# lxtGH/Video-K-Net

Hardware: AMD Instinct MI355X
Metric: frames/sec (S=3, N=100, 1024x2048) (higher is better)
Workload: dtype f32; 1 GPU; cfg2 video_knet_s3_r50: VideoKernelIterHead S=3, N=100 proposals + 17 stuff = 117 kernels, C=256, 1024x2048 frame -> 128x256 stride-8 features, ffn tracking link, x4 bilinear upsample of the final logits; streams_per_gpu=1, parallelism=frame-sharded dp1, x_storage=fp32

## Files before the change

### include/vkn.h

```cpp
#ifndef VKN_H
#define VKN_H
#include <stddef.h>
#include <stdint.h>

#ifdef __cplusplus
extern "C" {
#endif

#define VKN_VERSION 0x000600

#define VKN_OK 0
#define VKN_E_ARG (-1)
#define VKN_E_SHAPE (-2)
#define VKN_E_WORKSPACE (-3)
#define VKN_E_LAUNCH (-4)
#define VKN_E_ALIGN (-5)
#define VKN_E_RANGE (-6)

#define VKN_STATUS_RANGE 1u

#define VKN_FLAG_REF_KERNELS 1u
#define VKN_FLAG_EXACT_GEMM 2u
#define VKN_FLAG_LOGITS_HANDOFF 4u
#define VKN_FLAG_BITS_HANDOFF 16u
#define VKN_X_F32 0
#define VKN_X_F16 1
#define VKN_X_BF16 2
#define VKN_FLAG_X_F16 64u
#define VKN_FLAG_X_BF16 128u
#define VKN_FLAG_CHAIN_LAUNCHES 256u
#define VKN_FLAG_CHAIN_PERSISTENT 512u
#define VKN_FLAG_JOIN_EARLY 32768u
#define VKN_FLAG_SCALED_F16 16384u
#define VKN_FLAG_CHAIN_BF16X3 65536u
#define VKN_FLAG_CHAIN_KSPLIT 8192u
#define VKN_FLAG_SERIAL_LINK 32u
#define VKN_FLAG_CLIP_LINK 8u

#define VKN_FLAG_INIT_SEPARATE 131072u
#define VKN_FLAG_PHASE_A 1024u
#define VKN_FLAG_PHASE_B 2048u
#define VKN_FLAG_PHASE_C 4096u
#define VKN_FLAG_PHASE_MASK (VKN_FLAG_PHASE_A | VKN_FLAG_PHASE_B | VKN_FLAG_PHASE_C)

#define VKN_MAX_FCS 4

typedef struct VknDims {
    int B;
    int N;
    int C;
    int H, W;
    int heads;
    int ff;
    int ncls;
    int n_cls_fcs, n_mask_fcs;
    float thr_logit;
    float ln_eps;
} VknDims;

typedef struct VknStageWeights {
    const float *ft_w, *ft_b, *ft_wT;
    const float *dyn_w, *dyn_b;
    const float *inp_w, *inp_b;
    const float *ig_w, *ig_b, *ug_w, *ug_b;
    const float *norm_in_w, *norm_in_b;
    const float *norm_out_w, *norm_out_b;
    const float *inorm_in_w, *inorm_in_b;
    const float *inorm_out_w, *inorm_out_b;
    const float *fc_w, *fc_b, *fc_norm_w, *fc_norm_b;
    const float *attn_in_w, *attn_in_b;
    const float *attn_out_w, *attn_out_b;
    const float *attn_norm_w, *attn_norm_b;
    const float *ffn1_w, *ffn1_b;
    const float *ffn2_w, *ffn2_b;
    const float *ffn_norm_w, *ffn_norm_b;
    const float *cls_fc_w[VKN_MAX_FCS], *cls_ln_w[VKN_MAX_FCS], *cls_ln_b[VKN_MAX_FCS];
    const float *fc_cls_w, *fc_cls_b;
    const float *mask_fc_w[VKN_MAX_FCS], *mask_ln_w[VKN_MAX_FCS], *mask_ln_b[VKN_MAX_FCS];
    const float *fc_mask_w, *fc_mask_b;
    const float *pa_in_w, *pa_in_b, *pa_out_w, *pa_out_b, *pa_norm_w, *pa_norm_b;
    const float *lffn1_w, *lffn1_b, *lffn2_w, *lffn2_b, *lffn_norm_w, *lffn_norm_b;
    const void* prepared;
    size_t prepared_bytes;
} VknStageWeights;

int vkn_version(void);
const char* vkn_strerror(int code);
int vkn_workspace_init(void* ws, size_t ws_bytes, void* stream);
int vkn_workspace_status(void* ws, size_t ws_bytes, void* stream);
size_t vkn_sizeof_dims(void);
size_t vkn_sizeof_stage_weights(void);

size_t vkn_gather_workspace_bytes(int B, int N, int C, int P);
int vkn_mask_gather_f32(const float* x, const float* mask_logits, float thr_logit, float* xraw_out, float* cnt_out, int B,
                        int N, int C, int P, void* ws, size_t ws_bytes, unsigned flags, void* stream);

int vkn_mask_gather_real_f32(const float* x, const float* a, float* out, float* asum_out, int B, int N, int C, int P, void* ws,
                             size_t ws_bytes, void* stream);

size_t vkn_decode_workspace_bytes(int B, int N, int C);
int vkn_mask_decode_f32(const float* x, const float* kernels, const float* bias, float* out, int B, int N, int C, int P,
                        void* ws, size_t ws_bytes, unsigned flags, void* stream);
int vkn_mask_decode_scaled_f32(const float* x, const float* kernels, const float* bias, const float* out_scale, float* out, int B,
                               int N, int C, int P, void* ws, size_t ws_bytes, unsigned flags, void* stream);

int vkn_split_planes_f32(const float* kernels, void* kf_hi, void* kf_lo, int B, int N, int C, void* stream);
int vkn_mask_decode_planes_f32(const float* x, const void* kf_hi, const void* kf_lo, const float* bias, float* out, int B,
                               int N, int C, int P, void* stream);
int vkn_mask_decode_planes_x(const void* x, int x_dtype, const void* kf_hi, const void* kf_lo, const float* bias, float* out, int B,
                             int N, int C, int P, void* stream);

int vkn_decode_gather_supported(int C, int P);
int vkn_decode_gather_f32(const float* x, const void* kf_hi, const void* kf_lo, const float* bias, float thr_logit,
                          float* xraw_out, float* cnt_out, int B, int N, int C, int P, void* ws, size_t ws_bytes, void* stream);
int vkn_decode_gather_x(const void* x, int x_dtype, const void* kf_hi, const void* kf_lo, const float* bias, float thr_logit,
                        float* xraw_out, float* cnt_out, int B, int N, int C, int P, void* ws, size_t ws_bytes, void* stream);

int vkn_upsample_bilinear_f32(const float* in, float* out, int planes, int H, int W, int S, void* stream);
int vkn_upsample_bilinear_f16out(const float* in, void* out_f16, int planes, int H, int W, int S, void* stream);
int vkn_upsample_bilinear_bwd_f32(const float* grad_out, float* grad_in, int planes, int H, int W, int S, void* stream);

int vkn_focal_loss_blocks(int M, int ncls);
// ... 291 lines not shown
```

### video-k-net_amd/csrc/vkn_api.hip

```cpp
#include "../../include/vkn.h"
#include "vkn_common.h"
#include "vkn_launch.h"

namespace {

struct Carver {
    char* base;
    size_t off;
    template <class T>
    T* take(size_t n) {
        off = (off + 255) & ~(size_t)255;
        T* p = base ? reinterpret_cast<T*>(base + off) : nullptr;
        off += n * sizeof(T);
        return p;
    }
};

inline bool aligned16(const void* p) { return (reinterpret_cast<uintptr_t>(p) & 15) == 0; }
inline int npt_of(int N) { return (N + 31) / 32 * 32; }

struct StageWs {
    float *part, *cntp, *xraw, *cnt, *xfeat, *params, *inputf, *ig, *ug, *f, *obj1, *qkv, *ao, *obj2, *h, *partial, *t1, *t2,
        *maskfeat, *kb, *kern32, *lq, *lkv, *lobj, *lupd, *lf;
    _Float16 *kfh, *kfl;
    int* status;
};


enum MasksFrom {
    FROM_LOGITS,
    FROM_BITS,
    FROM_GATHERED,
    FROM_XFEAT
};
enum MasksTo {
    TO_LOGITS,
    TO_BITS,
    TO_GATHER,
    TO_KERNELS,
    TO_NONE
};
struct StageCall {
    const VknStageWeights* w = nullptr;
    const float *x = nullptr, *obj_in = nullptr;
    float *obj_out = nullptr, *cls_logits = nullptr, *x_feat_out = nullptr;
    bool cls_sigmoid = false;
    MasksFrom from = FROM_LOGITS;
    const float *masks_in = nullptr, *xfeat_in = nullptr;
    const unsigned* bits_in = nullptr;
    MasksTo to = TO_LOGITS;
    float* masks_out = nullptr;
    unsigned* bits_out = nullptr;
    float *kern_out = nullptr, *kb_out = nullptr;
    hipEvent_t prof0 = nullptr, prof1 = nullptr, obj_ready = nullptr;
    float* up_out = nullptr;
    int up_stride = 0, up_chunk = 0;
    bool* up_done = nullptr;
    const float* prev_obj = nullptr;
    float* track_out = nullptr;
    const VknStageWeights* link_pre = nullptr;
    const float* prev_pre = nullptr;
    const VknStageWeights* link_track = nullptr;
    int track_src = 0;
    bool keep_xfeat = false;
    const void* touch_next = nullptr;
    size_t touch_next_bytes = 0;
};

struct PrepW {
    const void *ft, *ftT, *dyn, *inp, *ig, *ug, *fc, *attn_in, *attn_out, *ffn1, *ffn2, *cls_fc[VKN_MAX_FCS], *fc_cls,
        *mask_fc[VKN_MAX_FCS], *fc_mask, *pa_in, *pa_in_kv, *pa_out, *lffn1, *lffn2;
    const void *dynft, *dec;
    float *dynft32, *bcnt, *dec32, *decb, *dvec, *kb0, *fmT;
    float* chain_consts;
    const void* h2[VKN_H2_COUNT];
    float* h2_scale;
    unsigned* h2_scratch;
};

inline bool has_composites(const VknDims* d, const VknStageWeights* w) {
    return w->ft_w && w->ft_wT && w->ft_b && w->dyn_w && w->dyn_b && w->fc_mask_w && w->fc_mask_b && d->n_mask_fcs > 0;
}

struct PrepItem {
    const float* src;
    int nout, k;
    const void** dst;
};

struct H2Shape { int nout, k; };
inline H2Shape h2_shape(const VknDims* d, const VknStageWeights* w, int i) {
    const int C = d->C, FF = d->ff;
    switch (i) {
        case VKN_H2_DYNFT: case VKN_H2_DYN: case VKN_H2_INP: return H2Shape{2 * C, C};
        case VKN_H2_IN: return H2Shape{3 * C, C};
        case VKN_H2_FFN1: return H2Shape{FF, C};
        case VKN_H2_FFN2: return H2Shape{C, FF};
        case VKN_H2_FCCLS: return H2Shape{w->fc_cls_w ? d->ncls : 0, C};
        default: return H2Shape{C, C};
    }
}

inline bool chain_width_ok(const VknDims* d) { return d->C == 256 && d->ff % 256 == 0 && d->ff <= 2048; }
inline bool chain_shape_ok(const VknDims* d) { return chain_width_ok(d) && d->n_cls_fcs == 1 && d->n_mask_fcs == 1; }

size_t carve_prepared(const VknDims* d, const VknStageWeights* w, char* base, PrepW* p, PrepItem* it = nullptr, int* n_out = nullptr) {
    const int C = d->C, FF = d->ff;
    Carver c{base, 0};
    int n = 0;
    auto add = [&](const float* src, int nout, int k, const void** dst) {
        *dst = src ? c.take<char>(vkn_split_w3_bytes(nout, k)) : nullptr;
        if (src && it) it[n] = PrepItem{src, nout, k, dst};
        if (src) ++n;
    };
    add(w->ft_w, C, C, &p->ft); add(w->ft_wT, C, C, &p->ftT);
    add(w->dyn_w, 2 * C, C, &p->dyn); add(w->inp_w, 2 * C, C, &p->inp);
    add(w->ig_w, C, C, &p->ig); add(w->ug_w, C, C, &p->ug); add(w->fc_w, C, C, &p->fc);
    add(w->attn_in_w, 3 * C, C, &p->attn_in); add(w->attn_out_w, C, C, &p->attn_out);
    add(w->ffn1_w, FF, C, &p->ffn1); add(w->ffn2_w, C, FF, &p->ffn2);
    for (int i = 0; i < VKN_MAX_FCS; ++i) add(i < d->n_cls_fcs ? w->cls_fc_w[i] : nullptr, C, C, &p->cls_fc[i]);
    add(w->fc_cls_w, d->ncls, C, &p->fc_cls);
    for (int i = 0; i < VKN_MAX_FCS; ++i) add(i < d->n_mask_fcs ? w->mask_fc_w[i] : nullptr, C, C, &p->mask_fc[i]);
    add(w->fc_mask_w, C, C, &p->fc_mask);
    add(w->pa_in_w, C, C, &p->pa_in); add(w->pa_in_w ? w->pa_in_w + (size_t)C * C : nullptr, 2 * C, C, &p->pa_in_kv);
    add(w->pa_out_w, C, C, &p->pa_out);
    add(w->lffn1_w, FF, C, &p->lffn1); add(w->lffn2_w, C, FF, &p->lffn2);
    p->dynft = p->dec = nullptr;
    p->dynft32 = p->bcnt = p->dec32 = p->decb = p->dvec = p->kb0 = p->fmT = p->chain_consts = nullptr;
    if (has_composites(d, w)) {
        const size_t Cs = d->C;
        p->dynft = c.take<char>(vkn_split_w3_bytes(2 * C, C));
        p->dec = c.take<char>(vkn_split_w3_bytes(C, C));
        p->dynft32 = c.take<float>(2 * Cs * Cs);
        p->bcnt = c.take<float>(2 * Cs);
        p->dec32 = c.take<float>(Cs * Cs);
        p->decb = c.take<float>(Cs);
        p->dvec = c.take<float>(Cs);
        p->kb0 = c.take<float>(4);
        p->fmT = c.take<float>(Cs * Cs);
        if (C == 256 && FF <= 2048) p->chain_consts = c.take<float>(vkn_chain_consts_floats());
    }
    for (int i = 0; i < VKN_H2_COUNT; ++i) p->h2[i] = nullptr;
    p->h2_scale = nullptr;
    p->h2_scratch = nullptr;
    if (has_composites(d, w) && chain_shape_ok(d) && w->inp_w && w->ig_w && w->ug_w && w->fc_w && w->attn_in_w && w->attn_out_w && w->ffn1_w &&
        w->ffn2_w && w->cls_fc_w[0] && w->mask_fc_w[0]) {
        for (int i = 0; i < VKN_H2_COUNT; ++i) {
            const H2Shape h = h2_shape(d, w, i);
            if (h.nout > 0) p->h2[i] = c.take<char>(vkn_split_h2_bytes(h.nout, h.k));
// ... 153 lines not shown
        e.bias = in_b + C; e.out = s.lkv; e.ldo = 2 * C;
        VKN_TRY(vkn_launch_gemm(kvsrc, nullptr, C, in_w + (size_t)C * C, in_kv_ws, M, C, 2 * C, 1, nullptr, e, st));
        VKN_TRY(vkn_launch_attn(s.lq, C, s.lkv, s.lkv + C, 2 * C, s.ao, C, d->B, d->N, d->N, heads, hd, st));
    }
    e = mk_epi(d);
    e.bias = out_b; e.resid = qsrc; e.ldr = C; e.ln_w = nw; e.ln_b = nb; e.out = out; e.ldo = C;
    return vkn_launch_gemm(s.ao, nullptr, C, out_w, out_ws, M, C, C, 1, nullptr, e, st);
}

int run_updator(const VknDims* d, const VknStageWeights* w, const PrepW& pw, const float* xfeat, const float* xraw,
                const float* cnt, const float* obj_in, float* out, const StageWs& s, hipStream_t st) {
    const int C = d->C, M = d->B * d->N;
    const bool fuse = (C == 256);
    VknGemmProb pr[2];
    VknEpi e = mk_epi(d); e.out = s.params; e.ldo = 2 * C;
    if (fuse) { e.ln_w = w->norm_out_w; e.ln_b = w->norm_out_b; e.ln_from_col = C; }
    if (xraw && pw.dynft) {
        e.bias = pw.bcnt; e.rowscale = cnt; e.bias2 = w->dyn_b;
        pr[0] = VknGemmProb{xraw, nullptr, nullptr, nullptr, C, pw.dynft32, pw.dynft, 2 * C, e};
    } else {
        e.bias = w->dyn_b;
        pr[0] = VknGemmProb{xfeat, nullptr, nullptr, nullptr, C, w->dyn_w, pw.dyn, 2 * C, e};
    }
    e = mk_epi(d); e.bias = w->inp_b; e.out = s.inputf; e.ldo = 2 * C;
    if (fuse) { e.ln_w = w->inorm_out_w; e.ln_b = w->inorm_out_b; e.ln_from_col = C; }
    pr[1] = VknGemmProb{obj_in, nullptr, nullptr, nullptr, C, w->inp_w, pw.inp, 2 * C, e};
    VKN_TRY(vkn_launch_gemm_group(pr, 2, M, C, 1, nullptr, st));
    float* ig = s.ig;
    float* ug = fuse ? s.ig + C : s.ug;
    const int ldg = fuse ? 2 * C : C;
    e = mk_epi(d); e.bias = w->ig_b; e.ln_w = w->inorm_in_w; e.ln_b = w->inorm_in_b; e.act = 2; e.out = ig; e.ldo = ldg;
    pr[0] = VknGemmProb{s.inputf, s.params, nullptr, nullptr, 2 * C, w->ig_w, pw.ig, C, e};
    e = mk_epi(d); e.bias = w->ug_b; e.ln_w = w->norm_in_w; e.ln_b = w->norm_in_b; e.act = 2; e.out = ug; e.ldo = ldg;
    pr[1] = VknGemmProb{s.inputf, s.params, nullptr, nullptr, 2 * C, w->ug_w, pw.ug, C, e};
    VKN_TRY(vkn_launch_gemm_group(pr, 2, M, C, 1, nullptr, st));
    e = mk_epi(d); e.bias = w->fc_b; e.ln_w = w->fc_norm_w; e.ln_b = w->fc_norm_b; e.act = 1; e.out = out; e.ldo = C;
    if (fuse) {
        pr[0] = VknGemmProb{ug, s.params + C, ig, s.inputf + C, 2 * C, w->fc_w, pw.fc, C, e};
        return vkn_launch_gemm_group(pr, 1, M, C, 1, nullptr, st);
    }
    VKN_TRY(vkn_launch_ku_mix(s.params, s.inputf, ig, ug, w->norm_out_w, w->norm_out_b, w->inorm_out_w, w->inorm_out_b,
                              d->ln_eps, s.f, M, C, st));
    return vkn_launch_gemm(s.f, nullptr, C, w->fc_w, pw.fc, M, C, C, 1, nullptr, e, st);
}

bool link_ks_ok(const VknDims* d, const VknStageWeights* w, const PrepW& pw, unsigned flags);
int run_link_ks(const VknDims* d, const VknStageWeights* w, const PrepW& pw, const float* cur, const float* kv, float* out,
                const StageWs& s, hipStream_t st);
int run_link(const VknDims* d, const VknStageWeights* w, const PrepW& pw, const float* cur, const float* prev,
             float* out, const StageWs& s, hipStream_t st, const float* update_feature = nullptr, unsigned flags = 0) {
    if (!w->pa_in_w || !w->lffn1_w) return VKN_E_ARG;
    const float* kv = prev;
    if (update_feature) {
        if (!w->dyn_w) return VKN_E_ARG;
        StageWs su = s;
        su.f = s.lf;
        VKN_TRY(run_updator(d, w, pw, update_feature, nullptr, nullptr, prev, s.lupd, su, st));
        kv = s.lupd;
    }
    if (link_ks_ok(d, w, pw, flags)) return run_link_ks(d, w, pw, cur, kv, out, s, st);
    VKN_TRY(run_attention(d, s, cur, kv, 8, w->pa_in_w, pw.pa_in, pw.pa_in_kv, w->pa_in_b, w->pa_out_w, pw.pa_out, w->pa_out_b,
                          w->pa_norm_w, w->pa_norm_b, s.t1, st));
    return run_ffn(d, s, s.t1, w->lffn1_w, pw.lffn1, w->lffn1_b, w->lffn2_w, pw.lffn2, w->lffn2_b, w->lffn_norm_w,
                   w->lffn_norm_b, out, st);
}

int carve_pw(const VknDims* d, const VknStageWeights* w, unsigned flags, PrepW* pw) {
    *pw = PrepW{};
    if (w->prepared && !(flags & VKN_FLAG_EXACT_GEMM) &&
        carve_prepared(d, w, static_cast<char*>(const_cast<void*>(w->prepared)), pw) > w->prepared_bytes)
        return VKN_E_WORKSPACE;
    return VKN_OK;
}

int run_track_link(const VknDims* d, const StageWs& s, hipStream_t st, const float* cur, const float* prev, float* out,
                   const VknStageWeights* w, const VknStageWeights* link_track, int track_src, const float* xfeat, unsigned flags) {
    const VknStageWeights* lw = link_track ? link_track : w;
    PrepW pw;
    VKN_TRY(carve_pw(d, lw, flags, &pw));
    return run_link(d, lw, pw, cur, prev, out, s, st, link_track ? (track_src == 2 ? cur : xfeat) : nullptr, flags);
}

int run_gather(const VknDims* d, const float* x, const float* masks, const unsigned* bits, const StageWs& s, unsigned flags,
               hipStream_t st, const void* touch = nullptr, size_t touch_bytes = 0) {
    const int B = d->B, N = d->N, C = d->C, P = d->H * d->W, xdt = xdt_of(flags);
    if (flags & VKN_FLAG_REF_KERNELS) return vkn_launch_gather_ref(x, masks, d->thr_logit, s.xraw, s.cnt, B, N, C, P, st);
    if (bits) return vkn_launch_gather_bits(x, bits, s.xraw, s.cnt, s.part, s.cntp, B, N, C, P, st, xdt, s.status, touch, touch_bytes);
    return vkn_launch_gather(x, masks, d->thr_logit, s.xraw, s.cnt, s.part, s.cntp, B, N, C, P, st, xdt, s.status, touch, touch_bytes);
}

int final_decode(const VknDims* d, const float* x, const StageWs& s, const float* kb, float* masks_out, unsigned flags,
                 hipStream_t st, hipEvent_t prof0, hipEvent_t prof1, float* up_out, int up_stride, int up_chunk, bool* up_done) {
    const int B = d->B, N = d->N, C = d->C, P = d->H * d->W;
    if ((flags & VKN_FLAG_REF_KERNELS) || (P & 1)) return vkn_launch_decode_ref(x, s.kern32, kb, masks_out, B, N, C, P, st);
    const int ch = (up_out && up_chunk > 0 && up_chunk < B) ? up_chunk : B;
    const size_t NPTC = (size_t)npt_of(N) * C;
    for (int b0 = 0; b0 < B; b0 += ch) {
        const int bn = (B - b0 < ch) ? B - b0 : ch;
        const float* xb = reinterpret_cast<const float*>(reinterpret_cast<const char*>(x) + (size_t)b0 * C * P * (xdt_of(flags) ? 2 : 4));
        if (b0 == 0 && prof0 && hipEventRecord(prof0, st) != hipSuccess) return VKN_E_LAUNCH;
        VKN_TRY(vkn_launch_decode(xb, s.kfh + b0 * NPTC, s.kfl + b0 * NPTC, kb ? kb + (size_t)b0 * N : nullptr,
                                  masks_out + (size_t)b0 * N * P, bn, N, C, P, st, xdt_of(flags)));
        if (b0 == 0 && prof1 && hipEventRecord(prof1, st) != hipSuccess) return VKN_E_LAUNCH;
        if (ch < B)
            VKN_TRY(vkn_launch_upsample(masks_out + (size_t)b0 * N * P,
                                        (flags & VKN_FLAG_SCALED_F16) ? reinterpret_cast<float*>(reinterpret_cast<_Float16*>(up_out) + (size_t)b0 * N * P * up_stride * up_stride)
                                                                      : up_out + (size_t)b0 * N * P * up_stride * up_stride,
                                        bn * N, d->H, d->W, up_stride, st, (flags & VKN_FLAG_SCALED_F16) ? 1 : 0));
    }
    if (ch < B && up_done) *up_done = true;
    return VKN_OK;
}

inline int persistent_min_row_tiles(const PrepW& pw, unsigned flags) {
    return (!(flags & VKN_FLAG_CHAIN_BF16X3) && pw.h2_scale && pw.h2[VKN_H2_DYNFT]) ? 22 : 64;
}
inline unsigned pw_off(const VknStageWeights* w, const void* p) {
    return (unsigned)(static_cast<const char*>(p) - static_cast<const char*>(w->prepared));
}
inline bool chain_weights_ok(const PrepW& pw, bool have_cls) {
    return pw.dynft && pw.dyn && pw.dec && pw.inp && pw.ig && pw.ug && pw.fc && pw.attn_in && pw.attn_out && pw.ffn1 && pw.ffn2 &&
           pw.cls_fc[0] && pw.mask_fc[0] && (!have_cls || pw.fc_cls);
}
inline bool chain_stage_ok(const VknDims* d, const VknStageWeights* w, const PrepW& pw, bool have_cls) {
    return chain_shape_ok(d) && w->prepared && w->prepared_bytes < (1ull << 31) && chain_weights_ok(pw, have_cls) && w->ffn1_w &&
           w->cls_ln_w[0] && w->mask_ln_w[0];
}
bool chain_fast_ok(const VknDims* d, const VknStageWeights* w, const PrepW& pw, unsigned flags, bool have_cls) {
    if (flags & (VKN_FLAG_CHAIN_LAUNCHES | VKN_FLAG_EXACT_GEMM)) return false;
    if (vkn_dbg_env("VKN_CHAIN_LAUNCHES", 0)) return false;
    if (!(flags & VKN_FLAG_CHAIN_PERSISTENT) && !vkn_dbg_env("VKN_CHAIN_PERSISTENT", 0) &&
        (d->B * d->N + 31) / 32 < persistent_min_row_tiles(pw, flags))
        return false;
    return pw.chain_consts && chain_stage_ok(d, w, pw, have_cls);
}
inline bool chain_h2(const PrepW& pw, unsigned flags, bool have_cls) {
    return !(flags & VKN_FLAG_CHAIN_BF16X3) && pw.h2_scale && pw.h2[VKN_H2_DYNFT] && pw.h2[VKN_H2_DEC] && (!have_cls || pw.h2[VKN_H2_FCCLS]);
}

int run_chain_fast(const VknDims* d, const VknStageWeights* w, const PrepW& pw, const float* a0, bool a0_raw, const float* cnt,
                   const float* obj_in, float* obj_out, float* cls_logits, bool cls_sigmoid, float* kern32_out, const StageWs& s,
                   hipStream_t st, bool h2 = false) {
    const int M = d->B * d->N, C = d->C;
    VknChainA a{};
    a.a0 = a0; a.obj_in = obj_in; a.rowscale = a0_raw ? cnt : nullptr;
    a.wbase = w->prepared; a.wbytes = w->prepared_bytes;
    if (h2) {
        a.off_dyn = pw_off(w, pw.h2[a0_raw ? VKN_H2_DYNFT : VKN_H2_DYN]);
        a.off_inp = pw_off(w, pw.h2[VKN_H2_INP]); a.off_ig = pw_off(w, pw.h2[VKN_H2_IG]); a.off_ug = pw_off(w, pw.h2[VKN_H2_UG]);
        a.off_fc = pw_off(w, pw.h2[VKN_H2_FC]); a.off_in = pw_off(w, pw.h2[VKN_H2_IN]);
    } else {
        a.off_dyn = pw_off(w, a0_raw ? pw.dynft : pw.dyn);
        a.off_inp = pw_off(w, pw.inp); a.off_ig = pw_off(w, pw.ig); a.off_ug = pw_off(w, pw.ug); a.off_fc = pw_off(w, pw.fc);
        a.off_in = pw_off(w, pw.attn_in);
    }
    a.consts = pw.chain_consts;
    a.eps = d->ln_eps; a.M = M; a.obj1 = s.obj1; a.qkv = s.qkv; a.status = s.status;
    VKN_TRY(h2 ? vkn_launch_chain_a_h2(a, st) : vkn_launch_chain_a(a, st));
    VKN_TRY(vkn_launch_attn(s.qkv, 3 * C, s.qkv + C, s.qkv + 2 * C, 3 * C, s.ao, C, d->B, d->N, d->N, d->heads, C / d->heads, st));
    VknChainC c{};
    c.ao = s.ao; c.obj1 = s.obj1; c.wbase = w->prepared; c.wbytes = w->prepared_bytes;
    if (h2) {
        c.off_out = pw_off(w, pw.h2[VKN_H2_OUT]); c.off_ffn1 = pw_off(w, pw.h2[VKN_H2_FFN1]); c.off_ffn2 = pw_off(w, pw.h2[VKN_H2_FFN2]);
        c.off_clsfc = pw_off(w, pw.h2[VKN_H2_CLSFC]); c.off_maskfc = pw_off(w, pw.h2[VKN_H2_MASKFC]);
        c.off_fccls = pw.h2[VKN_H2_FCCLS] ? pw_off(w, pw.h2[VKN_H2_FCCLS]) : 0u; c.off_dec = pw_off(w, pw.h2[VKN_H2_DEC]);
    } else {
        c.off_out = pw_off(w, pw.attn_out); c.off_ffn1 = pw_off(w, pw.ffn1); c.off_ffn2 = pw_off(w, pw.ffn2);
        c.off_clsfc = pw_off(w, pw.cls_fc[0]); c.off_maskfc = pw_off(w, pw.mask_fc[0]);
        c.off_fccls = pw.fc_cls ? pw_off(w, pw.fc_cls) : 0u; c.off_dec = pw_off(w, pw.dec);
    }
    c.consts = pw.chain_consts; c.kb0 = pw.kb0;
    c.ff = d->ff; c.ncls = d->ncls; c.cls_sigmoid = cls_sigmoid ? 1 : 0; c.eps = d->ln_eps; c.M = M;
    c.obj_out = obj_out; c.cls_out = cls_logits; c.kb_out = s.kb;
    if (kern32_out) c.kern_out = kern32_out;
    else { c.plane_hi = s.kfh; c.plane_lo = s.kfl; }
    c.rows_per_frame = d->N; c.NPT = npt_of(d->N); c.status = s.status;
    return h2 ? vkn_launch_chain_c_h2(c, st) : vkn_launch_chain_c(c, st);
}

#define VKN_KS_MAX_ROW_TILES 16
inline bool ks_width_ok(const VknDims* d) {
    return chain_width_ok(d) && (d->ff % 512 == 0 || d->ff <= 1024);
}
bool chain_ks_ok(const VknDims* d, const VknStageWeights* w, const PrepW& pw, unsigned flags, bool have_cls) {
    if (flags & (VKN_FLAG_CHAIN_LAUNCHES | VKN_FLAG_CHAIN_PERSISTENT | VKN_FLAG_EXACT_GEMM)) return false;
    if (vkn_dbg_env("VKN_CHAIN_LAUNCHES", 0) || vkn_dbg_env("VKN_CHAIN_PERSISTENT", 0) || !vkn_dbg_env("VKN_CHAIN_KSPLIT", 1)) return false;
    if (!(flags & VKN_FLAG_CHAIN_KSPLIT) && (d->B * d->N + 31) / 32 > VKN_KS_MAX_ROW_TILES) return false;
    if (!ks_width_ok(d) || !chain_stage_ok(d, w, pw, have_cls)) return false;
    const void* v16[] = {w->inorm_in_w, w->inorm_in_b, w->norm_in_w, w->norm_in_b, w->norm_out_w, w->norm_out_b, w->inorm_out_w, w->inorm_out_b,
                         w->fc_norm_w, w->fc_norm_b, w->attn_norm_w, w->attn_norm_b, w->ffn_norm_w, w->ffn_norm_b, w->ffn2_b,
                         w->cls_ln_w[0], w->cls_ln_b[0], w->mask_ln_w[0], w->mask_ln_b[0], pw.dvec};
    for (const void* p : v16)
        if (!p || !aligned16(p)) return false;
    return true;
}

VknKsProb ks_prob(const float* a, int lda, const void* W, int Nout, int KT, float eps) {
    VknKsProb p{};
    p.pro.a[0] = a; p.pro.lda[0] = lda; p.pro.nsum = 1; p.pro.eps = eps;
    p.Wsplit = W; p.Nout = Nout; p.KT = KT;
    return p;
}

int run_chain_ks(const VknDims* d, const VknStageWeights* w, const PrepW& pw, const float* a0, bool a0_raw, const float* cnt,
                 const float* obj_in, float* obj_out, float* cls_logits, bool cls_sigmoid, float* kern32_out, const StageWs& s,
                 hipStream_t st, hipEvent_t obj_ready) {
    const int M = d->B * d->N, C = d->C, FF = d->ff;
    const float eps = d->ln_eps;
    VknKsProb pr[2];
    pr[0] = ks_prob(a0, C, a0_raw ? pw.dynft : pw.dyn, 2 * C, 8, eps);
    if (a0_raw) { pr[0].epi.bias = pw.bcnt; pr[0].epi.rowscale = cnt; pr[0].epi.bias2 = w->dyn_b; }
    else pr[0].epi.bias = w->dyn_b;
    pr[0].epi.out = s.params; pr[0].epi.ldo = 2 * C;
    pr[1] = ks_prob(obj_in, C, pw.inp, 2 * C, 8, eps);
    pr[1].epi.bias = w->inp_b; pr[1].epi.out = s.inputf; pr[1].epi.ldo = 2 * C;
    VKN_TRY(vkn_launch_gemm_ks(pr, 2, 0, 0, 1, 0, M, st));
    pr[0] = ks_prob(s.inputf, 2 * C, pw.ig, C, 8, eps);
    pr[0].pro.a[1] = s.params; pr[0].pro.lda[1] = 2 * C;
    pr[1] = pr[0];
    pr[0].epi.bias = w->ig_b; pr[0].epi.out = s.ig; pr[0].epi.ldo = 2 * C;
    pr[1].Wsplit = pw.ug; pr[1].epi.bias = w->ug_b; pr[1].epi.out = s.ig + C; pr[1].epi.ldo = 2 * C;
    VKN_TRY(vkn_launch_gemm_ks(pr, 2, 1, 0, 1, 0, M, st));
    pr[0] = ks_prob(s.ig, 2 * C, pw.fc, C, 8, eps);
    pr[0].pro.a[1] = s.ig + C; pr[0].pro.lda[1] = 2 * C;
    pr[0].pro.a[2] = s.params + C; pr[0].pro.lda[2] = 2 * C;
    pr[0].pro.a[3] = s.inputf + C; pr[0].pro.lda[3] = 2 * C;
    pr[0].pro.ln_w[0] = w->inorm_in_w; pr[0].pro.ln_b[0] = w->inorm_in_b;
    pr[0].pro.ln_w[1] = w->norm_in_w; pr[0].pro.ln_b[1] = w->norm_in_b;
    pr[0].pro.ln_w[2] = w->norm_out_w; pr[0].pro.ln_b[2] = w->norm_out_b;
    pr[0].pro.ln_w[3] = w->inorm_out_w; pr[0].pro.ln_b[3] = w->inorm_out_b;
    pr[0].epi.bias = w->fc_b; pr[0].epi.out = s.f; pr[0].epi.ldo = C;
    VKN_TRY(vkn_launch_gemm_ks(pr, 1, 2, 0, 1, 0, M, st));
    pr[0] = ks_prob(s.f, C, pw.attn_in, 3 * C, 8, eps);
    pr[0].pro.ln_w[0] = w->fc_norm_w; pr[0].pro.ln_b[0] = w->fc_norm_b; pr[0].pro.act = 1;
    pr[0].pro.side_out = s.obj1; pr[0].pro.ld_side = C;
    pr[0].epi.bias = w->attn_in_b; pr[0].epi.out = s.qkv; pr[0].epi.ldo = 3 * C;
    VKN_TRY(vkn_launch_gemm_ks(pr, 1, 0, 0, 1, 0, M, st));
    VKN_TRY(vkn_launch_attn(s.qkv, 3 * C, s.qkv + C, s.qkv + 2 * C, 3 * C, s.ao, C, d->B, d->N, d->N, d->heads, C / d->heads, st));
    pr[0] = ks_prob(s.ao, C, pw.attn_out, C, 8, eps);
    pr[0].epi.bias = w->attn_out_b; pr[0].epi.resid = s.obj1; pr[0].epi.ldr = C; pr[0].epi.out = s.obj2; pr[0].epi.ldo = C;
    VKN_TRY(vkn_launch_gemm_ks(pr, 1, 0, 0, 1, 0, M, st));
    pr[0] = ks_prob(s.obj2, C, pw.ffn1, FF, 8, eps);
    pr[0].pro.ln_w[0] = w->attn_norm_w; pr[0].pro.ln_b[0] = w->attn_norm_b;
    pr[0].pro.side_out = s.t1; pr[0].pro.ld_side = C;
    pr[0].epi.bias = w->ffn1_b; pr[0].epi.act = 1; pr[0].epi.out = s.h; pr[0].epi.ldo = FF;
    VKN_TRY(vkn_launch_gemm_ks(pr, 1, 0, 0, 1, 0, M, st));
    const int kpw = (FF % 512 == 0) ? 2 : 1, zch = FF / (256 * kpw);
    pr[0] = ks_prob(s.h, FF, pw.ffn2, C, FF / 32, eps);
    pr[0].epi.out = s.partial; pr[0].epi.ldo = C;
    VKN_TRY(vkn_launch_gemm_ks(pr, 1, 0, zch, kpw, (long long)M * C, M, st));
    pr[0] = ks_prob(s.partial, C, pw.cls_fc[0], C, 8, eps);
    pr[0].pro.nsum = zch; pr[0].pro.sum_stride = (long long)M * C;
    pr[0].pro.pbias = w->ffn2_b; pr[0].pro.presid = s.t1; pr[0].pro.ldr = C;
    pr[0].pro.ln_w[0] = w->ffn_norm_w; pr[0].pro.ln_b[0] = w->ffn_norm_b;
    pr[1] = pr[0];
    pr[0].pro.side_out = obj_out; pr[0].pro.ld_side = C;
    pr[0].epi.out = s.lkv; pr[0].epi.ldo = 2 * C;
    pr[1].Wsplit = pw.mask_fc[0]; pr[1].epi.out = s.lkv + C; pr[1].epi.ldo = 2 * C;
    VKN_TRY(vkn_launch_gemm_ks(pr, 2, 0, 0, 1, 0, M, st));
    if (obj_ready && hipEventRecord(obj_ready, st) != hipSuccess) return VKN_E_LAUNCH;
    int np = 0;
    if (cls_logits) {
        pr[np] = ks_prob(s.lkv, 2 * C, pw.fc_cls, d->ncls, 8, eps);
        pr[np].pro.ln_w[0] = w->cls_ln_w[0]; pr[np].pro.ln_b[0] = w->cls_ln_b[0]; pr[np].pro.act = 1;
        pr[np].epi.bias = w->fc_cls_b; pr[np].epi.act = cls_sigmoid ? 2 : 0; pr[np].epi.out = cls_logits; pr[np].epi.ldo = d->ncls;
        ++np;
    }
    pr[np] = ks_prob(s.lkv + C, 2 * C, pw.dec, C, 8, eps);
    pr[np].pro.ln_w[0] = w->mask_ln_w[0]; pr[np].pro.ln_b[0] = w->mask_ln_b[0]; pr[np].pro.act = 1;
    pr[np].pro.dot_vec = pw.dvec; pr[np].pro.dot_bias = pw.kb0; pr[np].pro.dot_out = s.kb;
    pr[np].epi.bias = pw.decb; pr[np].epi.ldo = C;
    if (kern32_out) pr[np].epi.out = kern32_out;
    else { pr[np].epi.plane_hi = s.kfh; pr[np].epi.plane_lo = s.kfl; pr[np].epi.rows_per_frame = d->N; pr[np].epi.NPT = npt_of(d->N); }
    ++np;
    return vkn_launch_gemm_ks(pr, np, 0, 0, 1, 0, M, st);
}

bool link_ks_ok(const VknDims* d, const VknStageWeights* w, const PrepW& pw, unsigned flags) {
    if (flags & (VKN_FLAG_CHAIN_LAUNCHES | VKN_FLAG_CHAIN_PERSISTENT | VKN_FLAG_EXACT_GEMM)) return false;
    if (vkn_dbg_env("VKN_CHAIN_LAUNCHES", 0) || !vkn_dbg_env("VKN_CHAIN_KSPLIT", 1)) return false;
    if (!(flags & VKN_FLAG_CHAIN_KSPLIT) && (d->B * d->N + 31) / 32 > VKN_KS_MAX_ROW_TILES) return false;
    if (!ks_width_ok(d)) return false;
    if (!pw.pa_in || !pw.pa_in_kv || !pw.pa_out || !pw.lffn1 || !pw.lffn2) return false;
    if (!w->pa_norm_w || !w->pa_norm_b || !aligned16(w->pa_norm_w) || !aligned16(w->pa_norm_b)) return false;
    return true;
}

int run_link_ks(const VknDims* d, const VknStageWeights* w, const PrepW& pw, const float* cur, const float* kv, float* out,
                const StageWs& s, hipStream_t st) {
    const int M = d->B * d->N, C = d->C, FF = d->ff;
    const float eps = d->ln_eps;
    VknKsProb pr[2];
    pr[0] = ks_prob(cur, C, pw.pa_in, C, 8, eps);
    pr[0].epi.bias = w->pa_in_b; pr[0].epi.out = s.lq; pr[0].epi.ldo = C;
    pr[1] = ks_prob(kv, C, pw.pa_in_kv, 2 * C, 8, eps);
    pr[1].epi.bias = w->pa_in_b ? w->pa_in_b + C : nullptr; pr[1].epi.out = s.lkv; pr[1].epi.ldo = 2 * C;
    VKN_TRY(vkn_launch_gemm_ks(pr, 2, 0, 0, 1, 0, M, st));
    VKN_TRY(vkn_launch_attn(s.lq, C, s.lkv, s.lkv + C, 2 * C, s.ao, C, d->B, d->N, d->N, 8, C / 8, st));
    pr[0] = ks_prob(s.ao, C, pw.pa_out, C, 8, eps);
    pr[0].epi.bias = w->pa_out_b; pr[0].epi.resid = cur; pr[0].epi.ldr = C; pr[0].epi.out = s.t1; pr[0].epi.ldo = C;
    VKN_TRY(vkn_launch_gemm_ks(pr, 1, 0, 0, 1, 0, M, st));
    pr[0] = ks_prob(s.t1, C, pw.lffn1, FF, 8, eps);
    pr[0].pro.ln_w[0] = w->pa_norm_w; pr[0].pro.ln_b[0] = w->pa_norm_b;
    pr[0].pro.side_out = s.lf; pr[0].pro.ld_side = C;
    pr[0].epi.bias = w->lffn1_b; pr[0].epi.act = 1; pr[0].epi.out = s.h; pr[0].epi.ldo = FF;
    VKN_TRY(vkn_launch_gemm_ks(pr, 1, 0, 0, 1, 0, M, st));
    const int kpw = (FF % 512 == 0) ? 2 : 1, zch = FF / (256 * kpw);
    pr[0] = ks_prob(s.h, FF, pw.lffn2, C, FF / 32, eps);
    pr[0].epi.out = s.partial; pr[0].epi.ldo = C;
    VKN_TRY(vkn_launch_gemm_ks(pr, 1, 0, zch, kpw, (long long)M * C, M, st));
    VknEpi e = mk_epi(d);
    e.bias = w->lffn2_b; e.resid = s.lf; e.ldr = C; e.ln_w = w->lffn_norm_w; e.ln_b = w->lffn_norm_b; e.out = out; e.ldo = C;
    return vkn_launch_rowepi(s.partial, zch, M, C, e, st);
}

int emit_masks(const VknDims* d, const StageCall& c, const StageWs& s, bool ref_decode, const float* kern32, const float* kb,
               const void* touch, size_t touch_bytes, unsigned flags, hipStream_t st) {
    const int B = d->B, N = d->N, C = d->C, P = d->H * d->W, xdt = xdt_of(flags);
    if (c.to == TO_KERNELS) {
        if (c.kb_out && kb && hipMemcpyAsync(c.kb_out, kb, (size_t)B * N * sizeof(float), hipMemcpyDeviceToDevice, st) != hipSuccess)
            return VKN_E_LAUNCH;
        return VKN_OK;
    }
    if (c.to == TO_NONE) return VKN_OK;
    if (ref_decode) return vkn_launch_decode_ref(c.x, kern32, kb, c.masks_out, B, N, C, P, st);
    if (c.to == TO_GATHER)
        return vkn_launch_fused_decode_gather(c.x, s.kfh, s.kfl, kb, d->thr_logit, s.xraw, s.cnt, s.part, s.cntp, B, N, C, P, st, xdt, s.status,
                                              touch, touch_bytes);
    if (c.to == TO_BITS) return vkn_launch_decode_bits(c.x, s.kfh, s.kfl, kb, c.bits_out, d->thr_logit, B, N, C, P, st, xdt);
    return final_decode(d, c.x, s, kb, c.masks_out, flags, st, c.prof0, c.prof1, c.up_out, c.up_stride, c.up_chunk, c.up_done);
}

int run_stage(const VknDims* d, const StageCall& c, const StageWs& s, unsigned flags, hipStream_t st) {
    const VknStageWeights* w = c.w;
    const int N = d->N, C = d->C, P = d->H * d->W, M = d->B * N;
    const bool ref = (flags & VKN_FLAG_REF_KERNELS) != 0;
    const bool chain_only = c.to == TO_KERNELS, given_xfeat = c.from == FROM_XFEAT;
    const bool ref_decode = ref || (P & 1) || chain_only;
    const bool has_ft = w->ft_w != nullptr;
    const bool have_cls = w->fc_cls_w && c.cls_logits;
    float* const cls_logits = have_cls ? c.cls_logits : nullptr;
    const bool pre_link = c.link_pre && c.prev_pre;
    const bool need_xfeat = (pre_link && c.link_pre->dyn_w) || (c.link_track && c.track_src == 1) || c.keep_xfeat;
    if (xdt_of(flags) && !chain_only && (ref || (P % 64) != 0)) return VKN_E_SHAPE;
    PrepW pw;
    VKN_TRY(carve_pw(d, w, flags, &pw));
    const bool comp = pw.dynft != nullptr;
    const bool fewrow = comp && chain_ks_ok(d, w, pw, flags, have_cls), persistent = comp && chain_fast_ok(d, w, pw, flags, have_cls);
    const bool fast = fewrow || persistent;

    const bool will_fast = !given_xfeat && persistent && vkn_dbg_env("VKN_CHAIN_TOUCH", 1);
    const void* touch_nx = vkn_dbg_env("VKN_CHAIN_TOUCH", 1) ? c.touch_next : nullptr;
    const size_t touch_nx_bytes = touch_nx ? c.touch_next_bytes : 0;
    if (c.from == FROM_LOGITS || c.from == FROM_BITS)
        VKN_TRY(run_gather(d, c.x, c.masks_in, c.from == FROM_BITS ? c.bits_in : nullptr, s, flags, st, will_fast ? w->prepared : nullptr,
                           will_fast ? w->prepared_bytes : 0));

    float* xfeat = c.x_feat_out ? c.x_feat_out : s.xfeat;
    VknEpi e = mk_epi(d);
    if (given_xfeat) {
        xfeat = const_cast<float*>(c.xfeat_in);
    } else if (has_ft) {
        if (!comp || c.x_feat_out || need_xfeat) {
            e.bias = w->ft_b; e.rowscale = s.cnt; e.out = xfeat; e.ldo = C;
            VKN_TRY(vkn_launch_gemm(s.xraw, nullptr, C, w->ft_w, pw.ft, M, C, C, 1, nullptr, e, st));
        }
    } else {
        if (hipMemcpyAsync(xfeat, s.xraw, (size_t)M * C * sizeof(float), hipMemcpyDeviceToDevice, st) != hipSuccess)
            return VKN_E_LAUNCH;
    }

    const float* obj_in = c.obj_in;
    if (pre_link) {
        PrepW pl;
        VKN_TRY(carve_pw(d, c.link_pre, flags, &pl));
        VKN_TRY(run_link(d, c.link_pre, pl, obj_in, c.prev_pre, s.lobj, s, st, c.link_pre->dyn_w ? xfeat : nullptr, flags));
        obj_in = s.lobj;
    }

    const float* kb = has_ft ? s.kb : nullptr;
    float* const kern32 = ref_decode ? (chain_only ? c.kern_out : s.kern32) : nullptr;
    const bool link = c.prev_obj && c.track_out;
    if (fast) {
        const bool raw = !given_xfeat;
        if (fewrow) {
            VKN_TRY(run_chain_ks(d, w, pw, raw ? s.xraw : xfeat, raw, s.cnt, obj_in, c.obj_out, cls_logits, c.cls_sigmoid, kern32, s, st, c.obj_ready));
        } else {
            VKN_TRY(run_chain_fast(d, w, pw, raw ? s.xraw : xfeat, raw, s.cnt, obj_in, c.obj_out, cls_logits, c.cls_sigmoid, kern32, s, st,
                                   chain_h2(pw, flags, have_cls)));
            if (c.obj_ready && hipEventRecord(c.obj_ready, st) != hipSuccess) return VKN_E_LAUNCH;
        }
        VKN_TRY(emit_masks(d, c, s, ref_decode, s.kern32, kb, touch_nx, touch_nx_bytes, flags, st));
        if (link) VKN_TRY(run_track_link(d, s, st, c.obj_out, c.prev_obj, c.track_out, w, c.link_track, c.track_src, xfeat, flags));
        return VKN_OK;
    }

    VKN_TRY(run_updator(d, w, pw, xfeat, (comp && !given_xfeat) ? s.xraw : nullptr, s.cnt, obj_in, s.obj1, s, st));

    VKN_TRY(run_attention(d, s, s.obj1, s.obj1, d->heads, w->attn_in_w, pw.attn_in, nullptr, w->attn_in_b, w->attn_out_w,
                          pw.attn_out, w->attn_out_b, w->attn_norm_w, w->attn_norm_b, s.obj2, st));
    if (w->ffn1_w) {
        VKN_TRY(run_ffn(d, s, s.obj2, w->ffn1_w, pw.ffn1, w->ffn1_b, w->ffn2_w, pw.ffn2, w->ffn2_b, w->ffn_norm_w,
                        w->ffn_norm_b, c.obj_out, st));
    } else {
        if (hipMemcpyAsync(c.obj_out, s.obj2, (size_t)M * C * sizeof(float), hipMemcpyDeviceToDevice, st) != hipSuccess)
            return VKN_E_LAUNCH;
    }
    const float* obj3 = c.obj_out;

    const bool fork_late = vkn_dbg_env("VKN_LINK_FORK_LATE", 0) != 0;
    if (c.obj_ready && !fork_late && hipEventRecord(c.obj_ready, st) != hipSuccess) return VKN_E_LAUNCH;

    const float* tc = obj3;
    const float* tm = obj3;
    const int nl = d->n_cls_fcs > d->n_mask_fcs ? d->n_cls_fcs : d->n_mask_fcs;
    VknGemmProb pr[2];
    for (int i = 0; i < nl; ++i) {
        int np = 0;
        if (i < d->n_cls_fcs) {
            float* dst = (i & 1) ? s.t2 : s.t1;
            e = mk_epi(d); e.ln_w = w->cls_ln_w[i]; e.ln_b = w->cls_ln_b[i]; e.act = 1; e.out = dst; e.ldo = C;
            pr[np++] = VknGemmProb{tc, nullptr, nullptr, nullptr, C, w->cls_fc_w[i], pw.cls_fc[i], C, e};
            tc = dst;
        }
        if (i < d->n_mask_fcs) {
            float* dst = (i & 1) ? s.lq : s.f;
            e = mk_epi(d); e.ln_w = w->mask_ln_w[i]; e.ln_b = w->mask_ln_b[i]; e.act = 1; e.out = dst; e.ldo = C;
            if (comp && i == d->n_mask_fcs - 1) { e.dot_vec = pw.dvec; e.dot_bias = pw.kb0; e.dot_out = s.kb; }
            pr[np++] = VknGemmProb{tm, nullptr, nullptr, nullptr, C, w->mask_fc_w[i], pw.mask_fc[i], C, e};
            tm = dst;
        }
        VKN_TRY(vkn_launch_gemm_group(pr, np, M, C, 1, nullptr, st));
    }
    auto to_kernels = [&](VknEpi& ep) {
        ep.ldo = C;
        if (kern32) ep.out = kern32;
        else { ep.plane_hi = s.kfh; ep.plane_lo = s.kfl; ep.rows_per_frame = N; ep.NPT = npt_of(N); }
    };
    int np = 0;
    if (have_cls) {
        e = mk_epi(d); e.bias = w->fc_cls_b; e.out = cls_logits; e.ldo = d->ncls;
        if (c.cls_sigmoid) e.act = 2;
        pr[np++] = VknGemmProb{tc, nullptr, nullptr, nullptr, C, w->fc_cls_w, pw.fc_cls, d->ncls, e};
    }
    const float* kern = s.kern32;
    if (comp) {
        e = mk_epi(d); e.bias = pw.decb; to_kernels(e);
        pr[np++] = VknGemmProb{tm, nullptr, nullptr, nullptr, C, pw.dec32, pw.dec, C, e};
        VKN_TRY(vkn_launch_gemm_group(pr, np, M, C, 1, nullptr, st));
    } else {
        e = mk_epi(d); e.bias = w->fc_mask_b; e.out = (chain_only && !has_ft) ? c.kern_out : s.maskfeat; e.ldo = C;
        if (has_ft) { e.dot_vec = w->ft_b; e.dot_out = s.kb; }
        pr[np++] = VknGemmProb{tm, nullptr, nullptr, nullptr, C, w->fc_mask_w, pw.fc_mask, C, e};
        VKN_TRY(vkn_launch_gemm_group(pr, np, M, C, 1, nullptr, st));
        if (has_ft) {
            e = mk_epi(d); to_kernels(e);
            VKN_TRY(vkn_launch_gemm(s.maskfeat, nullptr, C, w->ft_wT, pw.ftT, M, C, C, 1, nullptr, e, st));
        } else if (chain_only) {
            if (c.kb_out && hipMemsetAsync(c.kb_out, 0, (size_t)M * sizeof(float), st) != hipSuccess) return VKN_E_LAUNCH;
        } else if (!ref_decode) {
            VKN_TRY(vkn_launch_split_planes(s.maskfeat, s.kfh, s.kfl, d->B, N, C, st));
        } else if (c.to == TO_NONE) {
            if (hipMemcpyAsync(s.kern32, s.maskfeat, (size_t)M * C * sizeof(float), hipMemcpyDeviceToDevice, st) != hipSuccess)
                return VKN_E_LAUNCH;
        } else {
            kern = s.maskfeat;
        }
    }
    VKN_TRY(emit_masks(d, c, s, ref_decode, kern, kb, touch_nx, touch_nx_bytes, flags, st));

    if (c.obj_ready && fork_late && hipEventRecord(c.obj_ready, st) != hipSuccess) return VKN_E_LAUNCH;
    if (link) VKN_TRY(run_track_link(d, s, st, obj3, c.prev_obj, c.track_out, w, c.link_track, c.track_src, xfeat, flags));
    return VKN_OK;
}

StageWs frame_ws(const StageWs& s, const VknDims* d, int b) {
    StageWs r = s;
    const size_t R = (size_t)b * d->N, C = d->C;
    r.xraw += R * C; r.cnt += R; r.xfeat += R * C; r.params += R * 2 * C; r.inputf += R * 2 * C; r.ig += R * 2 * C; r.ug += R * C;
    r.f += R * C; r.obj1 += R * C; r.qkv += R * 3 * C; r.ao += R * C; r.obj2 += R * C; r.h += R * d->ff; r.t1 += R * C; r.t2 += R * C;
    r.maskfeat += R * C; r.kb += R; r.kern32 += R * C; r.lq += R * C; r.lkv += R * 2 * C; r.lobj += R * C; r.lupd += R * C; r.lf += R * C;
    r.kfh += (size_t)b * npt_of(d->N) * C; r.kfl += (size_t)b * npt_of(d->N) * C;
    return r;
}

struct InitWs {
    _Float16 *ih, *il, *sh, *sl;
    float *part, *cntp, *cnt, *obj, *seg;
    _Float16 *ph, *pl;
    unsigned* bits;
};
size_t carve_init(int B, int Np, int ncls, int C, int P, bool need_seg, char* base, InitWs* s) {
    Carver c{base, 0};
    const size_t G = vkn_gather_groups(B, P), NPTp = npt_of(Np), NPTs = npt_of(ncls > 0 ? ncls : 1);
    s->ih = c.take<_Float16>(NPTp * C);
    s->il = c.take<_Float16>(NPTp * C);
    s->sh = c.take<_Float16>(NPTs * C);
    s->sl = c.take<_Float16>(NPTs * C);
    s->part = c.take<float>((size_t)B * G * NPTp * C);
    s->cntp = c.take<float>((size_t)B * G * NPTp);
    s->cnt = c.take<float>((size_t)B * Np);
    s->obj = c.take<float>((size_t)B * Np * C);
    s->seg = need_seg ? c.take<float>((size_t)B * ncls * P) : nullptr;
    s->ph = s->pl = nullptr;
    s->bits = nullptr;
    if (ncls > 0 && vkn_init_pass_supported(Np, ncls, C, P)) {
        s->ph = c.take<_Float16>((size_t)160 * C);
        s->pl = c.take<_Float16>((size_t)160 * C);
        s->bits = c.take<unsigned>((size_t)B * (P / 32) * NPTp);
    }
    return (c.off + 255) & ~(size_t)255;
}

}

// ... 562 lines not shown
    *mtmp = c.take<float>(M * P);
    *otmp = c.take<float>(M * d->C);
    *ctmp = c.take<float>(M * d->ncls);
    const size_t nw = (size_t)d->B * ((P + 31) / 32) * npt_of(d->N);
    bits[0] = c.take<unsigned>(nw);
    bits[1] = c.take<unsigned>(nw);
    return (c.off + 255) & ~(size_t)255;
}

size_t vkn_head_workspace_bytes(const VknDims* d) {
    if (check_dims(d) != VKN_OK) return 0;
    StageWs s;
    float *a, *b, *c;
    unsigned* bits[2];
    return carve_head(d, nullptr, &s, &a, &b, &c, bits);
}

static int head_forward_impl(const VknDims* d, int num_stages, const VknStageWeights* stages, const VknStageWeights* link_pre,
                             const VknStageWeights* link_track, int track_src, const float* x, const float* proposal_feats,
                             const float* mask_preds_in, const float* prev_obj, float* obj_out, float* cls_prob,
                             float* mask_preds_out, float* scaled_out, int upsample_stride, float* track_out, void* ws,
                             size_t ws_bytes, unsigned flags, void* stream, void* ev_decode_start, void* ev_decode_stop);

int vkn_head_forward_f32(const VknDims* d, int num_stages, const VknStageWeights* stages, const float* x,
                         const float* proposal_feats, const float* mask_preds_in, const float* prev_obj, float* obj_out,
                         float* cls_prob, float* mask_preds_out, float* scaled_out, int upsample_stride, float* track_out,
                         void* ws, size_t ws_bytes, unsigned flags, void* stream) {
    return head_forward_impl(d, num_stages, stages, nullptr, nullptr, 0, x, proposal_feats, mask_preds_in, prev_obj, obj_out,
                             cls_prob, mask_preds_out, scaled_out, upsample_stride, track_out, ws, ws_bytes, flags, stream, nullptr,
                             nullptr);
}

int vkn_head_forward_prof_f32(const VknDims* d, int num_stages, const VknStageWeights* stages, const float* x,
                              const float* proposal_feats, const float* mask_preds_in, const float* prev_obj, float* obj_out,
                              float* cls_prob, float* mask_preds_out, float* scaled_out, int upsample_stride, float* track_out,
                              void* ws, size_t ws_bytes, unsigned flags, void* stream, void* ev_decode_start,
                              void* ev_decode_stop) {
    return head_forward_impl(d, num_stages, stages, nullptr, nullptr, 0, x, proposal_feats, mask_preds_in, prev_obj, obj_out,
                             cls_prob, mask_preds_out, scaled_out, upsample_stride, track_out, ws, ws_bytes, flags, stream,
                             ev_decode_start, ev_decode_stop);
}

int vkn_head_forward_link_f32(const VknDims* d, int num_stages, const VknStageWeights* stages, const VknStageWeights* link_pre,
                              const VknStageWeights* link_track, int track_src, const float* x, const float* proposal_feats,
                              const float* mask_preds_in, const float* prev_obj, float* obj_out, float* cls_prob,
                              float* mask_preds_out, float* scaled_out, int upsample_stride, float* track_out, void* ws,
                              size_t ws_bytes, unsigned flags, void* stream) {
    if (track_src < 0 || track_src > 2 || (link_track && track_src == 0)) return VKN_E_ARG;
    return head_forward_impl(d, num_stages, stages, link_pre, link_track, track_src, x, proposal_feats, mask_preds_in, prev_obj,
                             obj_out, cls_prob, mask_preds_out, scaled_out, upsample_stride, track_out, ws, ws_bytes, flags, stream,
                             nullptr, nullptr);
}

static int head_forward_impl(const VknDims* d, int num_stages, const VknStageWeights* stages, const VknStageWeights* link_pre,
                             const VknStageWeights* link_track, int track_src, const float* x, const float* proposal_feats,
                             const float* mask_preds_in, const float* prev_obj, float* obj_out, float* cls_prob,
                             float* mask_preds_out, float* scaled_out, int upsample_stride, float* track_out, void* ws,
                             size_t ws_bytes, unsigned flags, void* stream, void* ev_decode_start, void* ev_decode_stop) {
    VKN_TRY(check_dims(d));
    if (num_stages <= 0 || !stages || !x || !proposal_feats || !mask_preds_in || !obj_out || !cls_prob || !mask_preds_out)
        return VKN_E_ARG;
    if (!aligned16(x) || !aligned16(proposal_feats) || !aligned16(mask_preds_in) || !aligned16(obj_out) ||
        !aligned16(mask_preds_out) || (scaled_out && !aligned16(scaled_out)))
        return VKN_E_ALIGN;
    if (mask_preds_in == mask_preds_out || proposal_feats == obj_out) return VKN_E_ARG;
    StageWs s;
    float *mtmp, *otmp, *ctmp;
    unsigned* bits[2];
    const size_t need = carve_head(d, nullptr, &s, &mtmp, &otmp, &ctmp, bits);
    if (!ws || ws_bytes < need || !aligned16(ws)) return VKN_E_WORKSPACE;
    carve_head(d, static_cast<char*>(ws), &s, &mtmp, &otmp, &ctmp, bits);
    hipStream_t st = static_cast<hipStream_t>(stream);
    const bool use_bits = !(flags & (VKN_FLAG_REF_KERNELS | VKN_FLAG_LOGITS_HANDOFF)) && ((d->H * d->W) % 64) == 0;
    const bool use_fused = use_bits && !(flags & VKN_FLAG_BITS_HANDOFF) && vkn_fused_supported(d->C, d->H * d->W);

    const unsigned ph = flags & VKN_FLAG_PHASE_MASK;
    const bool do_a = !ph || (ph & VKN_FLAG_PHASE_A), do_b = !ph || (ph & VKN_FLAG_PHASE_B), do_c = !ph || (ph & VKN_FLAG_PHASE_C);
    if (ph && !(link_pre && (flags & VKN_FLAG_CLIP_LINK) && prev_obj)) return VKN_E_ARG;

    const float* m_in = mask_preds_in;
    const float* o_in = proposal_feats;
    SideStream* joined = nullptr;
    bool up_done = false;
    for (int sidx = 0; sidx < num_stages; ++sidx) {
        const bool last = (sidx == num_stages - 1);
        if (!last && !do_a) {
            const bool to_out_s = ((num_stages - 1 - sidx) & 1) == 0;
            m_in = to_out_s ? mask_preds_out : mtmp;
            o_in = to_out_s ? obj_out : otmp;
            continue;
        }
        const bool to_out = ((num_stages - 1 - sidx) & 1) == 0;
        float* m_out = to_out ? mask_preds_out : mtmp;
        float* o_out = to_out ? obj_out : otmp;
        const float* prev = (last && track_out) ? prev_obj : nullptr;
        const bool clip = prev && (flags & VKN_FLAG_CLIP_LINK);
        SideStream* side = (prev && !(flags & VKN_FLAG_SERIAL_LINK)) ? side_stream() : nullptr;
        const bool link_after = clip || side;
        const float* prev_in_stage = link_after ? nullptr : prev;
        const unsigned* b_in = (use_bits && !use_fused && sidx > 0) ? bits[(sidx - 1) & 1] : nullptr;
        unsigned* b_out = (use_bits && !use_fused && !last) ? bits[sidx & 1] : nullptr;
        const float* prev_pre = (last && link_pre) ? prev_obj : nullptr;
        const bool seq = prev_pre && (flags & VKN_FLAG_CLIP_LINK) && (d->B > 1 || ph);
        const VknStageWeights* ltrack = (last && track_out) ? link_track : nullptr;
        StageCall c{};
        c.w = &stages[sidx]; c.x = x; c.obj_in = o_in; c.obj_out = o_out;
        c.cls_logits = last ? cls_prob : ctmp;
        c.cls_sigmoid = last;
        c.from = (use_fused && sidx > 0) ? FROM_GATHERED : (b_in ? FROM_BITS : FROM_LOGITS);
        c.masks_in = m_in; c.bits_in = b_in;
        c.link_pre = prev_pre ? link_pre : nullptr; c.prev_pre = prev_pre;
        c.link_track = ltrack; c.track_src = track_src;
        if (!last && use_fused && !(flags & (VKN_FLAG_CHAIN_LAUNCHES | VKN_FLAG_EXACT_GEMM)) && stages[sidx + 1].prepared) {
            PrepW pwn;
            (void)carve_pw(d, &stages[sidx + 1], flags, &pwn);
            if ((flags & VKN_FLAG_CHAIN_PERSISTENT) || (d->B * d->N + 31) / 32 >= persistent_min_row_tiles(pwn, flags)) {
                if (chain_h2(pwn, flags, false)) {
                    c.touch_next = pwn.h2[VKN_H2_DYNFT];
                    c.touch_next_bytes = (size_t)(reinterpret_cast<const char*>(pwn.h2_scale) - static_cast<const char*>(pwn.h2[VKN_H2_DYNFT]));
                } else {
                    c.touch_next = stages[sidx + 1].prepared;
                    c.touch_next_bytes = stages[sidx + 1].prepared_bytes;
                }
            }
        }
        hipEvent_t ev0 = last ? static_cast<hipEvent_t>(ev_decode_start) : nullptr;
        hipEvent_t ev1 = last ? static_cast<hipEvent_t>(ev_decode_stop) : nullptr;
        float* up_out = (last && scaled_out && upsample_stride > 1) ? scaled_out : nullptr;
        if (!seq) {
            c.to = (use_fused && !last) ? TO_GATHER : (b_out ? TO_BITS : TO_LOGITS);
            c.masks_out = m_out; c.bits_out = b_out;
            c.prof0 = ev0; c.prof1 = ev1; c.obj_ready = (prev && side) ? side->fork : nullptr;
            c.up_out = up_out; c.up_stride = upsample_stride; c.up_chunk = vkn_dbg_env("VKN_LAST_CHUNK", 0); c.up_done = &up_done;
            c.prev_obj = prev_in_stage; c.track_out = prev_in_stage ? track_out : nullptr;
            VKN_TRY(run_stage(d, c, s, flags, st));
        } else {
            const int N = d->N, C = d->C;
            if (do_a && c.from != FROM_GATHERED) VKN_TRY(run_gather(d, x, m_in, b_in, s, flags, st));
            VknDims d1 = *d;
            d1.B = 1;
            c.from = FROM_GATHERED;
            c.to = TO_NONE;
            c.keep_xfeat = ltrack && track_src == 1;
            c.link_track = nullptr;
            for (int b = 0; b < (do_b ? d->B : 0); ++b) {
                const size_t r = (size_t)b * N;
                const StageWs sb = frame_ws(s, d, b);
                c.obj_in = o_in + r * C; c.obj_out = o_out + r * C; c.cls_logits = cls_prob + r * d->ncls;
                c.prev_pre = b == 0 ? prev_obj : o_out + (r - N) * C;
                VKN_TRY(run_stage(&d1, c, sb, flags, st));
            }
            if (!do_c) return VKN_OK;
            if (prev && side && hipEventRecord(side->fork, st) != hipSuccess) return VKN_E_LAUNCH;
            VKN_TRY(final_decode(d, x, s, stages[sidx].ft_w ? s.kb : nullptr, m_out, flags, st, ev0, ev1, up_out, upsample_stride,
                                 vkn_dbg_env("VKN_LAST_CHUNK", 0), &up_done));
        }
        m_in = m_out;
        o_in = o_out;
        if (prev && link_after) {
            hipStream_t ls = side ? side->st : st;
            if (side && hipStreamWaitEvent(side->st, side->fork, 0) != hipSuccess) return VKN_E_LAUNCH;
            StageWs sl = s;
            if (side) {
                sl.lq = s.qkv;
                sl.lkv = s.qkv + (size_t)d->B * d->N * d->C;
                sl.t1 = s.obj1;
            }
            const float* pv = prev;
            if (clip) {
                const size_t fr = (size_t)d->N * d->C;
                float* pvb = otmp;
                if (hipMemcpyAsync(pvb, prev_obj, fr * sizeof(float), hipMemcpyDeviceToDevice, ls) != hipSuccess) return VKN_E_LAUNCH;
                if (d->B > 1 &&
                    hipMemcpyAsync(pvb + fr, obj_out, (size_t)(d->B - 1) * fr * sizeof(float), hipMemcpyDeviceToDevice, ls) != hipSuccess)
                    return VKN_E_LAUNCH;
                pv = pvb;
            }
            VKN_TRY(run_track_link(d, sl, ls, obj_out, pv, track_out, &stages[sidx], ltrack, track_src, s.xfeat, flags));
            if (side) {
                if (hipEventRecord(side->join, side->st) != hipSuccess) return VKN_E_LAUNCH;
                joined = side;
            }
        }
    }
    const bool join_early = (flags & VKN_FLAG_JOIN_EARLY) != 0;
    if (joined && join_early && hipStreamWaitEvent(st, joined->join, 0) != hipSuccess) return VKN_E_LAUNCH;
    if (scaled_out && upsample_stride > 1 && !up_done)
        VKN_TRY(vkn_launch_upsample(mask_preds_out, scaled_out, d->B * d->N, d->H, d->W, upsample_stride, st, (flags & VKN_FLAG_SCALED_F16) ? 1 : 0));
    if (joined && !join_early && hipStreamWaitEvent(st, joined->join, 0) != hipSuccess) return VKN_E_LAUNCH;
    return VKN_OK;
}

}
```

### video-k-net_amd/csrc/vkn_chain.hip

```cpp
#include "vkn_common.h"
#include "vkn_launch.h"

#ifdef CH_H2
typedef _Float16 ch_e;
#define CH_NPL 2
#define CH_WTILE 32768u
#define k_chain_a k_chain_a_h2
#define k_chain_c k_chain_c_h2
#define ChainAArgs ChainAArgsH2
#define ChainCArgs ChainCArgsH2
#define vkn_launch_chain_a vkn_launch_chain_a_h2
#define vkn_launch_chain_c vkn_launch_chain_c_h2
#else
typedef __bf16 ch_e;
#define CH_NPL 3
#define CH_WTILE 49152u
#endif
typedef ch_e ch_ex8 __attribute__((ext_vector_type(8)));
typedef ch_e ch_ex4 __attribute__((ext_vector_type(4)));
typedef unsigned int cu32x4 __attribute__((ext_vector_type(4)));

#define CH_THREADS 512
#define CH_ROWS 32
#define CH_C 256
// ... 197 lines not shown
        p[v] = s;
    }
}

template <int NV>
__device__ __forceinline__ void ch_layernorm(float (&v)[NV][16], const float* const (&lw)[NV], const float* const (&lb)[NV], float eps,
                                             float* S, int& sb, const ChLane& L) {
    float p[NV];
#pragma unroll
    for (int i = 0; i < NV; ++i) {
        float s = 0.f;
#pragma unroll
        for (int r = 0; r < 16; ++r) s += v[i][r];
        p[i] = s;
    }
    ch_rowsum<NV>(p, S + sb * CH_SBUF, L);
    sb ^= 1;
    float mean[NV];
#pragma unroll
    for (int i = 0; i < NV; ++i) {
        mean[i] = p[i] / 256.f;
        float s = 0.f;
#pragma unroll
        for (int r = 0; r < 16; ++r) {
            const float d = v[i][r] - mean[i];
            s += d * d;
        }
        p[i] = s;
    }
    ch_rowsum<NV>(p, S + sb * CH_SBUF, L);
    sb ^= 1;
#pragma unroll
    for (int i = 0; i < NV; ++i) {
        const float rstd = 1.0f / sqrtf(p[i] / 256.f + eps);
        float w[16], b[16];
        ch_cols(lw[i], L, w);
        ch_cols(lb[i], L, b);
#pragma unroll
        for (int r = 0; r < 16; ++r) v[i][r] = (v[i][r] - mean[i]) * rstd * w[r] + b[r];
    }
}

__device__ __forceinline__ void ch_img_write(ch_e* img, const float (&v)[16], const ChLane& L) {
#ifdef CH_H2
    {
        float m = 0.f;
#pragma unroll
        for (int r = 0; r < 16; ++r) m = fmaxf(m, fabsf(v[r]));
        bool bad = !(m < 32768.f);
#pragma unroll
        for (int r = 0; r < 16; ++r) bad |= (v[r] != v[r]);
        if (bad && L.status) atomicOr(L.status, VKN_STATUS_RANGE);
    }
#endif
#pragma unroll
    for (int q = 0; q < 4; ++q) {
        const float t[4] = {v[4 * q], v[4 * q + 1], v[4 * q + 2], v[4 * q + 3]};
        ch_ex4 o[CH_NPL];
        ch_split4(t, o);
        ch_e* d = img + L.li * CH_C + ((((L.wave << 2) + q) ^ L.li) & 31) * 8 + 4 * L.g;
#pragma unroll
        for (int i = 0; i < CH_NPL; ++i) *reinterpret_cast<ch_ex4*>(d + i * CH_PLANE) = o[i];
    }
}
#ifdef CH_H2
__device__ __forceinline__ float ch_img_write_rs(ch_e* img, const float (&v)[16], const ChLane& L, float* X) {
    float m = 0.f;
#pragma unroll
    for (int r = 0; r < 16; ++r) m = fmaxf(m, fabsf(v[r]));
    X[(L.wave * 2 + L.g) * 32 + L.li] = m;
    CH_BAR();
#pragma unroll
    for (int k = 0; k < 16; ++k) m = fmaxf(m, X[k * 32 + L.li]);
    float inv;
    const float sc = ch_row_pow2(m, inv);
    float t[16];
#pragma unroll
    for (int r = 0; r < 16; ++r) t[r] = v[r] * sc;
    ch_img_write(img, t, L);
    return inv;
}
#endif

__device__ __forceinline__ void ch_img_load(ch_e* img, const float* __restrict__ src, int ld, int m0, int M, int tid, float* rs = nullptr) {
    const int row = tid >> 4, c4 = (tid & 15) << 2;
    const float* s = src + (size_t)min(m0 + row, M - 1) * ld + c4;
    f32x4 t[4];
#pragma unroll
    for (int j = 0; j < 4; ++j) t[j] = *reinterpret_cast<const f32x4*>(s + 64 * j);
#ifdef CH_H2
    {
        float m = 0.f;
#pragma unroll
        for (int j = 0; j < 4; ++j)
#pragma unroll
            for (int e = 0; e < 4; ++e) m = fmaxf(m, fabsf(t[j][e]));
#pragma unroll
        for (int o = 1; o < 16; o <<= 1) m = fmaxf(m, __shfl_xor(m, o));
        float inv;
        const float sc = ch_row_pow2(m, inv);
#pragma unroll
        for (int j = 0; j < 4; ++j) t[j] *= sc;
        if ((tid & 15) == 0) rs[row] = inv;
    }
#endif
#pragma unroll
    for (int j = 0; j < 4; ++j) {
        const int col = c4 + 64 * j;
        const float tv[4] = {t[j][0], t[j][1], t[j][2], t[j][3]};
        ch_ex4 o[CH_NPL];
        ch_split4(tv, o);
        ch_e* d = img + row * CH_C + ((((col >> 3) ^ row) & 31) << 3) + (col & 7);
#pragma unroll
        for (int i = 0; i < CH_NPL; ++i) *reinterpret_cast<ch_ex4*>(d + i * CH_PLANE) = o[i];
    }
}
#ifdef CH_H2
#define CH_UNSCALE(A, U)                                     \
    do {                                                     \
        const float u_ = (U);                                \
        _Pragma("unroll") for (int r_ = 0; r_ < 16; ++r_)(A)[r_] *= u_; \
    } while (0)
#else
#define CH_UNSCALE(A, U) \
    do {                 \
    } while (0)
#endif

__device__ __forceinline__ void ch_store_rows(float* __restrict__ dst, int ld, int col0, int row, bool ok, const float (&v)[16],
                                              const ChLane& L) {
    if (!ok) return;
    float* d = dst + (size_t)row * ld + col0 + L.wave * 32 + 4 * L.g;
#pragma unroll
    for (int q = 0; q < 4; ++q) *reinterpret_cast<f32x4*>(d + 8 * q) = f32x4{v[4 * q], v[4 * q + 1], v[4 * q + 2], v[4 * q + 3]};
}

__device__ __forceinline__ void ch_park(float* P, const float (&v)[16], int tid) {
#pragma unroll
    for (int q = 0; q < 4; ++q) *reinterpret_cast<f32x4*>(P + (q * CH_THREADS + tid) * 4) = f32x4{v[4 * q], v[4 * q + 1], v[4 * q + 2], v[4 * q + 3]};
}
__device__ __forceinline__ void ch_unpark(const float* P, float (&v)[16], int tid) {
#pragma unroll
    for (int q = 0; q < 4; ++q) {
        const f32x4 t = *reinterpret_cast<const f32x4*>(P + (q * CH_THREADS + tid) * 4);
#pragma unroll
        for (int e = 0; e < 4; ++e) v[4 * q + e] = t[e];
    }
}

template <int NF>
__device__ __forceinline__ void ch_stage_consts(float* cst, const float* __restrict__ src, int tid) {
    constexpr int NV = NF / 4, PER = (NV + CH_THREADS - 1) / CH_THREADS;
    f32x4 t[PER];
#pragma unroll
    for (int i = 0; i < PER; ++i) {
        const int k = tid + i * CH_THREADS;
        t[i] = *reinterpret_cast<const f32x4*>(src + 4 * min(k, NV - 1));
    }
#pragma unroll
    for (int i = 0; i < PER; ++i) {
        const int k = tid + i * CH_THREADS;
        if (k < NV) *reinterpret_cast<f32x4*>(cst + 4 * k) = t[i];
    }
}

}

enum {
    CA_DYN_B = 0,
    CA_DYN_B2 = 512,
    CA_NO_W = 1024, CA_NO_B = 1280,
    CA_INP_B = 1536,
    CA_INO_W = 2048, CA_INO_B = 2304,
    CA_IG_B = 2560, CA_INI_W = 2816, CA_INI_B = 3072,
    CA_UG_B = 3328, CA_NI_W = 3584, CA_NI_B = 3840,
    CA_FC_B = 4096, CA_FCN_W = 4352, CA_FCN_B = 4608,
    CA_IN_B = 4864,
    CA_SC = 5632,
    CA_TOTAL = 5640
};

struct ChainAArgs {
    const float* a0;
    const float* obj_in;
    const float* rowscale;
    const void* wbase;
    unsigned wbytes;
    unsigned off_dyn, off_inp, off_ig, off_ug, off_fc, off_in;
    float eps;
    int M;
    float* obj1;
    float* qkv;
    const float* consts;
    int* status;
};

template <int ABL>
__global__ __launch_bounds__(CH_THREADS) void k_chain_a(const ChainAArgs A) {
    extern __shared__ __attribute__((aligned(16))) char smem_ca[];
    ch_e* IMG0 = reinterpret_cast<ch_e*>(smem_ca);
    ch_e* IMG1 = IMG0 + CH_IMG;
    float* S = reinterpret_cast<float*>(IMG1 + CH_IMG);
    float* CST = S + 2 * CH_SBUF;
    float* PARK = CST + CA_TOTAL;
#ifdef CH_H2
    float* RS = PARK + 16 * CH_THREADS;
#endif

    const int tid = threadIdx.x;
    ChLane L_ = ch_lane(tid);
    L_.status = A.status;
    const ChLane L = L_;
    const int m0 = blockIdx.x * CH_ROWS, M = A.M;
    const int row = m0 + L.li;
    const bool row_ok = row < M;
    const __amdgpu_buffer_rsrc_t wrs = __builtin_amdgcn_make_buffer_rsrc(const_cast<void*>(A.wbase), 0, (int)A.wbytes, 0x00020000);

    constexpr int RING = CH_RING_OF(ABL);
    ChRing<RING> R;
    {
        const ChNext first{A.off_dyn, A.off_dyn + 8u * CH_WTILE, 2};
#pragma unroll
        for (int j = 0; j < RING - 1; ++j) ch_wload<RING, CH_AUX_OF(ABL), CH_NP_OF(ABL)>(R, j, wrs, L, first.off(j));
        if (CH_NOLOAD(ABL)) ch_wload<RING>(R, RING - 1, wrs, L, A.off_dyn);
    }
    ch_stage_consts<CA_TOTAL>(CST, A.consts, tid);
#ifdef CH_H2
    ch_img_load(IMG0, A.a0, CH_C, m0, M, tid, RS);
    ch_img_load(IMG1, A.obj_in, CH_C, m0, M, tid, RS + 32);
#else
    ch_img_load(IMG0, A.a0, CH_C, m0, M, tid);
    ch_img_load(IMG1, A.obj_in, CH_C, m0, M, tid);
#endif
    const float bs = A.rowscale ? A.rowscale[min(row, M - 1)] : 1.f;
    CH_BAR();

    int sb = 0;
    f32x16 acc[2];
    float pout[1][16];
    ch_zero(acc[0]);
    ch_zero(acc[1]);
    ch_gemm<2, true, ABL>(acc, IMG0, IMG0, A.off_dyn, A.off_dyn + 8u * CH_WTILE, ChNext{A.off_inp, A.off_inp + 8u * CH_WTILE, 2}, R, wrs, L);
    CH_UNSCALE(acc[0], CST[CA_SC + 0] * RS[L.li]);
    CH_UNSCALE(acc[1], CST[CA_SC + 0] * RS[L.li]);
    {
        float b[16], b2[16], pin[16];
        ch_cols(CST + CA_DYN_B, L, b);
        ch_cols(CST + CA_DYN_B2, L, b2);
#pragma unroll
        for (int r = 0; r < 16; ++r) pin[r] = acc[0][r] + b[r] * bs + b2[r];
        ch_park(PARK, pin, tid);
        ch_cols(CST + CA_DYN_B + 256, L, b);
        ch_cols(CST + CA_DYN_B2 + 256, L, b2);
#pragma unroll
        for (int r = 0; r < 16; ++r) pout[0][r] = acc[1][r] + b[r] * bs + b2[r];
        const float* const lw[1] = {CST + CA_NO_W};
        const float* const lb[1] = {CST + CA_NO_B};
        ch_layernorm<1>(pout, lw, lb, A.eps, S, sb, L);
    }
    ch_zero(acc[0]);
    ch_zero(acc[1]);
    ch_gemm<2, true, ABL>(acc, IMG1, IMG1, A.off_inp, A.off_inp + 8u * CH_WTILE, ChNext{A.off_ig, A.off_ug, 2}, R, wrs, L);
    CH_UNSCALE(acc[0], CST[CA_SC + 1] * RS[32 + L.li]);
    CH_UNSCALE(acc[1], CST[CA_SC + 1] * RS[32 + L.li]);
#ifdef CH_H2
    float gate_inv;
#endif
    {
        float b[16], gate[16], iout[1][16];
        ch_cols(CST + CA_INP_B, L, b);
        ch_unpark(PARK, gate, tid);
#pragma unroll
        for (int r = 0; r < 16; ++r) gate[r] = (acc[0][r] + b[r]) * gate[r];
#ifdef CH_H2
        gate_inv = ch_img_write_rs(IMG0, gate, L, RS + 64);
#else
        ch_img_write(IMG0, gate, L);
#endif
        ch_cols(CST + CA_INP_B + 256, L, b);
#pragma unroll
        for (int r = 0; r < 16; ++r) iout[0][r] = acc[1][r] + b[r];
        const float* const lw[1] = {CST + CA_INO_W};
        const float* const lb[1] = {CST + CA_INO_B};
        ch_layernorm<1>(iout, lw, lb, A.eps, S, sb, L);
        ch_park(PARK, iout[0], tid);
    }
    ch_zero(acc[0]);
    ch_zero(acc[1]);
    ch_gemm<2, true, ABL>(acc, IMG0, IMG0, A.off_ig, A.off_ug, ChNext{A.off_fc, 0u, 1}, R, wrs, L);
#ifdef CH_H2
    CH_UNSCALE(acc[0], CST[CA_SC + 2] * gate_inv);
    CH_UNSCALE(acc[1], CST[CA_SC + 3] * gate_inv);
#endif
    {
        float gt[2][16], b[16];
        ch_cols(CST + CA_IG_B, L, b);
#pragma unroll
        for (int r = 0; r < 16; ++r) gt[0][r] = acc[0][r] + b[r];
        ch_cols(CST + CA_UG_B, L, b);
#pragma unroll
        for (int r = 0; r < 16; ++r) gt[1][r] = acc[1][r] + b[r];
        const float* const lw[2] = {CST + CA_INI_W, CST + CA_NI_W};
        const float* const lb[2] = {CST + CA_INI_B, CST + CA_NI_B};
        ch_layernorm<2>(gt, lw, lb, A.eps, S, sb, L);
        float f[16];
        ch_unpark(PARK, f, tid);
#pragma unroll
        for (int r = 0; r < 16; ++r) {
            const float ig = 1.0f / (1.0f + expf(-gt[0][r]));
            const float ug = 1.0f / (1.0f + expf(-gt[1][r]));
            f[r] = ug * pout[0][r] + ig * f[r];
        }
        ch_img_write(IMG1, f, L);
        CH_BAR();
    }
    f32x16 acc1[1];
    ch_zero(acc1[0]);
    ch_gemm<1, true, ABL>(acc1, IMG1, IMG1, A.off_fc, 0u, ChNext{A.off_in, 0u, 1}, R, wrs, L);
    CH_UNSCALE(acc1[0], CST[CA_SC + 4]);
    {
        float o[1][16], b[16];
        ch_cols(CST + CA_FC_B, L, b);
#pragma unroll
        for (int r = 0; r < 16; ++r) o[0][r] = acc1[0][r] + b[r];
        const float* const lw[1] = {CST + CA_FCN_W};
        const float* const lb[1] = {CST + CA_FCN_B};
        ch_layernorm<1>(o, lw, lb, A.eps, S, sb, L);
#pragma unroll
        for (int r = 0; r < 16; ++r) o[0][r] = fmaxf(o[0][r], 0.f);
        ch_store_rows(A.obj1, CH_C, 0, row, row_ok, o[0], L);
        ch_img_write(IMG0, o[0], L);
        CH_BAR();
    }
#pragma unroll 1
    for (int t = 0; t < 3; ++t) {
        asm volatile("" ::: "memory");
        ch_zero(acc1[0]);
        const ChNext nx = (t < 2) ? ChNext{A.off_in + (unsigned)(t + 1) * 8u * CH_WTILE, 0u, 1} : ChNext{0u, 0u, 0};
        ch_gemm<1, true, ABL>(acc1, IMG0, IMG0, A.off_in + (unsigned)t * 8u * CH_WTILE, 0u, nx, R, wrs, L);
        CH_UNSCALE(acc1[0], CST[CA_SC + 5]);
        float o[16], b[16];
        ch_cols(CST + CA_IN_B + 256 * t, L, b);
#pragma unroll
        for (int r = 0; r < 16; ++r) o[r] = acc1[0][r] + b[r];
        ch_store_rows(A.qkv, 3 * CH_C, 256 * t, row, row_ok, o, L);
    }
}

enum {
    CC_OUT_B = 0, CC_AN_W = 256, CC_AN_B = 512,
    CC_B2 = 768, CC_FN_W = 1024, CC_FN_B = 1280,
    CC_CLN_W = 1536, CC_CLN_B = 1792,
    CC_MLN_W = 2048, CC_MLN_B = 2304,
    CC_DVEC = 2560,
    CC_CLS_B = 2816,
    CC_DEC_B = 3072,
    CC_B1 = 3328,
    CC_SC = 3328 + 2048,
    CC_TOTAL = 3328 + 2048 + 8
};

struct ChainCArgs {
    const float* ao;
    const float* obj1;
    const void* wbase;
    unsigned wbytes;
    unsigned off_out, off_ffn1, off_ffn2, off_clsfc, off_maskfc, off_fccls, off_dec;
    int nchunks;
    int has_cls;
    int cls_sigmoid;
    int ncls;
    float eps;
    int M;
    const float* kb0;
    float* obj_out;
    float* cls_out;
    float* kb_out;
    _Float16* plane_hi;
    _Float16* plane_lo;
    float* kern_out;
    int rows_per_frame, NPT;
    const float* consts;
    int* status;
};

template <int ABL>
__global__ __launch_bounds__(CH_THREADS) void k_chain_c(const ChainCArgs A) {
    extern __shared__ __attribute__((aligned(16))) char smem_cc[];
    ch_e* IMG0 = reinterpret_cast<ch_e*>(smem_cc);
    ch_e* HID = IMG0 + CH_IMG;
    float* S = reinterpret_cast<float*>(HID + CH_IMG);
    float* CST = S + 2 * CH_SBUF;
#ifdef CH_H2
    float* RS = CST + CC_TOTAL;
#endif

    const int tid = threadIdx.x;
    ChLane L_ = ch_lane(tid);
    L_.status = A.status;
    const ChLane L = L_;
    const int m0 = blockIdx.x * CH_ROWS, M = A.M;
    const int row = m0 + L.li;
    const bool row_ok = row < M;
    const int rowc = min(row, M - 1);
    const __amdgpu_buffer_rsrc_t wrs = __builtin_amdgcn_make_buffer_rsrc(const_cast<void*>(A.wbase), 0, (int)A.wbytes, 0x00020000);

    constexpr int RING = CH_RING_OF(ABL);
    ChRing<RING> R;
    {
        const ChNext first{A.off_out, 0u, 1};
#pragma unroll
        for (int j = 0; j < RING - 1; ++j) ch_wload<RING, CH_AUX_OF(ABL), CH_NP_OF(ABL)>(R, j, wrs, L, first.off(j));
        if (CH_NOLOAD(ABL)) ch_wload<RING>(R, RING - 1, wrs, L, A.off_out);
    }
    ch_stage_consts<CC_TOTAL>(CST, A.consts, tid);
#ifdef CH_H2
    ch_img_load(IMG0, A.ao, CH_C, m0, M, tid, RS);
#else
    ch_img_load(IMG0, A.ao, CH_C, m0, M, tid);
#endif
    float obj[1][16];
    {
        const float* s = A.obj1 + (size_t)rowc * CH_C + L.wave * 32 + 4 * L.g;
#pragma unroll
        for (int q = 0; q < 4; ++q) {
            const f32x4 t = *reinterpret_cast<const f32x4*>(s + 8 * q);
#pragma unroll
            for (int e = 0; e < 4; ++e) obj[0][4 * q + e] = t[e];
        }
    }
    CH_BAR();

    int sb = 0;
    f32x16 acc1[1];
    ch_zero(acc1[0]);
    ch_gemm<1, true, ABL>(acc1, IMG0, IMG0, A.off_out, 0u, ChNext{A.off_ffn1, 0u, 1}, R, wrs, L);
    CH_UNSCALE(acc1[0], CST[CC_SC + 0] * RS[L.li]);
    {
        float b[16];
        ch_cols(CST + CC_OUT_B, L, b);
#pragma unroll
        for (int r = 0; r < 16; ++r) obj[0][r] = acc1[0][r] + b[r] + obj[0][r];
        const float* const lw[1] = {CST + CC_AN_W};
        const float* const lb[1] = {CST + CC_AN_B};
        ch_layernorm<1>(obj, lw, lb, A.eps, S, sb, L);
        ch_img_write(IMG0, obj[0], L);
        CH_BAR();
    }
    f32x16 acc2[1];
    ch_zero(acc2[0]);
#pragma unroll 1
    for (int c = 0; c < A.nchunks; ++c) {
        ch_zero(acc1[0]);
        ch_gemm<1, true, ABL>(acc1, IMG0, IMG0, A.off_ffn1 + (unsigned)c * 8u * CH_WTILE, 0u,
                         ChNext{A.off_ffn2 + (unsigned)c * 8u * CH_WTILE, 0u, 1}, R, wrs, L);
        CH_UNSCALE(acc1[0], CST[CC_SC + 1]);
        float h[16], b[16];
        ch_cols(CST + CC_B1 + 256 * c, L, b);
#pragma unroll
        for (int r = 0; r < 16; ++r) h[r] = fmaxf(acc1[0][r] + b[r], 0.f);
        CH_BAR();
        ch_img_write(HID, h, L);
        CH_BAR();
        const bool lastc = (c + 1 == A.nchunks);
        const ChNext nx = lastc ? ChNext{A.off_clsfc, A.off_maskfc, 2} : ChNext{A.off_ffn1 + (unsigned)(c + 1) * 8u * CH_WTILE, 0u, 1};
        ch_gemm<1, true, ABL>(acc2, HID, HID, A.off_ffn2 + (unsigned)c * 8u * CH_WTILE, 0u, nx, R, wrs, L);
    }
    CH_UNSCALE(acc2[0], CST[CC_SC + 2]);
    {
        float b[16];
        ch_cols(CST + CC_B2, L, b);
#pragma unroll
        for (int r = 0; r < 16; ++r) obj[0][r] = obj[0][r] + acc2[0][r] + b[r];
        const float* const lw[1] = {CST + CC_FN_W};
        const float* const lb[1] = {CST + CC_FN_B};
        ch_layernorm<1>(obj, lw, lb, A.eps, S, sb, L);
        ch_store_rows(A.obj_out, CH_C, 0, row, row_ok, obj[0], L);
        ch_img_write(IMG0, obj[0], L);
        CH_BAR();
    }
    f32x16 acc[2];
    ch_zero(acc[0]);
    ch_zero(acc[1]);
    const ChNext nfin = A.has_cls ? ChNext{A.off_fccls, A.off_dec, 2} : ChNext{A.off_dec, 0u, 1};
    ch_gemm<2, true, ABL>(acc, IMG0, IMG0, A.off_clsfc, A.off_maskfc, nfin, R, wrs, L);
    CH_UNSCALE(acc[0], CST[CC_SC + 3]);
    CH_UNSCALE(acc[1], CST[CC_SC + 4]);
    {
        float t[2][16];
#pragma unroll
        for (int r = 0; r < 16; ++r) {
            t[0][r] = acc[0][r];
            t[1][r] = acc[1][r];
        }
        const float* const lw[2] = {CST + CC_CLN_W, CST + CC_MLN_W};
        const float* const lb[2] = {CST + CC_CLN_B, CST + CC_MLN_B};
        ch_layernorm<2>(t, lw, lb, A.eps, S, sb, L);
        float dv[16], kd[1];
        ch_cols(CST + CC_DVEC, L, dv);
        kd[0] = 0.f;
#pragma unroll
        for (int r = 0; r < 16; ++r) {
            t[0][r] = fmaxf(t[0][r], 0.f);
            t[1][r] = fmaxf(t[1][r], 0.f);
            kd[0] += t[1][r] * dv[r];
        }
        ch_img_write(IMG0, t[0], L);
        ch_img_write(HID, t[1], L);
        ch_rowsum<1>(kd, S + sb * CH_SBUF, L);
        sb ^= 1;
        if (row_ok && L.wave == 0 && L.g == 0 && A.kb_out) A.kb_out[row] = kd[0] + (A.kb0 ? *A.kb0 : 0.f);
    }
    ch_zero(acc[0]);
    ch_zero(acc[1]);
    if (A.has_cls) {
        ch_gemm<2, false, ABL>(acc, IMG0, HID, A.off_fccls, A.off_dec, ChNext{0u, 0u, 0}, R, wrs, L);
        CH_UNSCALE(acc[0], CST[CC_SC + 5]);
        if (L.wave * 32 < A.ncls && row_ok && A.cls_out) {
            float b[16];
            ch_cols(CST + CC_CLS_B, L, b);
#pragma unroll
            for (int r = 0; r < 16; ++r) {
                const int col = L.wave * 32 + 8 * (r >> 2) + 4 * L.g + (r & 3);
                float v = acc[0][r] + b[r];
                if (A.cls_sigmoid) v = 1.0f / (1.0f + expf(-v));
                if (col < A.ncls) A.cls_out[(size_t)row * A.ncls + col] = v;
            }
        }
    } else {
        f32x16 accd[1];
        ch_zero(accd[0]);
        ch_gemm<1, true, ABL>(accd, HID, HID, A.off_dec, 0u, ChNext{0u, 0u, 0}, R, wrs, L);
        acc[1] = accd[0];
    }
    CH_UNSCALE(acc[1], CST[CC_SC + 6]);
    {
        float k[16], b[16];
        ch_cols(CST + CC_DEC_B, L, b);
#pragma unroll
        for (int r = 0; r < 16; ++r) k[r] = acc[1][r] + b[r];
        if (A.plane_hi) {
            if (row_ok) {
                const int fb = row / A.rows_per_frame, n = row - fb * A.rows_per_frame;
                const size_t base = ((size_t)fb * A.NPT + n) * CH_C + L.wave * 32 + 4 * L.g;
#pragma unroll
                for (int q = 0; q < 4; ++q) {
                    half4 h, l;
#pragma unroll
                    for (int e = 0; e < 4; ++e) {
                        _Float16 hh, ll;
                        vkn_split_f16(k[4 * q + e], hh, ll);
                        h[e] = hh;
                        l[e] = ll;
                    }
                    *reinterpret_cast<half4*>(A.plane_hi + base + 8 * q) = h;
                    *reinterpret_cast<half4*>(A.plane_lo + base + 8 * q) = l;
                }
            }
        } else {
            ch_store_rows(A.kern_out, CH_C, 0, row, row_ok, k, L);
        }
    }
}

#ifndef CH_H2
template <int ABL, int KC>
__global__ __launch_bounds__(CH_THREADS) void k_gemm_t3(const VknGemmProb p0, const VknGemmProb p1, int nprob, int M) {
    extern __shared__ __attribute__((aligned(16))) char smem_t3[];
    ch_e* IMG = reinterpret_cast<ch_e*>(smem_t3);
    float* S = reinterpret_cast<float*>(IMG + KC * CH_IMG);
    const bool second = (nprob > 1) && (blockIdx.z == 1);
    const VknGemmProb& P = second ? p1 : p0;
    const VknEpi& E = P.epi;
    const int Nout = P.Nout;
    const int m0 = blockIdx.y * CH_ROWS, n0 = blockIdx.x * 256;
    if (n0 >= Nout) return;

    const int tid = threadIdx.x;
    const ChLane L = ch_lane(tid);
    const int ntiles = (Nout + 255) / 256;
    const __amdgpu_buffer_rsrc_t wrs = __builtin_amdgcn_make_buffer_rsrc(const_cast<void*>(P.Wsplit), 0, (int)((unsigned)ntiles * (8u * KC) * CH_WTILE), 0x00020000);
    const unsigned wbase = (unsigned)blockIdx.x * (8u * KC) * CH_WTILE;
    constexpr int RING = CH_RING_OF(ABL);
    ChRing<RING> R;
#pragma unroll
    for (int j = 0; j < RING - 1; ++j) ch_wload<RING, CH_AUX_OF(ABL)>(R, j, wrs, L, wbase + (unsigned)j * CH_WTILE);

#pragma unroll
    for (int kc = 0; kc < KC; ++kc) {
        const int row = tid >> 4, c4 = (tid & 15) << 2;
        const size_t ro = (size_t)min(m0 + row, M - 1) * P.lda + c4 + 256 * kc;
        f32x4 t[4];
#pragma unroll
        for (int j = 0; j < 4; ++j) t[j] = *reinterpret_cast<const f32x4*>(P.A + ro + 64 * j);
        if (P.A2) {
#pragma unroll
            for (int j = 0; j < 4; ++j) t[j] *= *reinterpret_cast<const f32x4*>(P.A2 + ro + 64 * j);
        }
// ... 187 lines not shown
};
__global__ __launch_bounds__(256) void k_chain_pack(const ChPackTab T, float* __restrict__ out) {
    const int i = blockIdx.x;
    const float* s = T.src[i];
    for (int k = threadIdx.x; k < T.n[i]; k += 256) out[T.dst[i] + k] = s ? s[k] : T.fill[i];
}
static void ch_tab_add(ChPackTab& T, const float* src, int dst, int n, float fill) {
    if (T.count >= CH_PACK_MAX) return;
    const int i = T.count++;
    T.src[i] = src;
    T.dst[i] = dst;
    T.n[i] = n;
    T.fill[i] = fill;
}

size_t vkn_chain_consts_floats() { return (size_t)2 * CA_TOTAL + CC_TOTAL; }

int vkn_chain_pack_consts(const VknChainConsts& c, float* out, hipStream_t stream) {
    if (!out || c.ff <= 0 || c.ff > 2048 || c.ncls < 0 || c.ncls > 256) return VKN_E_ARG;
    ChPackTab T;
    T.count = 0;
    for (int mode = 0; mode < 2; ++mode) {
        const int o = mode * CA_TOTAL;
        ch_tab_add(T, mode == 0 ? c.bcnt : c.dyn_b, o + CA_DYN_B, 512, 0.f);
        ch_tab_add(T, mode == 0 ? c.dyn_b : nullptr, o + CA_DYN_B2, 512, 0.f);
        ch_tab_add(T, c.norm_out_w, o + CA_NO_W, 256, 1.f);   ch_tab_add(T, c.norm_out_b, o + CA_NO_B, 256, 0.f);
        ch_tab_add(T, c.inp_b, o + CA_INP_B, 512, 0.f);
        ch_tab_add(T, c.inorm_out_w, o + CA_INO_W, 256, 1.f); ch_tab_add(T, c.inorm_out_b, o + CA_INO_B, 256, 0.f);
        ch_tab_add(T, c.ig_b, o + CA_IG_B, 256, 0.f);
        ch_tab_add(T, c.inorm_in_w, o + CA_INI_W, 256, 1.f);  ch_tab_add(T, c.inorm_in_b, o + CA_INI_B, 256, 0.f);
        ch_tab_add(T, c.ug_b, o + CA_UG_B, 256, 0.f);
        ch_tab_add(T, c.norm_in_w, o + CA_NI_W, 256, 1.f);    ch_tab_add(T, c.norm_in_b, o + CA_NI_B, 256, 0.f);
        ch_tab_add(T, c.fc_b, o + CA_FC_B, 256, 0.f);
        ch_tab_add(T, c.fc_norm_w, o + CA_FCN_W, 256, 1.f);   ch_tab_add(T, c.fc_norm_b, o + CA_FCN_B, 256, 0.f);
        ch_tab_add(T, c.in_b, o + CA_IN_B, 768, 0.f);
        const float* sc[8] = {mode == 0 ? c.h2_inv[0] : c.h2_inv[1], c.h2_inv[2], c.h2_inv[3], c.h2_inv[4], c.h2_inv[5], c.h2_inv[6], nullptr, nullptr};
        for (int k = 0; k < 8; ++k) ch_tab_add(T, sc[k], o + CA_SC + k, 1, 1.f);
    }
    const int o = 2 * CA_TOTAL;
    ch_tab_add(T, c.out_b, o + CC_OUT_B, 256, 0.f);
    ch_tab_add(T, c.attn_norm_w, o + CC_AN_W, 256, 1.f);  ch_tab_add(T, c.attn_norm_b, o + CC_AN_B, 256, 0.f);
    ch_tab_add(T, c.ffn2_b, o + CC_B2, 256, 0.f);
    ch_tab_add(T, c.ffn_norm_w, o + CC_FN_W, 256, 1.f);   ch_tab_add(T, c.ffn_norm_b, o + CC_FN_B, 256, 0.f);
    ch_tab_add(T, c.cls_ln_w, o + CC_CLN_W, 256, 1.f);    ch_tab_add(T, c.cls_ln_b, o + CC_CLN_B, 256, 0.f);
    ch_tab_add(T, c.mask_ln_w, o + CC_MLN_W, 256, 1.f);   ch_tab_add(T, c.mask_ln_b, o + CC_MLN_B, 256, 0.f);
    ch_tab_add(T, c.dvec, o + CC_DVEC, 256, 0.f);
    ch_tab_add(T, c.fc_cls_b, o + CC_CLS_B, c.fc_cls_b ? c.ncls : 0, 0.f);
    ch_tab_add(T, nullptr, o + CC_CLS_B + (c.fc_cls_b ? c.ncls : 0), 256 - (c.fc_cls_b ? c.ncls : 0), 0.f);
    ch_tab_add(T, c.dec_b, o + CC_DEC_B, 256, 0.f);
    ch_tab_add(T, c.ffn1_b, o + CC_B1, c.ff, 0.f);
    ch_tab_add(T, nullptr, o + CC_B1 + c.ff, 2048 - c.ff, 0.f);
    for (int k = 0; k < 8; ++k) ch_tab_add(T, k < 7 ? c.h2_inv[7 + k] : nullptr, o + CC_SC + k, 1, 1.f);
    if (T.count >= CH_PACK_MAX) return VKN_E_ARG;
    hipLaunchKernelGGL(k_chain_pack, dim3(T.count), dim3(256), 0, stream, T, out);
    VKN_CHECK_LAUNCH();
    return VKN_OK;
}

#else
__global__ __launch_bounds__(256) void k_split_h2(const float* __restrict__ W, _Float16* __restrict__ Wp, int Nout, int K,
                                                  const float* __restrict__ scale) {
    const int kt = blockIdx.x, nt = blockIdx.y;
    _Float16* dst = Wp + ((size_t)nt * gridDim.x + kt) * (CH_WTILE / 2);
    const int row = threadIdx.x, n = nt * 256 + row;
    const float sc = scale[0];
    for (int k = 0; k < 32; ++k) {
        ch_e t[2] = {(ch_e)0.f, (ch_e)0.f};
        if (n < Nout) ch_split(W[(size_t)n * K + kt * 32 + k] * sc, t);
        const int q = k >> 3, e = k & 7;
        dst[((0 * 4 + q) * 256 + row) * 8 + e] = t[0];
        dst[((1 * 4 + q) * 256 + row) * 8 + e] = t[1];
    }
}
size_t vkn_split_h2_bytes(int Nout, int K) { return (size_t)((Nout + 255) / 256) * (size_t)(K / 32) * CH_WTILE; }
int vkn_launch_split_h2(const float* W, void* images, int Nout, int K, const float* scale, hipStream_t stream) {
    if (!W || !images || !scale || Nout <= 0 || K <= 0 || K % 32 != 0) return VKN_E_ARG;
    hipLaunchKernelGGL(k_split_h2, dim3(K / 32, (Nout + 255) / 256), dim3(256), 0, stream, W, static_cast<_Float16*>(images), Nout, K, scale);
    VKN_CHECK_LAUNCH();
    return VKN_OK;
}
#endif

int vkn_launch_chain_a(const VknChainA& p, hipStream_t stream) {
    if (!p.a0 || !p.obj_in || !p.wbase || !p.obj1 || !p.qkv || !p.consts || p.M <= 0 || p.wbytes >= (1ull << 31)) return VKN_E_ARG;
    ChainAArgs A{};
    A.a0 = p.a0; A.obj_in = p.obj_in; A.rowscale = p.rowscale; A.wbase = p.wbase; A.wbytes = (unsigned)p.wbytes;
    A.off_dyn = p.off_dyn; A.off_inp = p.off_inp; A.off_ig = p.off_ig; A.off_ug = p.off_ug; A.off_fc = p.off_fc; A.off_in = p.off_in;
    A.eps = p.eps; A.M = p.M; A.obj1 = p.obj1; A.qkv = p.qkv;
    A.consts = p.consts + (p.rowscale ? 0 : CA_TOTAL);
    A.status = p.status;
#ifdef CH_H2
    const size_t lds = (size_t)2 * CH_IMG * sizeof(ch_e) + (size_t)(2 * CH_SBUF + CA_TOTAL + 16 * CH_THREADS + 64 + 512) * sizeof(float);
#else
    const size_t lds = (size_t)2 * CH_IMG * sizeof(ch_e) + (size_t)(2 * CH_SBUF + CA_TOTAL + 16 * CH_THREADS) * sizeof(float);
#endif
#define CHA_LAUNCH(ABLV)                                                                                            \
    do {                                                                                                            \
        VKN_ALLOW_FULL_LDS(k_chain_a<ABLV>);                                                                        \
        hipLaunchKernelGGL(k_chain_a<ABLV>, dim3((p.M + CH_ROWS - 1) / CH_ROWS), dim3(CH_THREADS), lds, stream, A); \
    } while (0)
#ifdef VKN_DEBUG
    switch (vkn_dbg_env("VKN_CHAIN_ABL", 0)) {
        case 1: CHA_LAUNCH(1); break;
        case 2: CHA_LAUNCH(2); break;
        case 3: CHA_LAUNCH(3); break;
        case 4: CHA_LAUNCH(4); break;
        case 5: CHA_LAUNCH(5); break;
        case 6: CHA_LAUNCH(6); break;
        case 7: CHA_LAUNCH(7); break;
        case 8: CHA_LAUNCH(8); break;
        case 9: CHA_LAUNCH(9); break;
        case 10: CHA_LAUNCH(10); break;
        case 11: CHA_LAUNCH(11); break;
        default: CHA_LAUNCH(0); break;
    }
#else
    CHA_LAUNCH(0);
#endif
#undef CHA_LAUNCH
    VKN_CHECK_LAUNCH();
    return VKN_OK;
}

int vkn_launch_chain_c(const VknChainC& p, hipStream_t stream) {
    if (!p.ao || !p.obj1 || !p.wbase || !p.obj_out || !p.consts || p.M <= 0 || p.wbytes >= (1ull << 31)) return VKN_E_ARG;
    if (p.ff <= 0 || p.ff % 256 != 0 || p.ff > 2048 || p.ncls > 256) return VKN_E_SHAPE;
    if (!p.plane_hi == !p.kern_out || (p.plane_hi && !p.plane_lo)) return VKN_E_ARG;
    ChainCArgs A{};
    A.ao = p.ao; A.obj1 = p.obj1; A.wbase = p.wbase; A.wbytes = (unsigned)p.wbytes;
    A.off_out = p.off_out; A.off_ffn1 = p.off_ffn1; A.off_ffn2 = p.off_ffn2; A.off_clsfc = p.off_clsfc; A.off_maskfc = p.off_maskfc;
    A.off_fccls = p.off_fccls; A.off_dec = p.off_dec;
    A.nchunks = p.ff / 256; A.has_cls = (p.cls_out != nullptr) ? 1 : 0; A.cls_sigmoid = p.cls_sigmoid; A.ncls = p.ncls;
    A.eps = p.eps; A.M = p.M; A.kb0 = p.kb0; A.obj_out = p.obj_out; A.cls_out = p.cls_out; A.kb_out = p.kb_out;
    A.plane_hi = p.plane_hi; A.plane_lo = p.plane_lo; A.kern_out = p.kern_out; A.rows_per_frame = p.rows_per_frame; A.NPT = p.NPT;
    A.consts = p.consts + 2 * CA_TOTAL;
    A.status = p.status;
#ifdef CH_H2
    const size_t lds = (size_t)2 * CH_IMG * sizeof(ch_e) + (size_t)(2 * CH_SBUF + CC_TOTAL + 32) * sizeof(float);
#else
    const size_t lds = (size_t)2 * CH_IMG * sizeof(ch_e) + (size_t)(2 * CH_SBUF + CC_TOTAL) * sizeof(float);
#endif
#define CHC_LAUNCH(ABLV)                                                                                            \
    do {                                                                                                            \
        VKN_ALLOW_FULL_LDS(k_chain_c<ABLV>);                                                                        \
        hipLaunchKernelGGL(k_chain_c<ABLV>, dim3((p.M + CH_ROWS - 1) / CH_ROWS), dim3(CH_THREADS), lds, stream, A); \
    } while (0)
#ifdef VKN_DEBUG
    switch (vkn_dbg_env("VKN_CHAIN_ABL", 0)) {
        case 1: CHC_LAUNCH(1); break;
        case 2: CHC_LAUNCH(2); break;
        case 3: CHC_LAUNCH(3); break;
        case 4: CHC_LAUNCH(4); break;
        case 5: CHC_LAUNCH(5); break;
        case 6: CHC_LAUNCH(6); break;
        case 7: CHC_LAUNCH(7); break;
        case 8: CHC_LAUNCH(8); break;
        case 9: CHC_LAUNCH(9); break;
        case 10: CHC_LAUNCH(10); break;
        case 11: CHC_LAUNCH(11); break;
        default: CHC_LAUNCH(0); break;
    }
#else
    CHC_LAUNCH(0);
#endif
#undef CHC_LAUNCH
    VKN_CHECK_LAUNCH();
    return VKN_OK;
}
```

### video-k-net_amd/csrc/vkn_common.h

```cpp
#pragma once
#include <hip/hip_runtime.h>
#include <stdint.h>

typedef _Float16 half8 __attribute__((ext_vector_type(8)));
typedef _Float16 half4 __attribute__((ext_vector_type(4)));
typedef float f32x16 __attribute__((ext_vector_type(16)));
typedef float f32x4 __attribute__((ext_vector_type(4)));
typedef float f32x2 __attribute__((ext_vector_type(2)));

#define VKN_WAVE 64

#ifdef VKN_DEBUG
#include <stdlib.h>
static inline int vkn_dbg_env(const char* name, int dflt) {
    const char* e = getenv(name);
    return e ? atoi(e) : dflt;
}
#else
#define vkn_dbg_env(name, dflt) (dflt)
#endif
#ifdef VKN_DEBUG
#define VKN_ABL_IS(param, k) ((param) == (k))
#else
#define VKN_ABL_IS(param, k) false
#endif

__device__ __forceinline__ int vkn_cd_row(int r, int lane) { return (r & 3) + 8 * (r >> 2) + 4 * (lane >> 5); }

__device__ __forceinline__ void vkn_split_f16(float v, _Float16& hi, _Float16& lo) {
    hi = (_Float16)v;
    lo = (_Float16)(v - (float)hi);
}

typedef _Float16 vkn_half2 __attribute__((ext_vector_type(2)));
__device__ __forceinline__ void vkn_split_f16x2(float a, float b, vkn_half2& hi, vkn_half2& lo) {
    const f32x2 v = {a, b};
    hi = __builtin_convertvector(v, vkn_half2);
    float r0, r1;
    asm("v_fma_mix_f32 %0, %1, -1.0, %2 op_sel:[0,0,0] op_sel_hi:[1,0,0]" : "=v"(r0) : "v"(hi), "v"(a));
    asm("v_fma_mix_f32 %0, %1, -1.0, %2 op_sel:[1,0,0] op_sel_hi:[1,0,0]" : "=v"(r1) : "v"(hi), "v"(b));
    const f32x2 r = {r0, r1};
    lo = __builtin_convertvector(r, vkn_half2);
}

#define VKN_DPP_STEP(OP, X, CTRL, ROWMASK, IDENT)                                                                            \
    X = OP(X, __uint_as_float((unsigned)__builtin_amdgcn_update_dpp((int)__float_as_uint(IDENT), (int)__float_as_uint(X), CTRL, \
                                                                    ROWMASK, 0xF, false)))
__device__ __forceinline__ float vkn_add_(float a, float b) { return a + b; }
__device__ __forceinline__ float vkn_wave_sum(float v) {
    VKN_DPP_STEP(vkn_add_, v, 0x111, 0xF, 0.f);
    VKN_DPP_STEP(vkn_add_, v, 0x112, 0xF, 0.f);
    VKN_DPP_STEP(vkn_add_, v, 0x114, 0xF, 0.f);
    VKN_DPP_STEP(vkn_add_, v, 0x118, 0xF, 0.f);
    VKN_DPP_STEP(vkn_add_, v, 0x142, 0xA, 0.f);
    VKN_DPP_STEP(vkn_add_, v, 0x143, 0xC, 0.f);
    return __uint_as_float((unsigned)__builtin_amdgcn_readlane((int)__float_as_uint(v), 63));
}
__device__ __forceinline__ float vkn_wave_max(float v) {
    const float ninf = -INFINITY;
    VKN_DPP_STEP(fmaxf, v, 0x111, 0xF, ninf);
    VKN_DPP_STEP(fmaxf, v, 0x112, 0xF, ninf);
    VKN_DPP_STEP(fmaxf, v, 0x114, 0xF, ninf);
    VKN_DPP_STEP(fmaxf, v, 0x118, 0xF, ninf);
    VKN_DPP_STEP(fmaxf, v, 0x142, 0xA, ninf);
    VKN_DPP_STEP(fmaxf, v, 0x143, 0xC, ninf);
    return __uint_as_float((unsigned)__builtin_amdgcn_readlane((int)__float_as_uint(v), 63));
}
#undef VKN_DPP_STEP

#define VKN_OK 0
#define VKN_E_ARG (-1)
#define VKN_E_SHAPE (-2)
#define VKN_E_WORKSPACE (-3)
#define VKN_E_LAUNCH (-4)
#define VKN_E_ALIGN (-5)
#define VKN_E_RANGE (-6)
#ifndef VKN_STATUS_RANGE
#define VKN_STATUS_RANGE 1
#endif

static inline int vkn_allow_full_lds(const void* fn, unsigned long long* done_mask) {
    int dev = 0;
    if (hipGetDevice(&dev) != hipSuccess) return -1;
    const unsigned long long bit = 1ull << (dev & 63);
    if (__atomic_load_n(done_mask, __ATOMIC_ACQUIRE) & bit) return 0;
    hipFuncAttributes fa;
    if (hipFuncGetAttributes(&fa, fn) != hipSuccess) return -1;
    const int dyn = 160 * 1024 - (int)fa.sharedSizeBytes;
    if (hipFuncSetAttribute(fn, hipFuncAttributeMaxDynamicSharedMemorySize, dyn) != hipSuccess) return -1;
    __atomic_fetch_or(done_mask, bit, __ATOMIC_RELEASE);
    return 0;
}
#define VKN_ALLOW_FULL_LDS(fn)                                                        \
    do {                                                                              \
        static unsigned long long lds_done_ = 0;                                      \
        if (vkn_allow_full_lds((const void*)(fn), &lds_done_)) return VKN_E_LAUNCH;   \
    } while (0)

#define VKN_CHECK_LAUNCH()                                  \
    do {                                                    \
        if (hipGetLastError() != hipSuccess) return VKN_E_LAUNCH; \
    } while (0)
```

### video-k-net_amd/csrc/vkn_fused.hip

```cpp
#include "vkn_common.h"
#include "vkn_launch.h"

#define FU_THREADS 256
#define FU_WAVES 4
#define FU_TILE 64

typedef unsigned int fu_u32x2 __attribute__((ext_vector_type(2)));

#ifdef VKN_DEBUG
#include "../../tools/experiments/fused_variants.inc"
#endif

#define FS_THREADS 512
#define FS_TILE 32

#define FS_V_DEFAULT 7
#ifdef VKN_DEBUG
__device__ unsigned long long g_fs_prof[8][8];
#define FS_STAMP(k)                                                     \
    do {                                                                \
        if constexpr ((V & 8) != 0) {                                   \
            const unsigned long long now_ = __builtin_amdgcn_s_memtime(); \
            prof[k] += now_ - tprev;                                    \
            tprev = now_;                                               \
        }                                                               \
    } while (0)
#else
#define FS_STAMP(k) do { } while (0)
#endif
typedef short fs_short4 __attribute__((ext_vector_type(4)));
typedef short fs_short8 __attribute__((ext_vector_type(8)));
#define FS_WRITELANE(wd, val, row) asm volatile("v_writelane_b32 %0, %1, %2" : "+v"(wd) : "s"(val), "n"(row))

#ifdef VKN_DEBUG
#include "../../tools/experiments/fused_older.inc"
#endif

template <int NB, int C, int XH = 0, int PF = 0>
__global__ __launch_bounds__(FS_THREADS, 2) void k_fused_il(const float* __restrict__ x, const _Float16* __restrict__ kfh,
                                                             const _Float16* __restrict__ kfl, const float* __restrict__ kb,
                                                             float thr, float* __restrict__ part, float* __restrict__ cntp,
                                                             int N, int NPT, int n0_in, int P, int NZ) {
    constexpr int KS = C / 16;
    constexpr int NFG = KS / 16, NFD = KS / 4 - NFG, NF = NFD;
    static_assert(KS % 4 == 0 && 4 * (NFD + NFG) == KS, "C must be a multiple of 64");
    constexpr int NCB = C / 32;
    constexpr int CBW = (NCB + 3) / 4;
    constexpr bool ALLDEC = (NB == 4), ALLCB = (NCB % 4) == 0;
    constexpr int LDK = C + 8;
    constexpr int PLANE = FS_TILE * LDK;
    constexpr int IMG = 2 * PLANE;
    constexpr int V = PF ? 8 : 0;

    extern __shared__ __attribute__((aligned(16))) char smem[];
    _Float16* dimg = reinterpret_cast<_Float16*>(smem);
    half8* lut = reinterpret_cast<half8*>(dimg + 3 * IMG);
    unsigned* wbits = reinterpret_cast<unsigned*>(lut + 256);
    float* kbs = reinterpret_cast<float*>(wbits + 256);

    const int b = blockIdx.y, gidx = blockIdx.x / NZ, G = gridDim.x / NZ;
    const int n0 = n0_in + (blockIdx.x - gidx * NZ) * (NB * 32);
    const int tid = threadIdx.x, lane = tid & 63;
    const int wave = __builtin_amdgcn_readfirstlane(tid >> 6);
    const int g = lane >> 5, li = lane & 31;
    unsigned long long prof[8] = {0, 0, 0, 0, 0, 0, 0, 0}, tprev = 0;
    (void)prof; (void)tprev;

    const int nsup = ((P >> 6) - gidx + G - 1) / G;
    const int T = 2 * nsup;
    auto tile_p0 = [&](int t) { return (((t >> 1) * G + gidx) << 6) + ((t & 1) << 5); };

    for (int v = tid; v < 256; v += FS_THREADS) {
        half8 h;
#pragma unroll
        for (int e = 0; e < 8; ++e) h[e] = ((v >> ((e >> 1) + 4 * (e & 1))) & 1) ? (_Float16)1.f : (_Float16)0.f;
        lut[v] = h;
    }
    if (tid < 128) {
        const int n = n0 + tid;
        kbs[tid] = (kb && tid < NB * 32 && n < N) ? kb[(size_t)b * N + n] : 0.f;
        wbits[128 + tid] = 0u;
    }
    for (int v = tid; v < IMG / 8; v += FS_THREADS)
        reinterpret_cast<half8*>(dimg + 2 * IMG)[v] = half8{0, 0, 0, 0, 0, 0, 0, 0};

    const __amdgpu_buffer_rsrc_t xrs =
        XH ? __builtin_amdgcn_make_buffer_rsrc(const_cast<unsigned short*>(reinterpret_cast<const unsigned short*>(x) + (size_t)b * C * P), 0,
                                               C * P * 2, 0x00020000)
           : __builtin_amdgcn_make_buffer_rsrc(const_cast<float*>(x + (size_t)b * C * P), 0, C * P * 4, 0x00020000);
    const int lq = lane >> 4, lp = lane & 15;
    constexpr int XSH = XH ? 1 : 2;
    const int voff = (((lq << 2) * P + 2 * lp) << XSH);
    fu_u32x2 raw[2][NF][4];
    auto frag_ks = [&](int f) { return wave < 4 ? wave + 4 * f : 4 * NFD + (wave - 4) + 4 * f; };
    auto issue = [&](int slot, int t, int f) {
        const int ks = frag_ks(f);
        {
            const int soff = ((ks << 4) * P + tile_p0(t)) << XSH;
#pragma unroll
            for (int e = 0; e < 4; ++e) {
                if (XH) raw[slot][f][e] = fu_u32x2{__builtin_amdgcn_raw_buffer_load_b32(xrs, voff, soff + ((e * P) << 1), 0), 0u};
                else raw[slot][f][e] = __builtin_amdgcn_raw_buffer_load_b64(xrs, voff, soff + ((e * P) << 2), 3);
            }
        }
    };
    auto commit = [&](int slot, int buf, int f) {
        const int ks = frag_ks(f);
        {
            half4 h0, l0, h1, l1;
#pragma unroll
            for (int e = 0; e < 4; ++e) {
                const unsigned u0 = raw[slot][f][e][0], u1 = raw[slot][f][e][1];
                _Float16 h, l;
                if (XH == 1) {
                    h0[e] = __builtin_bit_cast(_Float16, (unsigned short)(u0 & 0xFFFFu));
                    h1[e] = __builtin_bit_cast(_Float16, (unsigned short)(u0 >> 16));
                } else if (XH == 2) {
                    h0[e] = (_Float16)__uint_as_float(u0 << 16);
                    h1[e] = (_Float16)__uint_as_float(u0 & 0xFFFF0000u);
                } else {
                    vkn_split_f16(__uint_as_float(u0), h, l);
                    h0[e] = h;
                    l0[e] = l;
                    vkn_split_f16(__uint_as_float(u1), h, l);
                    h1[e] = h;
// ... 225 lines not shown
            for (int nb = 0; nb < NB; ++nb) {
                const unsigned wv = wbits[wb * 128 + nb * 32 + li];
#pragma unroll
                for (int ps = 0; ps < 2; ++ps)
                    a[ps][nb] = lut[((wv >> (8 * ps + 4 * g)) & 0xFu) | (((wv >> (16 + 8 * ps + 4 * g)) & 0xFu) << 4)];
            }
            ldf(0, 0, dh);
            if (NSTEP > 1) ldf(1, 1, dh);
        };
        auto gather = [&](int t) {
            const _Float16* dh = dimg + (size_t)(t % 3) * IMG;
#pragma unroll
            for (int st = 0; st < NSTEP; ++st) {
                if (st + 2 < NSTEP) ldf((st + 2) % 3, st + 2, dh);
                const int j = st >> 1, ps = st & 1, cb = gw + 4 * j;
                if (ALLCB || cb < NCB) {
#pragma unroll
                    for (int nb = 0; nb < NB; ++nb) {
                        accg[j][nb] = __builtin_amdgcn_mfma_f32_32x32x16_f16(a[ps][nb], fbh[st % 3], accg[j][nb], 0, 0, 0);
                        if (!XH) accg[j][nb] = __builtin_amdgcn_mfma_f32_32x32x16_f16(a[ps][nb], fbl[st % 3], accg[j][nb], 0, 0, 0);
                    }
                }
            }
        };
#ifdef VKN_DEBUG
        if constexpr (PF != 0) tprev = __builtin_amdgcn_s_memtime();
#endif
        for (int i0 = 0; i0 < T; i0 += 2) {
#pragma unroll
            for (int u = 0; u < 2; ++u) {
                const int i = i0 + u;
                prep((i + 2) % 3, (i + 1) & 1);
                {
                    const _Float16* dh = dimg + (size_t)((i + 2) % 3) * IMG;
                    constexpr int NUNIT = 2 * NFG * 4, NCH = NSTEP * (XH ? 1 : 2);
                    int ch = 0;
#pragma unroll
                    for (int st = 0; st < NSTEP; ++st) {
                        if (st + 2 < NSTEP) ldf((st + 2) % 3, st + 2, dh);
                        const int j = st >> 1, ps = st & 1, cb = gw + 4 * j;
#pragma unroll
                        for (int pl = 0; pl < (XH ? 1 : 2); ++pl) {
                            if (ALLCB || cb < NCB) {
#pragma unroll
                                for (int nb = 0; nb < NB; ++nb)
                                    accg[j][nb] = __builtin_amdgcn_mfma_f32_32x32x16_f16(a[ps][nb], pl ? fbl[st % 3] : fbh[st % 3], accg[j][nb], 0, 0, 0);
                            }
#pragma unroll
                            for (int uu = (ch * NUNIT) / NCH; uu < ((ch + 1) * NUNIT) / NCH; ++uu) loader_unit(NFG, u ^ 1, (i + 1) % 3, min(i + 3, tlast), uu);
                            ++ch;
                            __builtin_amdgcn_sched_barrier(0);
                        }
                    }
                }
                __builtin_amdgcn_sched_barrier(0);
                FS_STAMP(4);
                __syncthreads();
                FS_STAMP(5);
            }
        }
        if (T >= 1) {
            prep((T - 1) % 3, (T - 1) & 1);
            gather(T - 1);
        }
#ifdef VKN_DEBUG
        if constexpr (PF != 0)
            if (lane == 0 && blockIdx.x == 0 && blockIdx.y == 0)
                for (int k = 0; k < 8; ++k) g_fs_prof[wave][k] = prof[k];
#endif
#pragma unroll
        for (int j = 0; j < CBW; ++j) {
            const int cb = gw + 4 * j;
            if (cb < NCB) {
#pragma unroll
                for (int nb = 0; nb < NB; ++nb)
#pragma unroll
                    for (int r = 0; r < 16; ++r) {
                        const int n = n0 + nb * 32 + vkn_cd_row(r, lane);
                        if (n < NPT) pp[(size_t)n * C + cb * 32 + li] = accg[j][nb][r];
                    }
            }
        }
    }
}

#ifdef VKN_DEBUG
#include "../../tools/experiments/fused_w4.inc"
#endif


#ifdef VKN_DEBUG
static size_t fusedw4_lds_bytes(int C) { return (size_t)4 * 2 * FS_TILE * (C + 8) * sizeof(_Float16) + 256 * 16 + 256 * 4 + 128 * 4; }
#endif
static size_t fuseds_lds_bytes(int C) { return (size_t)3 * 2 * FS_TILE * (C + 8) * sizeof(_Float16) + 256 * 16 + 256 * 4 + 128 * 4; }

#ifdef VKN_DEBUG
static size_t fused_lds_bytes(int C) { return (size_t)4 * FU_TILE * (C + 8) * sizeof(_Float16) + 256 * 16 + 256 * 4 + 128 * 4; }
static size_t fused8_lds_bytes(int C) {
    return (size_t)(2 * FU_TILE + 128) * (C + 8) * sizeof(_Float16) + 256 * 16 + 256 * 4 + 128 * 4 + 128 * 4;
}
#endif

int vkn_fused_supported(int C, int P) {
    return (C == 64 || C == 128 || C == 256) && (P % 64) == 0 && (size_t)C * P * 4 < ((size_t)1 << 31);
}

int vkn_launch_fused_decode_gather(const float* x, const _Float16* kfh, const _Float16* kfl, const float* kb, float thr,
                                   float* xraw, float* cnt, float* part, float* cntp, int B, int N, int C, int P,
                                   hipStream_t stream, int xdt, int* status, const void* touch, size_t touch_bytes) {
    if (B <= 0 || N <= 0 || P <= 0 || xdt < 0 || xdt > 2) return VKN_E_ARG;
    if (!vkn_fused_supported(C, P)) return VKN_E_SHAPE;
    const int NPT = (N + 31) / 32 * 32;
    const int G = vkn_gather_groups(B, P);
#ifdef VKN_DEBUG
    const int variant = vkn_dbg_env("VKN_FUSED", 10);
    const bool eight = variant == 1;
    const size_t lds = variant >= 2 ? fuseds_lds_bytes(C) : (eight ? fused8_lds_bytes(C) : fused_lds_bytes(C));
#else
    const size_t lds = fuseds_lds_bytes(C);
#endif
#ifdef VKN_DEBUG
    const bool one_pass = (variant >= 10 && variant <= 19) && !vkn_dbg_env("VKN_FUSED_CHUNK_LOOP", 0);
#else
    const bool one_pass = true;
#endif
    const int NZ = one_pass ? (NPT + 127) / 128 : 1;
    const int nb_one = (NPT / 32 + NZ - 1) / NZ;
    for (int n0 = 0; n0 < (one_pass ? 1 : NPT); n0 += 128) {
        const int nb = one_pass ? nb_one : ((NPT - n0 >= 128) ? 4 : (NPT - n0) / 32);
        dim3 grid(G * NZ, B, 1);
#ifdef VKN_DEBUG
#define FU_LAUNCH_XV(NBV, CV, XHV, VV)                                                                                         \
    do {                                                                                                                       \
        VKN_ALLOW_FULL_LDS((k_fused_dgs<NBV, CV, XHV, VV>));                                                                   \
        hipLaunchKernelGGL((k_fused_dgs<NBV, CV, XHV, VV>), grid, dim3(FS_THREADS), lds, stream, x, kfh, kfl, kb, thr, part,   \
                           cntp, N, NPT, n0, P);                                                                               \
    } while (0)
#define FU_LAUNCH_PQ(NBV, CV, XHV, PFV)                                                                                        \
    do {                                                                                                                       \
        VKN_ALLOW_FULL_LDS((k_fused_pq<NBV, CV, XHV, PFV>));                                                                   \
        hipLaunchKernelGGL((k_fused_pq<NBV, CV, XHV, PFV>), grid, dim3(FS_THREADS), fusedq_lds_bytes(C), stream, x, kfh, kfl,  \
                           kb, thr, part, cntp, N, NPT, n0, P);                                                                \
    } while (0)
#endif
#define FU_LAUNCH_IL(NBV, CV, XHV, PFV)                                                                                        \
    do {                                                                                                                       \
        VKN_ALLOW_FULL_LDS((k_fused_il<NBV, CV, XHV, PFV>));                                                                   \
        hipLaunchKernelGGL((k_fused_il<NBV, CV, XHV, PFV>), grid, dim3(FS_THREADS), lds, stream, x, kfh, kfl, kb, thr, part,   \
                           cntp, N, NPT, n0, P, NZ);                                                                           \
    } while (0)
#ifdef VKN_DEBUG
#define FU_LAUNCH_W4(NBV, CV, XHV, PFV)                                                                                        \
    do {                                                                                                                       \
        VKN_ALLOW_FULL_LDS((k_fused_w4<NBV, CV, XHV, PFV>));                                                                   \
        hipLaunchKernelGGL((k_fused_w4<NBV, CV, XHV, PFV>), grid, dim3(W4_THREADS), fusedw4_lds_bytes(C), stream, x, kfh, kfl,  \
                           kb, thr, part, cntp, N, NPT, n0, P, NZ);                                                            \
    } while (0)
#endif
#ifdef VKN_DEBUG
#define FU_LAUNCH_PP(NBV, CV, XHV, PFV)                                                                                        \
    do {                                                                                                                       \
        VKN_ALLOW_FULL_LDS((k_fused_pp<NBV, CV, XHV, PFV>));                                                                   \
        hipLaunchKernelGGL((k_fused_pp<NBV, CV, XHV, PFV>), grid, dim3(FS_THREADS), lds, stream, x, kfh, kfl, kb, thr, part,   \
                           cntp, N, NPT, n0, P);                                                                               \
    } while (0)
#endif
#ifdef VKN_DEBUG
#define FU_LAUNCH_X(NBV, CV, XHV)                                                          \
    do {                                                                                   \
        const int vv = vkn_dbg_env("VKN_FUSED_V", FS_V_DEFAULT);                           \
        const bool cfg2 = NBV == 4 && CV == 256 && XHV == 0;                               \
        if (variant == 4 && cfg2) FU_LAUNCH_PP(4, 256, 0, 1);                              \
        else if (variant == 6 && cfg2) FU_LAUNCH_PQ(4, 256, 0, 1);                         \
        else if (variant == 7 && cfg2) FU_LAUNCH_PQ(4, 256, 0, 2);                         \
        else if (variant == 8 && cfg2) FU_LAUNCH_PQ(4, 256, 0, 3);                         \
        else if (variant == 9 && cfg2) FU_LAUNCH_PQ(4, 256, 0, 4);                         \
        else if (variant == 3) FU_LAUNCH_PP(NBV, CV, XHV, 0);                              \
        else if (variant == 10) FU_LAUNCH_IL(NBV, CV, XHV, 0);                             \
        else if (variant == 12) FU_LAUNCH_W4(NBV, CV, XHV, 0);                             \
        else if (variant == 13 && cfg2) FU_LAUNCH_W4(4, 256, 0, 1);                        \
        else if (variant == 14 && cfg2) FU_LAUNCH_W4(4, 256, 0, 2);                        \
        else if (variant == 15 && cfg2) FU_LAUNCH_W4(4, 256, 0, 3);                        \
        else if (variant == 16 && cfg2) FU_LAUNCH_W4(4, 256, 0, 4);                        \
        else if (variant == 11 && cfg2) FU_LAUNCH_IL(4, 256, 0, 1);                        \
        else if (variant == 17 && cfg2) FU_LAUNCH_IL(4, 256, 0, 2);                        \
        else if (variant == 18 && cfg2) FU_LAUNCH_IL(4, 256, 0, 3);                        \
        else if (variant == 19 && cfg2) FU_LAUNCH_IL(4, 256, 0, 4);                        \
        else if (variant == 5) FU_LAUNCH_PQ(NBV, CV, XHV, 0);                              \
        else if (cfg2 && vv != FS_V_DEFAULT) {                                             \
            switch (vv) {                                                                  \
                case 0: FU_LAUNCH_XV(4, 256, 0, 0); break;                                 \
                case 1: FU_LAUNCH_XV(4, 256, 0, 1); break;                                 \
                case 2: FU_LAUNCH_XV(4, 256, 0, 2); break;                                 \
                case 3: FU_LAUNCH_XV(4, 256, 0, 3); break;                                 \
                case 4: FU_LAUNCH_XV(4, 256, 0, 4); break;                                 \
                case 5: FU_LAUNCH_XV(4, 256, 0, 5); break;                                 \
                case 15: FU_LAUNCH_XV(4, 256, 0, 15); break;                               \
                default: FU_LAUNCH_XV(4, 256, 0, 6); break;                                \
            }                                                                              \
        } else FU_LAUNCH_XV(NBV, CV, XHV, FS_V_DEFAULT);                                   \
    } while (0)
#else
#define FU_LAUNCH_X(NBV, CV, XHV) FU_LAUNCH_IL(NBV, CV, XHV, 0)
#endif
#define FU_LAUNCH_S(NBV, CV)                        \
    do {                                            \
        if (xdt == 1) FU_LAUNCH_X(NBV, CV, 1);      \
        else if (xdt == 2) FU_LAUNCH_X(NBV, CV, 2); \
        else FU_LAUNCH_X(NBV, CV, 0);               \
    } while (0)
#ifdef VKN_DEBUG
#define FU_LAUNCH(NBV, CV)                                                                                                     \
    do {                                                                                                                       \
        if (variant >= 2 || xdt != 0) FU_LAUNCH_S(NBV, CV);                                                                    \
        else if (eight) {                                                                                                      \
            VKN_ALLOW_FULL_LDS((k_fused_dg8<NBV, CV>));                                                                        \
            hipLaunchKernelGGL((k_fused_dg8<NBV, CV>), grid, dim3(FU8_THREADS), lds, stream, x, kfh, kfl, kb, thr, part, cntp, \
                               N, NPT, n0, P);                                                                                 \
        } else {                                                                                                               \
            VKN_ALLOW_FULL_LDS((k_fused_dg<NBV, CV>));                                                                         \
            hipLaunchKernelGGL((k_fused_dg<NBV, CV>), grid, dim3(FU_THREADS), lds, stream, x, kfh, kfl, kb, thr, part, cntp,   \
                               N, NPT, n0, P);                                                                                 \
        }                                                                                                                      \
    } while (0)
#else
#define FU_LAUNCH(NBV, CV) FU_LAUNCH_S(NBV, CV)
#endif
#define FU_CASE(NBV)                               \
    case NBV:                                      \
        if (C == 256) FU_LAUNCH(NBV, 256);         \
        else if (C == 128) FU_LAUNCH(NBV, 128);    \
        else FU_LAUNCH(NBV, 64);                   \
        break;
        switch (nb) {
            FU_CASE(1)
            FU_CASE(2)
            FU_CASE(3)
            FU_CASE(4)
            default:
                return VKN_E_SHAPE;
        }
#undef FU_CASE
#undef FU_LAUNCH
#undef FU_LAUNCH_S
#undef FU_LAUNCH_X
#undef FU_LAUNCH_IL
#ifdef VKN_DEBUG
#undef FU_LAUNCH_XV
#undef FU_LAUNCH_PP
#undef FU_LAUNCH_PQ
#undef FU_LAUNCH_W4
#endif
        VKN_CHECK_LAUNCH();
    }
    return vkn_launch_gather_reduce(part, cntp, xraw, cnt, B, N, C, G, stream, status, touch, touch_bytes);
}

#ifdef VKN_DEBUG
extern "C" int vkn_dbg_fused_prof(unsigned long long* out64) {
    return hipMemcpyFromSymbol(out64, HIP_SYMBOL(g_fs_prof), sizeof(unsigned long long) * 64) == hipSuccess ? 0 : -4;
}
#endif
```

### video-k-net_amd/csrc/vkn_gather.hip

```cpp
#include "vkn_common.h"
#include "vkn_launch.h"

#define GA_THREADS 512
#define GA_WAVES 8
#define GA_PT 32
#define GA_LDR 40

template <int NB, int BITS, int XH = 0>
__global__ __launch_bounds__(GA_THREADS, 2) void k_gather_mfma(const float* __restrict__ x,
                                                               const float* __restrict__ masks, float thr,
                                                               float* __restrict__ part, float* __restrict__ cntp, int N,
                                                               int NPT, int n0, int C, int P, int px_per_wg,
                                                               long long mask_fs, int ileave, int x_alias) {
    extern __shared__ __attribute__((aligned(16))) char smem[];
    constexpr bool REAL = (BITS == 2 || BITS == 3);
    static_assert(!(XH && REAL), "half-storage x: binary operands only");
    constexpr int XCH = XH ? 2 : 4;
    const int rows_buf = 2 * C + (REAL ? 2 : 1) * NB * 32;
    _Float16* lds = reinterpret_cast<_Float16*>(smem);

    const int b = blockIdx.y, gidx = blockIdx.x, G = gridDim.x;
    const int tid = threadIdx.x, lane = tid & 63;
    const int wave = __builtin_amdgcn_readfirstlane(tid >> 6);
    const int g = lane >> 5, li = lane & 31;

    const int p_begin = ileave ? 0 : gidx * px_per_wg;
    const int p_end = ileave ? 0 : min(P, p_begin + px_per_wg);
    const int nsup_i = ileave ? (((P >> 6) - gidx + G - 1) / G) : 0;
    const int ntiles = ileave ? 2 * nsup_i : ((p_end > p_begin) ? (p_end - p_begin + GA_PT - 1) / GA_PT : 0);
    auto tile_p0 = [&](int t) { return ileave ? ((((t >> 1) * G + gidx) << 6) + ((t & 1) << 5)) : p_begin + t * GA_PT; };

    const float* xb = x + (size_t)b * C * P;
    const unsigned short* xb16 = reinterpret_cast<const unsigned short*>(x) + (size_t)b * C * P;
    const float* mb = masks + (size_t)b * mask_fs;
    const unsigned* wb = reinterpret_cast<const unsigned*>(masks) + (size_t)b * (P >> 5) * NPT + n0;
    const bool vec_ok = ((P & 3) == 0);
    half8* lut = reinterpret_cast<half8*>(lds + (size_t)2 * rows_buf * GA_LDR);
    if (BITS == 1) {
        for (int v = tid; v < 256; v += GA_THREADS) {
            half8 h;
#pragma unroll
            for (int e = 0; e < 8; ++e) h[e] = ((v >> ((e >> 1) + 4 * (e & 1))) & 1) ? (_Float16)1.f : (_Float16)0.f;
            lut[v] = h;
        }
    }

    const int nxch = XH ? C * 4 : C * 8;
    const int nmch = NB * 32 * 8;
    f32x4 xrA[4], xrB[4];
    f32x4 mrA[2], mrB[2];

    const float off_v = (BITS == 2) ? 0.f : -INFINITY;
    const f32x4 neg_inf = {off_v, off_v, off_v, off_v};

    auto issue = [&](int t, f32x4 (&xr)[4], f32x4 (&mr)[2]) {
        const int p0 = tile_p0(t);
#pragma unroll
        for (int i = 0; i < XCH; ++i) {
            const int idc = min(tid + i * GA_THREADS, nxch - 1);
            if (XH)
                xr[i] = *reinterpret_cast<const f32x4*>(xb16 + (size_t)(idc >> 2) * P + p0 + ((idc & 3) << 3));
            else if (BITS == 2 && x_alias >= 0) {
                const int ch = idc >> 3;
                xr[i] = *reinterpret_cast<const f32x4*>(xb + (size_t)(ch >= x_alias ? ch - x_alias : ch) * P + p0 + ((idc & 7) << 2));
            } else
                xr[i] = __builtin_nontemporal_load(reinterpret_cast<const f32x4*>(xb + (size_t)(idc >> 3) * P + p0 + ((idc & 7) << 2)));
        }
        if (BITS == 1) {
            const unsigned* wp = wb + (size_t)((p0 >> 6) << 1) * NPT + min(tid, NB * 32 - 1);
            const unsigned we = wp[0], wo = wp[NPT];
            mr[0][0] = __uint_as_float(we);
            mr[0][1] = __uint_as_float(wo);
        } else {
#pragma unroll
            for (int i = 0; i < 2; ++i) {
                const int idc = min(tid + i * GA_THREADS, nmch - 1);
                const int n = min(n0 + (idc >> 3), N - 1);
                mr[i] = *reinterpret_cast<const f32x4*>(mb + (size_t)n * P + p0 + ((idc & 7) << 2));
            }
        }
    };

    auto issue_slow = [&](int t, f32x4 (&xr)[4], f32x4 (&mr)[2]) {
        const int p0 = tile_p0(t);
#pragma unroll
        for (int i = 0; i < 4; ++i) {
            const int idx = tid + i * GA_THREADS;
            f32x4 v = {0.f, 0.f, 0.f, 0.f};
            if (idx < nxch) {
                const int p = p0 + ((idx & 7) << 2);
                const int ch = idx >> 3;
                const float* src = xb + (size_t)((BITS == 2 && x_alias >= 0 && ch >= x_alias) ? ch - x_alias : ch) * P + p;
#pragma unroll
                for (int k = 0; k < 4; ++k)
                    if (p + k < p_end) v[k] = src[k];
            }
// ... 116 lines not shown
        for (int ks = 0; ks < 2; ++ks) {
            const int off = (ks << 4) + (g << 3);
            const int bsh = 16 * odd32 + 8 * ks + 4 * g;
            if (has_cb) {
                const half8 bh = *reinterpret_cast<const half8*>(xh + (wave * 32 + li) * GA_LDR + off);
                const half8 bl = *reinterpret_cast<const half8*>(xl + (wave * 32 + li) * GA_LDR + off);
#pragma unroll
                for (int nb = 0; nb < NB; ++nb) {
                    half8 a;
                    if (BITS == 1) {
                        const unsigned we = reinterpret_cast<const unsigned*>(mk)[nb * 32 + li];
                        const unsigned wo = reinterpret_cast<const unsigned*>(mk)[NB * 32 + nb * 32 + li];
                        a = lut[((we >> bsh) & 0xFu) | (((wo >> bsh) & 0xFu) << 4)];
                    } else {
                        a = *reinterpret_cast<const half8*>(mk + (nb * 32 + li) * GA_LDR + off);
                    }
                    acc[nb] = __builtin_amdgcn_mfma_f32_32x32x16_f16(a, bh, acc[nb], 0, 0, 0);
                    if (!XH) acc[nb] = __builtin_amdgcn_mfma_f32_32x32x16_f16(a, bl, acc[nb], 0, 0, 0);
                    if (REAL) {
                        const half8 al = *reinterpret_cast<const half8*>(mk + (NB * 32 + nb * 32 + li) * GA_LDR + off);
                        acc[nb] = __builtin_amdgcn_mfma_f32_32x32x16_f16(al, bh, acc[nb], 0, 0, 0);
                    }
                }
            }
            if (has_cnt) {
                half8 a;
                if (BITS == 1) {
                    const unsigned we = reinterpret_cast<const unsigned*>(mk)[wave * 32 + li];
                    const unsigned wo = reinterpret_cast<const unsigned*>(mk)[NB * 32 + wave * 32 + li];
                    a = lut[((we >> bsh) & 0xFu) | (((wo >> bsh) & 0xFu) << 4)];
                } else {
                    a = *reinterpret_cast<const half8*>(mk + (wave * 32 + li) * GA_LDR + off);
                }
                accc = __builtin_amdgcn_mfma_f32_32x32x16_f16(a, ones, accc, 0, 0, 0);
                if (REAL) {
                    const half8 al = *reinterpret_cast<const half8*>(mk + (NB * 32 + wave * 32 + li) * GA_LDR + off);
                    accc = __builtin_amdgcn_mfma_f32_32x32x16_f16(al, ones, accc, 0, 0, 0);
                }
            }
        }
    };

    const int nfull = ileave ? ntiles : (vec_ok ? (p_end - p_begin) / GA_PT : 0);
    if (nfull > 0) {
        issue(0, xrA, mrA);
        issue(min(1, nfull - 1), xrB, mrB);
        commit(0, xrA, mrA);
        __syncthreads();
        for (int t = 0; t < nfull; t += 2) {
            issue(min(t + 2, nfull - 1), xrA, mrA);
            compute(0, (tile_p0(t) >> 5) & 1);
            if (t + 1 < nfull) commit(1, xrB, mrB);
            __syncthreads();
            if (t + 1 >= nfull) break;
            issue(min(t + 3, nfull - 1), xrB, mrB);
            compute(1, (tile_p0(t + 1) >> 5) & 1);
            if (t + 2 < nfull) commit(0, xrA, mrA);
            __syncthreads();
        }
    }
    for (int t = nfull; t < ntiles; ++t) {
        issue_slow(t, xrA, mrA);
        commit(0, xrA, mrA);
        __syncthreads();
        compute(0, 0);
        __syncthreads();
    }

    float* pp = part + ((size_t)b * G + gidx) * NPT * C;
    if (has_cb) {
#pragma unroll
        for (int nb = 0; nb < NB; ++nb)
#pragma unroll
            for (int r = 0; r < 16; ++r) {
                const int n = n0 + nb * 32 + vkn_cd_row(r, lane);
                pp[(size_t)n * C + wave * 32 + li] = acc[nb][r];
            }
    }
    if (has_cnt && li == 0) {
        float* cp = cntp + ((size_t)b * G + gidx) * NPT;
#pragma unroll
        for (int r = 0; r < 16; ++r) cp[n0 + wave * 32 + vkn_cd_row(r, lane)] = accc[r];
    }
}

template <int NB>
__global__ __launch_bounds__(GA_THREADS, 2) void k_gather_bits_w(const float* __restrict__ x, const unsigned* __restrict__ bits,
                                                                  float* __restrict__ part, float* __restrict__ cntp, int N,
                                                                  int NPT, int n0, int C, int P, int px_per_wg, int ileave) {
    extern __shared__ __attribute__((aligned(16))) char smem[];
    constexpr int WTILE = 2 * 32 * GA_LDR;
    const int b = blockIdx.y, gidx = blockIdx.x, G = gridDim.x;
    const int tid = threadIdx.x, lane = tid & 63;
    const int wave = __builtin_amdgcn_readfirstlane(tid >> 6);
    const int g = lane >> 5, li = lane & 31;
    _Float16* wl = reinterpret_cast<_Float16*>(smem) + (size_t)wave * 2 * WTILE;
    half8* lut = reinterpret_cast<half8*>(reinterpret_cast<_Float16*>(smem) + (size_t)GA_WAVES * 2 * WTILE);
    for (int v = tid; v < 256; v += GA_THREADS) {
        half8 h;
#pragma unroll
        for (int e = 0; e < 8; ++e) h[e] = ((v >> ((e >> 1) + 4 * (e & 1))) & 1) ? (_Float16)1.f : (_Float16)0.f;
        lut[v] = h;
    }
    __syncthreads();

    const int p_begin = gidx * px_per_wg;
    const int p_end = min(P, p_begin + px_per_wg);
    const int nsup = ileave ? (((P >> 6) - gidx + G - 1) / G)
                            : ((p_end > p_begin) ? (p_end - p_begin) >> 6 : 0);
    auto sup_p0 = [&](int s) { return ileave ? ((s * G + gidx) << 6) : p_begin + (s << 6); };
    const bool has_cb = (wave * 32 < C);
    const bool has_cnt = (wave < NB);

    f32x16 acc[NB];
#pragma unroll
    for (int nb = 0; nb < NB; ++nb)
#pragma unroll
        for (int r = 0; r < 16; ++r) acc[nb][r] = 0.f;
    unsigned cnt_i = 0;

    if (has_cb && nsup > 0) {
        const float* xw = x + ((size_t)b * C + wave * 32) * P;
        const unsigned* wb = bits + (size_t)b * (P >> 5) * NPT + n0 + li;
        const int lrow = lane >> 3, lchk = lane & 7;
        f32x4 xa[8], xb[8];
        unsigned wa[2 * NB], wv[2 * NB];

        auto issue = [&](int s, f32x4 (&xr)[8], unsigned (&wr)[2 * NB]) {
            const int p0 = sup_p0(s);
#pragma unroll
            for (int h = 0; h < 2; ++h)
#pragma unroll
                for (int i = 0; i < 4; ++i)
                    xr[h * 4 + i] = __builtin_nontemporal_load(
                        reinterpret_cast<const f32x4*>(xw + (size_t)(lrow + 8 * i) * P + p0 + 32 * h + (lchk << 2)));
            const unsigned* wp = wb + (size_t)((p0 >> 6) << 1) * NPT;
#pragma unroll
            for (int nb = 0; nb < NB; ++nb) {
                wr[nb] = wp[nb * 32];
                wr[NB + nb] = wp[NPT + nb * 32];
            }
        };
        auto commit = [&](const f32x4 (&xr)[8]) {
#pragma unroll
            for (int h = 0; h < 2; ++h) {
                _Float16* xh = wl + h * WTILE;
                _Float16* xl = xh + 32 * GA_LDR;
#pragma unroll
                for (int i = 0; i < 4; ++i) {
                    half4 hh, ll;
#pragma unroll
                    for (int k = 0; k < 4; ++k) {
                        _Float16 a, c2;
                        vkn_split_f16(xr[h * 4 + i][k], a, c2);
                        hh[k] = a;
                        ll[k] = c2;
                    }
                    const int off = (lrow + 8 * i) * GA_LDR + (lchk << 2);
                    *reinterpret_cast<half4*>(xh + off) = hh;
                    *reinterpret_cast<half4*>(xl + off) = ll;
                }
            }
        };
        auto compute = [&](const unsigned (&wr)[2 * NB]) {
#pragma unroll
            for (int h = 0; h < 2; ++h) {
                const _Float16* xh = wl + h * WTILE;
                const _Float16* xl = xh + 32 * GA_LDR;
#pragma unroll
                for (int ks = 0; ks < 2; ++ks) {
                    const int off = (ks << 4) + (g << 3);
                    const int bsh = 16 * h + 8 * ks + 4 * g;
                    const half8 bh = *reinterpret_cast<const half8*>(xh + li * GA_LDR + off);
                    const half8 bl = *reinterpret_cast<const half8*>(xl + li * GA_LDR + off);
#pragma unroll
                    for (int nb = 0; nb < NB; ++nb) {
                        const half8 a = lut[((wr[nb] >> bsh) & 0xFu) | (((wr[NB + nb] >> bsh) & 0xFu) << 4)];
                        acc[nb] = __builtin_amdgcn_mfma_f32_32x32x16_f16(a, bh, acc[nb], 0, 0, 0);
                        acc[nb] = __builtin_amdgcn_mfma_f32_32x32x16_f16(a, bl, acc[nb], 0, 0, 0);
                    }
                }
            }
        };
        auto lds_fence = [&]() {
            __builtin_amdgcn_s_waitcnt(0xc07f);
            __builtin_amdgcn_wave_barrier();
        };

        const int last = nsup - 1;
        issue(0, xa, wa);
        for (int s = 0; s < nsup; s += 2) {
            issue(min(s + 1, last), xb, wv);
            commit(xa);
            lds_fence();
            compute(wa);
            lds_fence();
            if (s + 1 >= nsup) break;
            issue(min(s + 2, last), xa, wa);
            commit(xb);
            lds_fence();
            compute(wv);
            lds_fence();
        }
    }

    if (has_cnt) {
        const unsigned* wc = bits + (size_t)b * (P >> 5) * NPT + n0 + wave * 32 + li;
        for (int s2 = 0; s2 < nsup; ++s2) {
            const unsigned* wp = wc + (size_t)((sup_p0(s2) >> 6) << 1) * NPT;
            cnt_i += __popc(wp[0]) + __popc(wp[NPT]);
        }
    }

    float* pp = part + ((size_t)b * G + gidx) * NPT * C;
    if (has_cb) {
#pragma unroll
        for (int nb = 0; nb < NB; ++nb)
#pragma unroll
            for (int r = 0; r < 16; ++r) {
                const int n = n0 + nb * 32 + vkn_cd_row(r, lane);
                pp[(size_t)n * C + wave * 32 + li] = acc[nb][r];
            }
    }
    if (has_cnt && g == 0) cntp[((size_t)b * G + gidx) * NPT + n0 + wave * 32 + li] = (float)cnt_i;
}

__global__ __launch_bounds__(256) void k_gather_reduce(const float* __restrict__ part, const float* __restrict__ cntp,
                                                        float* __restrict__ xraw, float* __restrict__ cnt, int N, int NPT,
                                                        int C, int G, int* __restrict__ status, const char* __restrict__ touch,
                                                        unsigned touch_bytes) {
    if (touch) {
        const unsigned per = (touch_bytes / gridDim.x + 15u) & ~15u;
        const unsigned t0 = blockIdx.x * per, t1 = min(t0 + per, touch_bytes & ~15u);
        for (unsigned o = t0 + threadIdx.x * 16u; o < t1; o += 256u * 16u) {
            const f32x4 v = *reinterpret_cast<const f32x4*>(touch + o);
            asm volatile("" ::"v"(v));
        }
    }
    __shared__ f32x4 comb[3][64];
    const int row = blockIdx.x;
    const int b = row / N, n = row - b * N;
    const int lane = threadIdx.x & 63;
    const int k = __builtin_amdgcn_readfirstlane(threadIdx.x >> 6);
    const size_t gstride = (size_t)NPT * C;
    const float* pp = part + ((size_t)b * G * NPT + n) * C;
    const int G4 = G & ~3;
    for (int c0 = 0; c0 < C; c0 += 256) {
        const int c4 = c0 + lane * 4;
        const bool ok = c4 < C;
        const float* pc = pp + (ok ? c4 : 0);
        f32x4 s = {0.f, 0.f, 0.f, 0.f};
        int gi = k;
        for (; gi + 28 < G4; gi += 32) {
            f32x4 v[8];
#pragma unroll
            for (int u = 0; u < 8; ++u) v[u] = *reinterpret_cast<const f32x4*>(pc + (size_t)(gi + 4 * u) * gstride);
#pragma unroll
            for (int u = 0; u < 8; ++u) s += v[u];
        }
        for (; gi < G4; gi += 4) s += *reinterpret_cast<const f32x4*>(pc + (size_t)gi * gstride);
        if (k == 0)
            for (gi = G4; gi < G; ++gi) s += *reinterpret_cast<const f32x4*>(pc + (size_t)gi * gstride);
        if (c0) __syncthreads();
        if (k) comb[k - 1][lane] = s;
        __syncthreads();
        if (k == 0 && ok) {
            const f32x4 r = (s + comb[0][lane]) + (comb[1][lane] + comb[2][lane]);
            *reinterpret_cast<f32x4*>(xraw + (size_t)row * C + c4) = r;
            if (status && !(fabsf(r[0]) <= 3.0e38f && fabsf(r[1]) <= 3.0e38f && fabsf(r[2]) <= 3.0e38f && fabsf(r[3]) <= 3.0e38f))
                atomicOr(status, 1);
        }
    }
    if (k == 1) {
        const float* cp = cntp + (size_t)b * G * NPT + n;
        float s = 0.f;
        for (int gi = lane; gi < G; gi += 64) s += cp[(size_t)gi * NPT];
        s = vkn_wave_sum(s);
        if (lane == 0) cnt[row] = s;
    }
}

__global__ __launch_bounds__(256) void k_gather_ref(const float* __restrict__ x, const float* __restrict__ masks,
                                                    float thr, float* __restrict__ xraw, float* __restrict__ cnt, int N,
                                                    int C, int P, long long mask_fs) {
    const int n = blockIdx.x, b = blockIdx.y;
    const float* mp = masks + (size_t)b * mask_fs + (size_t)n * P;
    for (int c = threadIdx.x; c < C; c += 256) {
        const float* xp = x + ((size_t)b * C + c) * P;
        float s = 0.f;
        for (int p = 0; p < P; ++p)
            if (mp[p] >= thr) s += xp[p];
        xraw[((size_t)b * N + n) * C + c] = s;
    }
    if (threadIdx.x == 0) {
        float s = 0.f;
        for (int p = 0; p < P; ++p)
            if (mp[p] >= thr) s += 1.f;
        cnt[(size_t)b * N + n] = s;
    }
}

int vkn_launch_gather_reduce(const float* part, const float* cntp, float* xraw, float* cnt, int B, int N, int C, int G,
                             hipStream_t stream, int* status, const void* touch, size_t touch_bytes) {
    if (touch_bytes >= (1ull << 31)) touch = nullptr;
    hipLaunchKernelGGL(k_gather_reduce, dim3(B * N), dim3(256), 0, stream, part, cntp, xraw, cnt, N, (N + 31) / 32 * 32, C, G, status,
                       static_cast<const char*>(touch), (unsigned)touch_bytes);
    VKN_CHECK_LAUNCH();
    return VKN_OK;
}

int vkn_gather_groups(int B, int P) {
    int wg_per_frame = 256 / (B > 0 ? B : 1);
    if (wg_per_frame < 1) wg_per_frame = 1;
    int px_per_wg = (P + wg_per_frame - 1) / wg_per_frame;
    px_per_wg = (px_per_wg + GA_PT - 1) / GA_PT * GA_PT;
    return (P + px_per_wg - 1) / px_per_wg;
}

int vkn_launch_gather(const float* x, const float* masks, float thr, float* xraw, float* cnt, float* part, float* cntp,
                      int B, int N, int C, int P, hipStream_t stream, int xdt, int* status, const void* touch, size_t touch_bytes) {
    return vkn_launch_gather_ex(x, masks, thr, xraw, cnt, part, cntp, B, N, C, P, N, stream, xdt, status, touch, touch_bytes);
}

static int gather_launch(const float* x, const float* masks, float thr, float* xraw, float* cnt, float* part, float* cntp, int B,
                         int N, int C, int P, int mask_rows, int bits, hipStream_t stream, int xdt = 0, int* status = nullptr,
                         const void* touch = nullptr, size_t touch_bytes = 0, int x_alias = -1);

int vkn_launch_gather_ex(const float* x, const float* masks, float thr, float* xraw, float* cnt, float* part, float* cntp,
                         int B, int N, int C, int P, int mask_rows, hipStream_t stream, int xdt, int* status, const void* touch,
                         size_t touch_bytes) {
    return gather_launch(x, masks, thr, xraw, cnt, part, cntp, B, N, C, P, mask_rows, 0, stream, xdt, status, touch, touch_bytes);
}

int vkn_launch_gather_real(const float* x, const float* a, float* xraw, float* cnt, float* part, float* cntp, int B, int N, int C,
                           int P, int mask_rows, hipStream_t stream, int x_alias, float x_floor) {
    if (x_alias > C || (x_alias > 0 && (C - x_alias > x_alias || B != 1))) return VKN_E_ARG;
    return gather_launch(x, a, x_alias >= 0 ? x_floor : 0.f, xraw, cnt, part, cntp, B, N, C, P, mask_rows, 2, stream, 0, nullptr, nullptr, 0,
                         x_alias);
}

int vkn_launch_gather_soft(const float* x, const float* masks, float thr, float* xraw, float* cnt, float* part, float* cntp, int B,
                           int N, int C, int P, int mask_rows, hipStream_t stream) {
    return gather_launch(x, masks, thr, xraw, cnt, part, cntp, B, N, C, P, mask_rows, 3, stream);
}

int vkn_launch_gather_bits(const float* x, const unsigned* bits, float* xraw, float* cnt, float* part, float* cntp, int B, int N,
                           int C, int P, hipStream_t stream, int xdt, int* status, const void* touch, size_t touch_bytes) {
    if ((P % 64) != 0) return VKN_E_SHAPE;
    return gather_launch(x, reinterpret_cast<const float*>(bits), 0.f, xraw, cnt, part, cntp, B, N, C, P, N, 1, stream, xdt, status, touch,
                         touch_bytes);
}

static int gather_launch(const float* x, const float* masks, float thr, float* xraw, float* cnt, float* part, float* cntp, int B,
                         int N, int C, int P, int mask_rows, int bits, hipStream_t stream, int xdt, int* status, const void* touch,
                         size_t touch_bytes, int x_alias) {
    if (x_alias >= 0 && bits != 2) return VKN_E_ARG;
    if (B <= 0 || N <= 0 || P <= 0 || mask_rows < N) return VKN_E_ARG;
    if (xdt < 0 || xdt > 2) return VKN_E_ARG;
    if (xdt && (bits >= 2 || (P % 64) != 0)) return VKN_E_SHAPE;
    const long long mask_fs = (long long)mask_rows * P;
    if (C % 32 != 0 || C > 256) return VKN_E_SHAPE;
    const int NPT = (N + 31) / 32 * 32;
    int wg_per_frame = 256 / B;
    if (wg_per_frame < 1) wg_per_frame = 1;
    int px_per_wg = (P + wg_per_frame - 1) / wg_per_frame;
    px_per_wg = (px_per_wg + GA_PT - 1) / GA_PT * GA_PT;
    const int G = (P + px_per_wg - 1) / px_per_wg;
    const int ileave = ((P % 64) == 0 && vkn_dbg_env("VKN_GATHER_ILEAVE", 1) != 0) ? 1 : 0;
    const bool wave_indep = bits == 1 && xdt == 0 && vkn_dbg_env("VKN_GATHER_BITS_W", 1) != 0 && (C % 32) == 0 &&
                            (px_per_wg % 64) == 0;
    for (int n0 = 0; n0 < NPT; n0 += 128) {
        const int nb = (NPT - n0 >= 128) ? 4 : (NPT - n0) / 32;
        dim3 grid(G, B, 1), block(GA_THREADS);
        if (wave_indep) {
            const size_t ldsw = (size_t)GA_WAVES * 2 * 2 * 32 * GA_LDR * sizeof(_Float16) + 4096;
            const unsigned* bw = reinterpret_cast<const unsigned*>(masks);
#define GA_WLAUNCH(NBV)                                                                                              \
    case NBV:                                                                                                        \
        VKN_ALLOW_FULL_LDS(k_gather_bits_w<NBV>);                                                                    \
        hipLaunchKernelGGL(k_gather_bits_w<NBV>, grid, block, ldsw, stream, x, bw, part, cntp, N, NPT, n0, C, P, px_per_wg, ileave); \
        break;
            switch (nb) {
                GA_WLAUNCH(1)
                GA_WLAUNCH(2)
                GA_WLAUNCH(3)
                GA_WLAUNCH(4)
                default:
                    return VKN_E_SHAPE;
            }
#undef GA_WLAUNCH
            VKN_CHECK_LAUNCH();
            continue;
        }
        const size_t lds = (size_t)2 * (2 * C + (bits >= 2 ? 2 : 1) * nb * 32) * GA_LDR * sizeof(_Float16) + (bits == 1 ? 4096 : 0);
#define GA_LAUNCH(NBV, BV, XHV)                                                                                  \
    do {                                                                                                         \
        VKN_ALLOW_FULL_LDS((k_gather_mfma<NBV, BV, XHV>));                                                       \
        hipLaunchKernelGGL((k_gather_mfma<NBV, BV, XHV>), grid, block, lds, stream, x, masks, thr, part, cntp, N, NPT, n0, C, P, \
                           px_per_wg, mask_fs, ileave, x_alias);                                                 \
    } while (0)
#define GA_CASE(NBV)                                 \
    case NBV:                                        \
        if (bits == 3) GA_LAUNCH(NBV, 3, 0);         \
        else if (bits == 2) GA_LAUNCH(NBV, 2, 0);    \
        else if (bits && xdt == 1) GA_LAUNCH(NBV, 1, 1); \
        else if (bits && xdt == 2) GA_LAUNCH(NBV, 1, 2); \
        else if (bits) GA_LAUNCH(NBV, 1, 0);         \
        else if (xdt == 1) GA_LAUNCH(NBV, 0, 1);     \
        else if (xdt == 2) GA_LAUNCH(NBV, 0, 2);     \
        else GA_LAUNCH(NBV, 0, 0);                   \
        break;
        switch (nb) {
            GA_CASE(1)
            GA_CASE(2)
            GA_CASE(3)
            GA_CASE(4)
            default:
                return VKN_E_SHAPE;
        }
#undef GA_CASE
#undef GA_LAUNCH
        VKN_CHECK_LAUNCH();
    }
    hipLaunchKernelGGL(k_gather_reduce, dim3(B * N), dim3(256), 0, stream, part, cntp, xraw, cnt, N, NPT, C, G, status,
                       static_cast<const char*>(touch), (unsigned)(touch_bytes < (1ull << 31) ? touch_bytes : 0));
    VKN_CHECK_LAUNCH();
    return VKN_OK;
}

int vkn_launch_gather_ref(const float* x, const float* masks, float thr, float* xraw, float* cnt, int B, int N, int C,
                          int P, hipStream_t stream) {
    return vkn_launch_gather_ref_ex(x, masks, thr, xraw, cnt, B, N, C, P, N, stream);
}

int vkn_launch_gather_ref_ex(const float* x, const float* masks, float thr, float* xraw, float* cnt, int B, int N, int C,
                             int P, int mask_rows, hipStream_t stream) {
    if (mask_rows < N) return VKN_E_ARG;
    hipLaunchKernelGGL(k_gather_ref, dim3(N, B), dim3(256), 0, stream, x, masks, thr, xraw, cnt, N, C, P,
                       (long long)mask_rows * P);
    VKN_CHECK_LAUNCH();
    return VKN_OK;
}
```

### video-k-net_amd/csrc/vkn_launch.h

```cpp
#pragma once
#include <hip/hip_runtime.h>
#include <stddef.h>

struct VknEpi {
    const float* bias;
    const float* rowscale;
    const float* bias2;
    const float* resid;
    int ldr;
    const float* ln_w;
    const float* ln_b;
    int ln_from_col;
    float eps;
    int act;
    float* out;
    int ldo;
    const float* dot_vec;
    const float* dot_bias;
    float* dot_out;
    _Float16* plane_hi;
    _Float16* plane_lo;
    int rows_per_frame;
    int NPT;
};

struct VknGemmProb {
    const float* A;
    const float* A2;
    const float* A3;
    const float* A4;
    int lda;
    const float* W;
    const void* Wsplit;
    int Nout;
    VknEpi epi;
};

int vkn_gather_groups(int B, int P);
int vkn_launch_gather_ex(const float* x, const float* masks, float thr, float* xraw, float* cnt, float* part, float* cntp,
                         int B, int N, int C, int P, int mask_rows, hipStream_t stream, int xdt = 0, int* status = nullptr,
                         const void* touch = nullptr, size_t touch_bytes = 0);
int vkn_launch_gather_ref_ex(const float* x, const float* masks, float thr, float* xraw, float* cnt, int B, int N, int C,
                             int P, int mask_rows, hipStream_t stream);
int vkn_launch_gather_real(const float* x, const float* a, float* xraw, float* cnt, float* part, float* cntp, int B, int N, int C,
                           int P, int mask_rows, hipStream_t stream, int x_alias = -1, float x_floor = 0.f);
int vkn_launch_gather_soft(const float* x, const float* masks, float thr, float* xraw, float* cnt, float* part, float* cntp, int B,
                           int N, int C, int P, int mask_rows, hipStream_t stream);
int vkn_launch_gather_bits(const float* x, const unsigned* bits, float* xraw, float* cnt, float* part, float* cntp, int B, int N,
                           int C, int P, hipStream_t stream, int xdt = 0, int* status = nullptr, const void* touch = nullptr,
                           size_t touch_bytes = 0);
int vkn_launch_gather_reduce(const float* part, const float* cntp, float* xraw, float* cnt, int B, int N, int C, int G,
                             hipStream_t stream, int* status = nullptr, const void* touch = nullptr, size_t touch_bytes = 0);
int vkn_fused_supported(int C, int P);
int vkn_launch_fused_decode_gather(const float* x, const _Float16* kfh, const _Float16* kfl, const float* kb, float thr,
                                   float* xraw, float* cnt, float* part, float* cntp, int B, int N, int C, int P,
                                   hipStream_t stream, int xdt = 0, int* status = nullptr, const void* touch = nullptr,
                                   size_t touch_bytes = 0);
int vkn_launch_gather(const float* x, const float* masks, float thr, float* xraw, float* cnt, float* part, float* cntp,
                      int B, int N, int C, int P, hipStream_t stream, int xdt = 0, int* status = nullptr, const void* touch = nullptr,
                      size_t touch_bytes = 0);
int vkn_launch_gather_ref(const float* x, const float* masks, float thr, float* xraw, float* cnt, int B, int N, int C,
                          int P, hipStream_t stream);
struct VknDecodeStrides {
    long long plane;
    long long kb;
    long long out;
};
int vkn_launch_decode_ex(const float* x, const _Float16* kfh, const _Float16* kfl, const float* kb, float* out, int B, int N,
                         int C, int P, int shared, int out_rows, hipStream_t stream, int xdt = 0, const float* oscale = nullptr);
int vkn_launch_decode_ref_ex(const float* x, const float* kern, const float* kb, float* out, int B, int N, int C, int P,
                             int shared, int out_rows, hipStream_t stream);
int vkn_launch_decode_bits(const float* x, const _Float16* kfh, const _Float16* kfl, const float* kb, unsigned* bits_out,
                           float thr, int B, int N, int C, int P, hipStream_t stream, int xdt = 0);
int vkn_launch_decode(const float* x, const _Float16* kfh, const _Float16* kfl, const float* kb, float* out, int B, int N,
                      int C, int P, hipStream_t stream, int xdt = 0);
int vkn_launch_decode_ref(const float* x, const float* kern, const float* kb, float* out, int B, int N, int C, int P,
                          hipStream_t stream);
int vkn_launch_split_planes(const float* kern, _Float16* kfh, _Float16* kfl, int B, int N, int C, hipStream_t stream);
int vkn_launch_gemm(const float* A, const float* A2, int lda, const float* W, const void* Wsplit, int M, int K, int Nout,
                    int ksplit, float* partial, const VknEpi& epi, hipStream_t stream);
int vkn_launch_gemm_group(const VknGemmProb* probs, int nprob, int M, int K, int ksplit, float* partial, hipStream_t stream);
size_t vkn_split_w3_bytes(int Nout, int K);
int vkn_launch_add2(const float* a, const float* b, float* out, size_t n, hipStream_t st);
int vkn_launch_add2_half(const void* a, const void* b, void* out, size_t n, int xdt, hipStream_t st);
int vkn_launch_add_rows(const float* a, const float* pos, float* out, size_t rows, int C, int period, hipStream_t st);
struct InitPassArgs {
    const float *loc, *sem;
    const _Float16 *kh, *kl;
    const float* seg_b;
    float *x_out, *masks, *seg;
    unsigned* bits;
    float thr;
    int Np, ncls, nth, cat, N, C, P, px_per_wg;
    int npt;
};
int vkn_init_pass_supported(int Np, int ncls, int C, int P);
int vkn_launch_init_pass(const InitPassArgs& a, int B, hipStream_t st);
int vkn_launch_init_finish(const float* init_w, const float* obj, const float* seg_w, float* out, int B, int Np, int N, int nth,
                           int C, hipStream_t st);
int vkn_launch_ffn_fused(const float* X, int ldx, const void* W1s, const float* b1, const void* W2s, int M, int C, int FF, int HS,
                         float* partial, const VknEpi& epi2, hipStream_t stream);
int vkn_launch_transpose(const float* src, float* dst, int R, int Cc, hipStream_t st);
int vkn_launch_split_w3(const float* W, void* Wp, int Nout, int K, hipStream_t stream);
int vkn_launch_split_w3_t(const float* W, void* Wp, int Nout, int K, hipStream_t stream);
int vkn_launch_ku_mix(const float* params, const float* inputf, const float* ig, const float* ug, const float* no_w,
                      const float* no_b, const float* ino_w, const float* ino_b, float eps, float* f, int M, int C,
                      hipStream_t stream);
int vkn_launch_attn(const float* Q, int ldq, const float* K, const float* V, int ldkv, float* out, int ldo, int B, int Nq,
                    int Nk, int heads, int hd, hipStream_t stream);
int vkn_launch_upsample(const float* in, float* out, int planes, int H, int W, int S, hipStream_t stream, int out_f16 = 0);

struct VknPanopticCfg;
size_t vkn_panoptic_ws_bytes(int B, int K, int Ho, int Wo);
int vkn_launch_panoptic_joint(const VknPanopticCfg* c, const float* cls, const float* masks, int B, int N, int ncls,
                              int* panoptic_seg, int* info, int* nseg, int* bbox, void* ws, size_t ws_bytes, hipStream_t st);

struct VknChainConsts {
    const float *bcnt, *dyn_b;
    const float *norm_out_w, *norm_out_b, *inp_b, *inorm_out_w, *inorm_out_b;
    const float *ig_b, *inorm_in_w, *inorm_in_b, *ug_b, *norm_in_w, *norm_in_b;
    const float *fc_b, *fc_norm_w, *fc_norm_b, *in_b;
    const float *out_b, *attn_norm_w, *attn_norm_b, *ffn1_b, *ffn2_b, *ffn_norm_w, *ffn_norm_b;
    const float *cls_ln_w, *cls_ln_b, *mask_ln_w, *mask_ln_b, *dvec, *fc_cls_b, *dec_b;
    int ff, ncls;
    const float* h2_inv[14];
};
enum { VKN_H2_DYNFT = 0, VKN_H2_DYN, VKN_H2_INP, VKN_H2_IG, VKN_H2_UG, VKN_H2_FC, VKN_H2_IN, VKN_H2_OUT, VKN_H2_FFN1, VKN_H2_FFN2,
       VKN_H2_CLSFC, VKN_H2_MASKFC, VKN_H2_FCCLS, VKN_H2_DEC, VKN_H2_COUNT };
size_t vkn_chain_consts_floats();
int vkn_chain_pack_consts(const VknChainConsts& c, float* out, hipStream_t stream);
struct VknChainA {
    const float* a0;
    const float* obj_in;
    const float* rowscale;
    const void* wbase;
    size_t wbytes;
    unsigned off_dyn, off_inp, off_ig, off_ug, off_fc, off_in;
    const float* consts;
    float eps;
    int M;
    float* obj1;
    float* qkv;
    int* status;
};
struct VknChainC {
    const float* ao;
    const float* obj1;
    const void* wbase;
    size_t wbytes;
    unsigned off_out, off_ffn1, off_ffn2, off_clsfc, off_maskfc, off_fccls, off_dec;
    const float* consts;
    const float* kb0;
    int ff, ncls, cls_sigmoid;
    float eps;
    int M;
    float* obj_out;
    float* cls_out;
    float* kb_out;
    _Float16 *plane_hi, *plane_lo;
    float* kern_out;
    int rows_per_frame, NPT;
    int* status;
};
int vkn_launch_gemm_t3(const VknGemmProb* probs, int nprob, int M, int K, hipStream_t stream);
int vkn_launch_chain_a(const VknChainA& p, hipStream_t stream);
int vkn_launch_chain_c(const VknChainC& p, hipStream_t stream);
int vkn_launch_chain_a_h2(const VknChainA& p, hipStream_t stream);
int vkn_launch_chain_c_h2(const VknChainC& p, hipStream_t stream);
size_t vkn_split_h2_bytes(int Nout, int K);
int vkn_launch_split_h2(const float* W, void* images, int Nout, int K, const float* scale, hipStream_t stream);

struct VknKsPro {
    const float* a[4];
    int lda[4];
    int nsum;
    long long sum_stride;
    const float* pbias;
    const float* presid;
    int ldr;
    const float* ln_w[4];
    const float* ln_b[4];
    float eps;
    int act;
    float* side_out;
    int ld_side;
    const float* dot_vec;
    const float* dot_bias;
    float* dot_out;
};
struct VknKsEpi {
    const float* bias;
    const float* rowscale;
    const float* bias2;
    const float* resid;
    int ldr;
    int act;
    float* out;
    int ldo;
    _Float16* plane_hi;
    _Float16* plane_lo;
    int rows_per_frame, NPT;
};
struct VknKsProb {
    VknKsPro pro;
    const void* Wsplit;
    int Nout;
    int KT;
    VknKsEpi epi;
};
int vkn_launch_rowepi(const float* partial, int ks, int M, int Nout, const VknEpi& epi, hipStream_t stream);
int vkn_launch_gemm_ks(const VknKsProb* probs, int nprob, int mode, int zchunks, int kpw, long long out_zstride, int M, hipStream_t stream);
```

### video-k-net_amd/ops.py

```python
import ctypes
import struct
import threading

import torch

from . import _lib
from ._lib import VknDims, VknStageWeights, check

_H = _lib.CONSTS
FLAG_REF_KERNELS = _H['VKN_FLAG_REF_KERNELS']
FLAG_EXACT_GEMM = _H['VKN_FLAG_EXACT_GEMM']
FLAG_LOGITS_HANDOFF = _H['VKN_FLAG_LOGITS_HANDOFF']
FLAG_BITS_HANDOFF = _H['VKN_FLAG_BITS_HANDOFF']
FLAG_CHAIN_LAUNCHES = _H['VKN_FLAG_CHAIN_LAUNCHES']
FLAG_CHAIN_PERSISTENT = _H['VKN_FLAG_CHAIN_PERSISTENT']
FLAG_JOIN_EARLY = _H['VKN_FLAG_JOIN_EARLY']
FLAG_SCALED_F16 = _H['VKN_FLAG_SCALED_F16']
FLAG_CHAIN_BF16X3 = _H['VKN_FLAG_CHAIN_BF16X3']
FLAG_INIT_SEPARATE = _H['VKN_FLAG_INIT_SEPARATE']
FLAG_CHAIN_KSPLIT = _H['VKN_FLAG_CHAIN_KSPLIT']
FLAG_SERIAL_LINK = _H['VKN_FLAG_SERIAL_LINK']

_tls = threading.local()


def _ptr(t):
    return ctypes.c_void_p(t.data_ptr()) if t is not None else ctypes.c_void_p(0)


def _stream():
    return ctypes.c_void_p(torch.cuda.current_stream().cuda_stream)


def _req(t, name):
    if not torch.is_tensor(t) or not t.is_cuda:
        raise _lib.VknLibraryError(f'{name}: expected a CUDA/HIP tensor — the MI355X path has no CPU fallback')
    if t.dtype != torch.float32:
        raise TypeError(f'{name}: expected float32, got {t.dtype}')
    t = t.contiguous()
    if t.data_ptr() % 16:
        t = t.clone(memory_format=torch.contiguous_format)
    return t


_X_DTYPES = {torch.float32: _H['VKN_X_F32'], torch.float16: _H['VKN_X_F16'], torch.bfloat16: _H['VKN_X_BF16']}
FLAG_X_F16, FLAG_X_BF16 = _H['VKN_FLAG_X_F16'], _H['VKN_FLAG_X_BF16']


def _req_x(t, name='x'):
    if not torch.is_tensor(t) or not t.is_cuda:
        raise _lib.VknLibraryError(f'{name}: expected a CUDA/HIP tensor — the MI355X path has no CPU fallback')
    if t.dtype not in _X_DTYPES:
        raise TypeError(f'{name}: expected float32, float16 or bfloat16, got {t.dtype}')
    t = t.contiguous()
    if t.data_ptr() % 16:
        t = t.clone(memory_format=torch.contiguous_format)
    return t, _X_DTYPES[t.dtype]


def _workspace(nbytes, device, scratch=False):
    cache = getattr(_tls, 'ws', None)
    if cache is None:
        cache = _tls.ws = {}
    key = (device, torch.cuda.current_stream(device).cuda_stream)
    buf = cache.get(key)
    need = int(nbytes) + 256
    if buf is None or buf.numel() < need:
        old = buf
        buf = torch.empty(max(need, 512), dtype=torch.uint8, device=device)
        if old is None:
            buf[:256].zero_()
        else:
            buf[:256].copy_(old[:256])
        cache[key] = buf
        gen = getattr(_tls, 'ws_gen', None)
        if gen is None:
            gen = _tls.ws_gen = {}
        gen[key] = gen.get(key, 0) + 1
    return buf[256:] if scratch else buf


def workspace_generation(device):
    gen = getattr(_tls, 'ws_gen', None) or {}
    return gen.get((device, torch.cuda.current_stream(device).cuda_stream), 0)


def workspace_status(device=None):
    device = torch.device(device if device is not None else torch.cuda.current_device())
    if device.index is None:
        device = torch.device('cuda', torch.cuda.current_device())
    cache = getattr(_tls, 'ws', None) or {}
    buf = cache.get((device, torch.cuda.current_stream(device).cuda_stream))
    if buf is None:
        return
    with torch.cuda.device(device):
        check(_lib.lib().vkn_workspace_status(_ptr(buf), buf.numel(), _stream()))


_THR_CACHE = {}


def thr_logit(hard_mask_thr=0.5):
    key = float(hard_mask_thr)
    if key in _THR_CACHE:
# ... 1101 lines not shown
```

Measured before the change: 10010 frames/s.

## Fold gather partial reduction into chain kernel and skip unused intermediate cls head

When the next stage runs the persistent chain kernel, the gather no longer launches its separate reduce kernel. The chain A kernel instead sums the per-group partials and counts directly while loading its input tile. Intermediate stages also skip the classification FC/LN path by default, because their class logits are never consumed; a CLS_ALL_STAGES flag restores the old behaviour. This saves a launch plus a write and re-read of xraw per stage and cuts GEMM work, at the cost of more complex chain-kernel loading and extra template variants.

New measurement: 10090 frames/s, median of 5. No clear change (+0.8%).

```diff
diff --git a/include/vkn.h b/include/vkn.h
--- a/include/vkn.h
+++ b/include/vkn.h
@@ -38,6 +38,8 @@
 #define VKN_FLAG_CLIP_LINK 8u
 
 #define VKN_FLAG_INIT_SEPARATE 131072u
+#define VKN_FLAG_REDUCE_SEPARATE 262144u
+#define VKN_FLAG_CLS_ALL_STAGES 524288u
 #define VKN_FLAG_PHASE_A 1024u
 #define VKN_FLAG_PHASE_B 2048u
 #define VKN_FLAG_PHASE_C 4096u
diff --git a/video-k-net_amd/csrc/vkn_api.hip b/video-k-net_amd/csrc/vkn_api.hip
--- a/video-k-net_amd/csrc/vkn_api.hip
+++ b/video-k-net_amd/csrc/vkn_api.hip
@@ -65,6 +65,8 @@
     bool keep_xfeat = false;
     const void* touch_next = nullptr;
     size_t touch_next_bytes = 0;
+    bool next_folds = false;
+    bool partials_in = false;
 };
 
 struct PrepW {
@@ -384,11 +386,14 @@
 }
 
 int run_gather(const VknDims* d, const float* x, const float* masks, const unsigned* bits, const StageWs& s, unsigned flags,
-               hipStream_t st, const void* touch = nullptr, size_t touch_bytes = 0) {
+               hipStream_t st, const void* touch = nullptr, size_t touch_bytes = 0, bool keep_partials = false) {
     const int B = d->B, N = d->N, C = d->C, P = d->H * d->W, xdt = xdt_of(flags);
-    if (flags & VKN_FLAG_REF_KERNELS) return vkn_launch_gather_ref(x, masks, d->thr_logit, s.xraw, s.cnt, B, N, C, P, st);
-    if (bits) return vkn_launch_gather_bits(x, bits, s.xraw, s.cnt, s.part, s.cntp, B, N, C, P, st, xdt, s.status, touch, touch_bytes);
-    return vkn_launch_gather(x, masks, d->thr_logit, s.xraw, s.cnt, s.part, s.cntp, B, N, C, P, st, xdt, s.status, touch, touch_bytes);
+    if (flags & VKN_FLAG_REF_KERNELS)
+        return keep_partials ? VKN_E_ARG : vkn_launch_gather_ref(x, masks, d->thr_logit, s.xraw, s.cnt, B, N, C, P, st);
+    if (bits)
+        return vkn_launch_gather_bits(x, bits, s.xraw, s.cnt, s.part, s.cntp, B, N, C, P, st, xdt, s.status, touch, touch_bytes, keep_partials);
+    return vkn_launch_gather(x, masks, d->thr_logit, s.xraw, s.cnt, s.part, s.cntp, B, N, C, P, st, xdt, s.status, touch, touch_bytes,
+                             keep_partials);
 }
 
 int final_decode(const VknDims* d, const float* x, const StageWs& s, const float* kb, float* masks_out, unsigned flags,
@@ -442,10 +447,15 @@
 
 int run_chain_fast(const VknDims* d, const VknStageWeights* w, const PrepW& pw, const float* a0, bool a0_raw, const float* cnt,
                    const float* obj_in, float* obj_out, float* cls_logits, bool cls_sigmoid, float* kern32_out, const StageWs& s,
-                   hipStream_t st, bool h2 = false) {
+                   hipStream_t st, bool h2 = false, bool fold = false) {
     const int M = d->B * d->N, C = d->C;
     VknChainA a{};
     a.a0 = a0; a.obj_in = obj_in; a.rowscale = a0_raw ? cnt : nullptr;
+    if (fold) {
+        if (!a0_raw) return VKN_E_ARG;
+        a.a0 = nullptr; a.rowscale = nullptr;
+        a.part = s.part; a.cntp = s.cntp; a.G = vkn_gather_groups(d->B, d->H * d->W); a.N = d->N; a.NPT = npt_of(d->N);
+    }
     a.wbase = w->prepared; a.wbytes = w->prepared_bytes;
     if (h2) {
         a.off_dyn = pw_off(w, pw.h2[a0_raw ? VKN_H2_DYNFT : VKN_H2_DYN]);
@@ -559,7 +569,12 @@
     pr[0].pro.side_out = obj_out; pr[0].pro.ld_side = C;
     pr[0].epi.out = s.lkv; pr[0].epi.ldo = 2 * C;
     pr[1].Wsplit = pw.mask_fc[0]; pr[1].epi.out = s.lkv + C; pr[1].epi.ldo = 2 * C;
-    VKN_TRY(vkn_launch_gemm_ks(pr, 2, 0, 0, 1, 0, M, st));
+    if (cls_logits) {
+        VKN_TRY(vkn_launch_gemm_ks(pr, 2, 0, 0, 1, 0, M, st));
+    } else {
+        pr[1].pro.side_out = obj_out; pr[1].pro.ld_side = C;
+        VKN_TRY(vkn_launch_gemm_ks(pr + 1, 1, 0, 0, 1, 0, M, st));
+    }
     if (obj_ready && hipEventRecord(obj_ready, st) != hipSuccess) return VKN_E_LAUNCH;
     int np = 0;
     if (cls_logits) {
@@ -628,9 +643,20 @@
     if (ref_decode) return vkn_launch_decode_ref(c.x, kern32, kb, c.masks_out, B, N, C, P, st);
     if (c.to == TO_GATHER)
         return vkn_launch_fused_decode_gather(c.x, s.kfh, s.kfl, kb, d->thr_logit, s.xraw, s.cnt, s.part, s.cntp, B, N, C, P, st, xdt, s.status,
-                                              touch, touch_bytes);
+                                              touch, touch_bytes, c.next_folds ? 1 : 0);
     if (c.to == TO_BITS) return vkn_launch_decode_bits(c.x, s.kfh, s.kfl, kb, c.bits_out, d->thr_logit, B, N, C, P, st, xdt);
     return final_decode(d, c.x, s, kb, c.masks_out, flags, st, c.prof0, c.prof1, c.up_out, c.up_stride, c.up_chunk, c.up_done);
+}
+
+#define VKN_FOLD_MAX_GROUPS 16
+inline bool fold_shape_ok(const VknDims* d, unsigned flags) {
+    return !(flags & (VKN_FLAG_REDUCE_SEPARATE | VKN_FLAG_REF_KERNELS)) && vkn_gather_groups(d->B, d->H * d->W) <= VKN_FOLD_MAX_GROUPS;
+}
+bool fold_ok(const VknDims* d, const VknStageWeights* w, unsigned flags, bool have_cls, bool need_xfeat) {
+    if (need_xfeat || !fold_shape_ok(d, flags)) return false;
+    PrepW pw;
+    if (carve_pw(d, w, flags, &pw) != VKN_OK || !pw.dynft) return false;
+    return !chain_ks_ok(d, w, pw, flags, have_cls) && chain_fast_ok(d, w, pw, flags, have_cls);
 }
 
 int run_stage(const VknDims* d, const StageCall& c, const StageWs& s, unsigned flags, hipStream_t st) {
@@ -654,9 +680,12 @@
     const bool will_fast = !given_xfeat && persistent && vkn_dbg_env("VKN_CHAIN_TOUCH", 1);
     const void* touch_nx = vkn_dbg_env("VKN_CHAIN_TOUCH", 1) ? c.touch_next : nullptr;
     const size_t touch_nx_bytes = touch_nx ? c.touch_next_bytes : 0;
-    if (c.from == FROM_LOGITS || c.from == FROM_BITS)
+    const bool own_gather = c.from == FROM_LOGITS || c.from == FROM_BITS;
+    const bool fold = own_gather ? (persistent && !fewrow && !need_xfeat && !c.x_feat_out && has_ft && fold_shape_ok(d, flags)) : c.partials_in;
+    if (fold && (c.from == FROM_XFEAT || !persistent || fewrow || need_xfeat || c.x_feat_out || !has_ft)) return VKN_E_ARG;
+    if (own_gather)
         VKN_TRY(run_gather(d, c.x, c.masks_in, c.from == FROM_BITS ? c.bits_in : nullptr, s, flags, st, will_fast ? w->prepared : nullptr,
-                           will_fast ? w->prepared_bytes : 0));
+                           will_fast ? w->prepared_bytes : 0, fold));
 
     float* xfeat = c.x_feat_out ? c.x_feat_out : s.xfeat;
     VknEpi e = mk_epi(d);
@@ -689,7 +718,7 @@
             VKN_TRY(run_chain_ks(d, w, pw, raw ? s.xraw : xfeat, raw, s.cnt, obj_in, c.obj_out, cls_logits, c.cls_sigmoid, kern32, s, st, c.obj_ready));
         } else {
             VKN_TRY(run_chain_fast(d, w, pw, raw ? s.xraw : xfeat, raw, s.cnt, obj_in, c.obj_out, cls_logits, c.cls_sigmoid, kern32, s, st,
-                                   chain_h2(pw, flags, have_cls)));
+                                   chain_h2(pw, flags, have_cls), fold));
             if (c.obj_ready && hipEventRecord(c.obj_ready, st) != hipSuccess) return VKN_E_LAUNCH;
         }
         VKN_TRY(emit_masks(d, c, s, ref_decode, s.kern32, kb, touch_nx, touch_nx_bytes, flags, st));
@@ -719,7 +748,7 @@
     VknGemmProb pr[2];
     for (int i = 0; i < nl; ++i) {
         int np = 0;
-        if (i < d->n_cls_fcs) {
+        if (have_cls && i < d->n_cls_fcs) {
             float* dst = (i & 1) ? s.t2 : s.t1;
             e = mk_epi(d); e.ln_w = w->cls_ln_w[i]; e.ln_b = w->cls_ln_b[i]; e.act = 1; e.out = dst; e.ldo = C;
             pr[np++] = VknGemmProb{tc, nullptr, nullptr, nullptr, C, w->cls_fc_w[i], pw.cls_fc[i], C, e};
@@ -732,7 +761,7 @@
             pr[np++] = VknGemmProb{tm, nullptr, nullptr, nullptr, C, w->mask_fc_w[i], pw.mask_fc[i], C, e};
             tm = dst;
         }
-        VKN_TRY(vkn_launch_gemm_group(pr, np, M, C, 1, nullptr, st));
+        if (np) VKN_TRY(vkn_launch_gemm_group(pr, np, M, C, 1, nullptr, st));
     }
     auto to_kernels = [&](VknEpi& ep) {
         ep.ldo = C;
@@ -1461,6 +1490,7 @@
     const float* o_in = proposal_feats;
     SideStream* joined = nullptr;
     bool up_done = false;
+    bool partials_pending = false;
     for (int sidx = 0; sidx < num_stages; ++sidx) {
         const bool last = (sidx == num_stages - 1);
         if (!last && !do_a) {
@@ -1484,9 +1514,11 @@
         const VknStageWeights* ltrack = (last && track_out) ? link_track : nullptr;
         StageCall c{};
         c.w = &stages[sidx]; c.x = x; c.obj_in = o_in; c.obj_out = o_out;
-        c.cls_logits = last ? cls_prob : ctmp;
+        c.cls_logits = last ? cls_prob : ((flags & VKN_FLAG_CLS_ALL_STAGES) ? ctmp : nullptr);
         c.cls_sigmoid = last;
         c.from = (use_fused && sidx > 0) ? FROM_GATHERED : (b_in ? FROM_BITS : FROM_LOGITS);
+        c.partials_in = c.from == FROM_GATHERED && partials_pending;
+        partials_pending = false;
         c.masks_in = m_in; c.bits_in = b_in;
         c.link_pre = prev_pre ? link_pre : nullptr; c.prev_pre = prev_pre;
         c.link_track = ltrack; c.track_src = track_src;
@@ -1502,6 +1534,16 @@
                     c.touch_next_bytes = stages[sidx + 1].prepared_bytes;
                 }
             }
+        }
+        if (!last && use_fused) {
+            const bool nlast = (sidx + 1 == num_stages - 1);
+            const float* nprev_pre = (nlast && link_pre) ? prev_obj : nullptr;
+            const bool nseq = nprev_pre && (flags & VKN_FLAG_CLIP_LINK) && (d->B > 1 || ph);
+            const VknStageWeights* nltrack = (nlast && track_out) ? link_track : nullptr;
+            const bool nneed_xfeat = (nprev_pre && link_pre->dyn_w) || (nltrack && track_src == 1);
+            const bool ncls = stages[sidx + 1].fc_cls_w && (nlast || (flags & VKN_FLAG_CLS_ALL_STAGES));
+            c.next_folds = !nseq && fold_ok(d, &stages[sidx + 1], flags, ncls, nneed_xfeat);
+            partials_pending = c.next_folds;
         }
         hipEvent_t ev0 = last ? static_cast<hipEvent_t>(ev_decode_start) : nullptr;
         hipEvent_t ev1 = last ? static_cast<hipEvent_t>(ev_decode_stop) : nullptr;
diff --git a/video-k-net_amd/csrc/vkn_chain.hip b/video-k-net_amd/csrc/vkn_chain.hip
--- a/video-k-net_amd/csrc/vkn_chain.hip
+++ b/video-k-net_amd/csrc/vkn_chain.hip
@@ -303,12 +303,8 @@
 }
 #endif
 
-__device__ __forceinline__ void ch_img_load(ch_e* img, const float* __restrict__ src, int ld, int m0, int M, int tid, float* rs = nullptr) {
+__device__ __forceinline__ void ch_img_put(ch_e* img, f32x4 (&t)[4], int tid, float* rs) {
     const int row = tid >> 4, c4 = (tid & 15) << 2;
-    const float* s = src + (size_t)min(m0 + row, M - 1) * ld + c4;
-    f32x4 t[4];
-#pragma unroll
-    for (int j = 0; j < 4; ++j) t[j] = *reinterpret_cast<const f32x4*>(s + 64 * j);
 #ifdef CH_H2
     {
         float m = 0.f;
@@ -335,6 +331,64 @@
 #pragma unroll
         for (int i = 0; i < CH_NPL; ++i) *reinterpret_cast<ch_ex4*>(d + i * CH_PLANE) = o[i];
     }
+}
+__device__ __forceinline__ void ch_img_load(ch_e* img, const float* __restrict__ src, int ld, int m0, int M, int tid, float* rs = nullptr) {
+    const int row = tid >> 4, c4 = (tid & 15) << 2;
+    const float* s = src + (size_t)min(m0 + row, M - 1) * ld + c4;
+    f32x4 t[4];
+#pragma unroll
+    for (int j = 0; j < 4; ++j) t[j] = *reinterpret_cast<const f32x4*>(s + 64 * j);
+    ch_img_put(img, t, tid, rs);
+}
+__device__ __forceinline__ void ch_img_reduce(ch_e* img, const float* __restrict__ part, int G, int N, int NPT, int m0, int M, int tid,
+                                              int* status, float* rs = nullptr) {
+    const int row = tid >> 4, c4 = (tid & 15) << 2;
+    const int m = min(m0 + row, M - 1), b = m / N, n = m - b * N;
+    const size_t gs = (size_t)NPT * CH_C;
+    const float* p = part + ((size_t)b * G * NPT + n) * CH_C + c4;
+    const int G4 = G & ~3;
+    f32x4 t[4];
+#pragma unroll
+    for (int j0 = 0; j0 < 4; j0 += 2) {
+        f32x4 sm[4][2];
+#pragma unroll
+        for (int k = 0; k < 4; ++k) sm[k][0] = sm[k][1] = f32x4{0.f, 0.f, 0.f, 0.f};
+        int gi = 0;
+        for (; gi + 8 <= G4; gi += 8) {
+            f32x4 v[8][2];
+#pragma unroll
+            for (int u = 0; u < 8; ++u)
+#pragma unroll
+                for (int j = 0; j < 2; ++j) v[u][j] = *reinterpret_cast<const f32x4*>(p + (size_t)(gi + u) * gs + 64 * (j0 + j));
+#pragma unroll
+            for (int u = 0; u < 8; ++u)
+#pragma unroll
+                for (int j = 0; j < 2; ++j) sm[u & 3][j] += v[u][j];
+        }
+        for (; gi < G4; gi += 4) {
+            f32x4 v[4][2];
+#pragma unroll
+            for (int u = 0; u < 4; ++u)
+#pragma unroll
+                for (int j = 0; j < 2; ++j) v[u][j] = *reinterpret_cast<const f32x4*>(p + (size_t)(gi + u) * gs + 64 * (j0 + j));
+#pragma unroll
+            for (int u = 0; u < 4; ++u)
+#pragma unroll
+                for (int j = 0; j < 2; ++j) sm[u][j] += v[u][j];
+        }
+        for (; gi < G; ++gi)
+#pragma unroll
+            for (int j = 0; j < 2; ++j) sm[0][j] += *reinterpret_cast<const f32x4*>(p + (size_t)gi * gs + 64 * (j0 + j));
+#pragma unroll
+        for (int j = 0; j < 2; ++j) t[j0 + j] = (sm[0][j] + sm[1][j]) + (sm[2][j] + sm[3][j]);
+    }
+    bool fin = true;
+#pragma unroll
+    for (int j = 0; j < 4; ++j)
+#pragma unroll
+        for (int e = 0; e < 4; ++e) fin = fin && (fabsf(t[j][e]) <= 3.0e38f);
+    if (status && !fin) atomicOr(status, VKN_STATUS_RANGE);
+    ch_img_put(img, t, tid, rs);
 }
 #ifdef CH_H2
 #define CH_UNSCALE(A, U)                                     \
@@ -414,6 +468,9 @@
     float* qkv;
     const float* consts;
     int* status;
+    const float* part;
+    const float* cntp;
+    int G, N, NPT;
 };
 
 template <int ABL>
@@ -447,13 +504,24 @@
     }
     ch_stage_consts<CA_TOTAL>(CST, A.consts, tid);
 #ifdef CH_H2
-    ch_img_load(IMG0, A.a0, CH_C, m0, M, tid, RS);
-    ch_img_load(IMG1, A.obj_in, CH_C, m0, M, tid, RS + 32);
+    float* const rs0 = RS;
+    float* const rs1 = RS + 32;
 #else
-    ch_img_load(IMG0, A.a0, CH_C, m0, M, tid);
-    ch_img_load(IMG1, A.obj_in, CH_C, m0, M, tid);
-#endif
-    const float bs = A.rowscale ? A.rowscale[min(row, M - 1)] : 1.f;
+    float* const rs0 = nullptr;
+    float* const rs1 = nullptr;
+#endif
+    float bs = 1.f;
+    if (A.part) {
+        ch_img_reduce(IMG0, A.part, A.G, A.N, A.NPT, m0, M, tid, A.status, rs0);
+        const int m = min(row, M - 1), fb = m / A.N, n = m - fb * A.N;
+        const float* cp = A.cntp + (size_t)fb * A.G * A.NPT + n;
+        bs = 0.f;
+        for (int gi = 0; gi < A.G; ++gi) bs += cp[(size_t)gi * A.NPT];
+    } else {
+        ch_img_load(IMG0, A.a0, CH_C, m0, M, tid, rs0);
+        if (A.rowscale) bs = A.rowscale[min(row, M - 1)];
+    }
+    ch_img_load(IMG1, A.obj_in, CH_C, m0, M, tid, rs1);
     CH_BAR();
 
     int sb = 0;
@@ -605,7 +673,7 @@
     int* status;
 };
 
-template <int ABL>
+template <int ABL, bool CLS>
 __global__ __launch_bounds__(CH_THREADS) void k_chain_c(const ChainCArgs A) {
     extern __shared__ __attribute__((aligned(16))) char smem_cc[];
     ch_e* IMG0 = reinterpret_cast<ch_e*>(smem_cc);
@@ -684,7 +752,8 @@
         ch_img_write(HID, h, L);
         CH_BAR();
         const bool lastc = (c + 1 == A.nchunks);
-        const ChNext nx = lastc ? ChNext{A.off_clsfc, A.off_maskfc, 2} : ChNext{A.off_ffn1 + (unsigned)(c + 1) * 8u * CH_WTILE, 0u, 1};
+        const ChNext nx = !lastc ? ChNext{A.off_ffn1 + (unsigned)(c + 1) * 8u * CH_WTILE, 0u, 1}
+                                 : (CLS ? ChNext{A.off_clsfc, A.off_maskfc, 2} : ChNext{A.off_maskfc, 0u, 1});
         ch_gemm<1, true, ABL>(acc2, HID, HID, A.off_ffn2 + (unsigned)c * 8u * CH_WTILE, 0u, nx, R, wrs, L);
     }
     CH_UNSCALE(acc2[0], CST[CC_SC + 2]);
@@ -703,20 +772,38 @@
     f32x16 acc[2];
     ch_zero(acc[0]);
     ch_zero(acc[1]);
-    const ChNext nfin = A.has_cls ? ChNext{A.off_fccls, A.off_dec, 2} : ChNext{A.off_dec, 0u, 1};
-    ch_gemm<2, true, ABL>(acc, IMG0, IMG0, A.off_clsfc, A.off_maskfc, nfin, R, wrs, L);
-    CH_UNSCALE(acc[0], CST[CC_SC + 3]);
-    CH_UNSCALE(acc[1], CST[CC_SC + 4]);
+    const ChNext nfin = CLS ? ChNext{A.off_fccls, A.off_dec, 2} : ChNext{A.off_dec, 0u, 1};
     {
         float t[2][16];
-#pragma unroll
-        for (int r = 0; r < 16; ++r) {
-            t[0][r] = acc[0][r];
-            t[1][r] = acc[1][r];
-        }
-        const float* const lw[2] = {CST + CC_CLN_W, CST + CC_MLN_W};
-        const float* const lb[2] = {CST + CC_CLN_B, CST + CC_MLN_B};
-        ch_layernorm<2>(t, lw, lb, A.eps, S, sb, L);
+        if constexpr (CLS) {
+            ch_gemm<2, true, ABL>(acc, IMG0, IMG0, A.off_clsfc, A.off_maskfc, nfin, R, wrs, L);
+            CH_UNSCALE(acc[0], CST[CC_SC + 3]);
+            CH_UNSCALE(acc[1], CST[CC_SC + 4]);
+#pragma unroll
+            for (int r = 0; r < 16; ++r) {
+                t[0][r] = acc[0][r];
+                t[1][r] = acc[1][r];
+            }
+            const float* const lw[2] = {CST + CC_CLN_W, CST + CC_MLN_W};
+            const float* const lb[2] = {CST + CC_CLN_B, CST + CC_MLN_B};
+            ch_layernorm<2>(t, lw, lb, A.eps, S, sb, L);
+        } else {
+            f32x16 accm[1];
+            ch_zero(accm[0]);
+            ch_gemm<1, true, ABL>(accm, IMG0, IMG0, A.off_maskfc, 0u, nfin, R, wrs, L);
+            CH_UNSCALE(accm[0], CST[CC_SC + 4]);
+            float tm[1][16];
+#pragma unroll
+            for (int r = 0; r < 16; ++r) tm[0][r] = accm[0][r];
+            const float* const lw[1] = {CST + CC_MLN_W};
+            const float* const lb[1] = {CST + CC_MLN_B};
+            ch_layernorm<1>(tm, lw, lb, A.eps, S, sb, L);
+#pragma unroll
+            for (int r = 0; r < 16; ++r) {
+                t[0][r] = 0.f;
+                t[1][r] = tm[0][r];
+            }
+        }
         float dv[16], kd[1];
         ch_cols(CST + CC_DVEC, L, dv);
         kd[0] = 0.f;
@@ -726,7 +813,7 @@
             t[1][r] = fmaxf(t[1][r], 0.f);
             kd[0] += t[1][r] * dv[r];
         }
-        ch_img_write(IMG0, t[0], L);
+        if (CLS) ch_img_write(IMG0, t[0], L);
         ch_img_write(HID, t[1], L);
         ch_rowsum<1>(kd, S + sb * CH_SBUF, L);
         sb ^= 1;
@@ -734,7 +821,7 @@
     }
     ch_zero(acc[0]);
     ch_zero(acc[1]);
-    if (A.has_cls) {
+    if constexpr (CLS) {
         ch_gemm<2, false, ABL>(acc, IMG0, HID, A.off_fccls, A.off_dec, ChNext{0u, 0u, 0}, R, wrs, L);
         CH_UNSCALE(acc[0], CST[CC_SC + 5]);
         if (L.wave * 32 < A.ncls && row_ok && A.cls_out) {
@@ -1088,13 +1175,15 @@
 #endif
 
 int vkn_launch_chain_a(const VknChainA& p, hipStream_t stream) {
-    if (!p.a0 || !p.obj_in || !p.wbase || !p.obj1 || !p.qkv || !p.consts || p.M <= 0 || p.wbytes >= (1ull << 31)) return VKN_E_ARG;
+    if ((!p.a0 && !p.part) || !p.obj_in || !p.wbase || !p.obj1 || !p.qkv || !p.consts || p.M <= 0 || p.wbytes >= (1ull << 31)) return VKN_E_ARG;
+    if (p.part && (!p.cntp || p.G <= 0 || p.N <= 0 || p.NPT < p.N || p.M % p.N != 0)) return VKN_E_ARG;
     ChainAArgs A{};
     A.a0 = p.a0; A.obj_in = p.obj_in; A.rowscale = p.rowscale; A.wbase = p.wbase; A.wbytes = (unsigned)p.wbytes;
     A.off_dyn = p.off_dyn; A.off_inp = p.off_inp; A.off_ig = p.off_ig; A.off_ug = p.off_ug; A.off_fc = p.off_fc; A.off_in = p.off_in;
     A.eps = p.eps; A.M = p.M; A.obj1 = p.obj1; A.qkv = p.qkv;
-    A.consts = p.consts + (p.rowscale ? 0 : CA_TOTAL);
+    A.consts = p.consts + ((p.rowscale || p.part) ? 0 : CA_TOTAL);
     A.status = p.status;
+    A.part = p.part; A.cntp = p.cntp; A.G = p.G; A.N = p.N; A.NPT = p.NPT;
 #ifdef CH_H2
     const size_t lds = (size_t)2 * CH_IMG * sizeof(ch_e) + (size_t)(2 * CH_SBUF + CA_TOTAL + 16 * CH_THREADS + 64 + 512) * sizeof(float);
 #else
@@ -1146,10 +1235,15 @@
 #else
     const size_t lds = (size_t)2 * CH_IMG * sizeof(ch_e) + (size_t)(2 * CH_SBUF + CC_TOTAL) * sizeof(float);
 #endif
-#define CHC_LAUNCH(ABLV)                                                                                            \
-    do {                                                                                                            \
-        VKN_ALLOW_FULL_LDS(k_chain_c<ABLV>);                                                                        \
-        hipLaunchKernelGGL(k_chain_c<ABLV>, dim3((p.M + CH_ROWS - 1) / CH_ROWS), dim3(CH_THREADS), lds, stream, A); \
+#define CHC_LAUNCH_(ABLV, CLSV)                                                                                             \
+    do {                                                                                                                    \
+        VKN_ALLOW_FULL_LDS((k_chain_c<ABLV, CLSV>));                                                                        \
+        hipLaunchKernelGGL((k_chain_c<ABLV, CLSV>), dim3((p.M + CH_ROWS - 1) / CH_ROWS), dim3(CH_THREADS), lds, stream, A); \
+    } while (0)
+#define CHC_LAUNCH(ABLV)                        \
+    do {                                        \
+        if (A.has_cls) CHC_LAUNCH_(ABLV, true); \
+        else CHC_LAUNCH_(ABLV, false);          \
     } while (0)
 #ifdef VKN_DEBUG
     switch (vkn_dbg_env("VKN_CHAIN_ABL", 0)) {
@@ -1170,6 +1264,7 @@
     CHC_LAUNCH(0);
 #endif
 #undef CHC_LAUNCH
+#undef CHC_LAUNCH_
     VKN_CHECK_LAUNCH();
     return VKN_OK;
 }
diff --git a/video-k-net_amd/csrc/vkn_common.h b/video-k-net_amd/csrc/vkn_common.h
--- a/video-k-net_amd/csrc/vkn_common.h
+++ b/video-k-net_amd/csrc/vkn_common.h
@@ -68,6 +68,17 @@
 }
 #undef VKN_DPP_STEP
 
+__device__ __forceinline__ void vkn_touch_slice(const char* __restrict__ touch, unsigned touch_bytes, unsigned wg, unsigned nwg,
+                                                unsigned tid, unsigned nthr) {
+    if (!touch) return;
+    const unsigned per = (touch_bytes / nwg + 15u) & ~15u;
+    const unsigned t0 = wg * per, t1 = min(t0 + per, touch_bytes & ~15u);
+    for (unsigned o = t0 + tid * 16u; o < t1; o += nthr * 16u) {
+        const f32x4 v = *reinterpret_cast<const f32x4*>(touch + o);
+        asm volatile("" ::"v"(v));
+    }
+}
+
 #define VKN_OK 0
 #define VKN_E_ARG (-1)
 #define VKN_E_SHAPE (-2)
diff --git a/video-k-net_amd/csrc/vkn_fused.hip b/video-k-net_amd/csrc/vkn_fused.hip
--- a/video-k-net_amd/csrc/vkn_fused.hip
+++ b/video-k-net_amd/csrc/vkn_fused.hip
@@ -40,7 +40,8 @@
 __global__ __launch_bounds__(FS_THREADS, 2) void k_fused_il(const float* __restrict__ x, const _Float16* __restrict__ kfh,
                                                              const _Float16* __restrict__ kfl, const float* __restrict__ kb,
                                                              float thr, float* __restrict__ part, float* __restrict__ cntp,
-                                                             int N, int NPT, int n0_in, int P, int NZ) {
+                                                             int N, int NPT, int n0_in, int P, int NZ,
+                                                             const char* __restrict__ touch, unsigned touch_bytes) {
     constexpr int KS = C / 16;
     constexpr int NFG = KS / 16, NFD = KS / 4 - NFG, NF = NFD;
     static_assert(KS % 4 == 0 && 4 * (NFD + NFG) == KS, "C must be a multiple of 64");
@@ -432,6 +433,7 @@
             }
         }
     }
+    vkn_touch_slice(touch, touch_bytes, blockIdx.y * gridDim.x + blockIdx.x, gridDim.x * gridDim.y, tid, FS_THREADS);
 }
 
 #ifdef VKN_DEBUG
@@ -457,8 +459,11 @@
 
 int vkn_launch_fused_decode_gather(const float* x, const _Float16* kfh, const _Float16* kfl, const float* kb, float thr,
                                    float* xraw, float* cnt, float* part, float* cntp, int B, int N, int C, int P,
-                                   hipStream_t stream, int xdt, int* status, const void* touch, size_t touch_bytes) {
+                                   hipStream_t stream, int xdt, int* status, const void* touch, size_t touch_bytes,
+                                   int keep_partials) {
     if (B <= 0 || N <= 0 || P <= 0 || xdt < 0 || xdt > 2) return VKN_E_ARG;
+    if (touch_bytes >= (1ull << 31)) touch = nullptr;
+    const char* const touch_il = keep_partials ? static_cast<const char*>(touch) : nullptr;
     if (!vkn_fused_supported(C, P)) return VKN_E_SHAPE;
     const int NPT = (N + 31) / 32 * 32;
     const int G = vkn_gather_groups(B, P);
@@ -497,7 +502,7 @@
     do {                                                                                                                       \
         VKN_ALLOW_FULL_LDS((k_fused_il<NBV, CV, XHV, PFV>));                                                                   \
         hipLaunchKernelGGL((k_fused_il<NBV, CV, XHV, PFV>), grid, dim3(FS_THREADS), lds, stream, x, kfh, kfl, kb, thr, part,   \
-                           cntp, N, NPT, n0, P, NZ);                                                                           \
+                           cntp, N, NPT, n0, P, NZ, touch_il, (unsigned)touch_bytes);                                          \
     } while (0)
 #ifdef VKN_DEBUG
 #define FU_LAUNCH_W4(NBV, CV, XHV, PFV)                                                                                        \
@@ -603,6 +608,7 @@
 #endif
         VKN_CHECK_LAUNCH();
     }
+    if (keep_partials) return VKN_OK;
     return vkn_launch_gather_reduce(part, cntp, xraw, cnt, B, N, C, G, stream, status, touch, touch_bytes);
 }
 
diff --git a/video-k-net_amd/csrc/vkn_gather.hip b/video-k-net_amd/csrc/vkn_gather.hip
--- a/video-k-net_amd/csrc/vkn_gather.hip
+++ b/video-k-net_amd/csrc/vkn_gather.hip
@@ -11,7 +11,8 @@
                                                                const float* __restrict__ masks, float thr,
                                                                float* __restrict__ part, float* __restrict__ cntp, int N,
                                                                int NPT, int n0, int C, int P, int px_per_wg,
-                                                               long long mask_fs, int ileave, int x_alias) {
+                                                               long long mask_fs, int ileave, int x_alias,
+                                                               const char* __restrict__ touch, unsigned touch_bytes) {
     extern __shared__ __attribute__((aligned(16))) char smem[];
     constexpr bool REAL = (BITS == 2 || BITS == 3);
     static_assert(!(XH && REAL), "half-storage x: binary operands only");
@@ -294,6 +295,7 @@
 #pragma unroll
         for (int r = 0; r < 16; ++r) cp[n0 + wave * 32 + vkn_cd_row(r, lane)] = accc[r];
     }
+    vkn_touch_slice(touch, touch_bytes, blockIdx.y * gridDim.x + blockIdx.x, gridDim.x * gridDim.y, tid, GA_THREADS);
 }
 
 template <int NB>
@@ -441,14 +443,7 @@
                                                         float* __restrict__ xraw, float* __restrict__ cnt, int N, int NPT,
                                                         int C, int G, int* __restrict__ status, const char* __restrict__ touch,
                                                         unsigned touch_bytes) {
-    if (touch) {
-        const unsigned per = (touch_bytes / gridDim.x + 15u) & ~15u;
-        const unsigned t0 = blockIdx.x * per, t1 = min(t0 + per, touch_bytes & ~15u);
-        for (unsigned o = t0 + threadIdx.x * 16u; o < t1; o += 256u * 16u) {
-            const f32x4 v = *reinterpret_cast<const f32x4*>(touch + o);
-            asm volatile("" ::"v"(v));
-        }
-    }
+    vkn_touch_slice(touch, touch_bytes, blockIdx.x, gridDim.x, threadIdx.x, 256u);
     __shared__ f32x4 comb[3][64];
     const int row = blockIdx.x;
     const int b = row / N, n = row - b * N;
@@ -530,18 +525,20 @@
 }
 
 int vkn_launch_gather(const float* x, const float* masks, float thr, float* xraw, float* cnt, float* part, float* cntp,
-                      int B, int N, int C, int P, hipStream_t stream, int xdt, int* status, const void* touch, size_t touch_bytes) {
-    return vkn_launch_gather_ex(x, masks, thr, xraw, cnt, part, cntp, B, N, C, P, N, stream, xdt, status, touch, touch_bytes);
+                      int B, int N, int C, int P, hipStream_t stream, int xdt, int* status, const void* touch, size_t touch_bytes,
+                      int keep_partials) {
+    return vkn_launch_gather_ex(x, masks, thr, xraw, cnt, part, cntp, B, N, C, P, N, stream, xdt, status, touch, touch_bytes, keep_partials);
 }
 
 static int gather_launch(const float* x, const float* masks, float thr, float* xraw, float* cnt, float* part, float* cntp, int B,
                          int N, int C, int P, int mask_rows, int bits, hipStream_t stream, int xdt = 0, int* status = nullptr,
-                         const void* touch = nullptr, size_t touch_bytes = 0, int x_alias = -1);
+                         const void* touch = nullptr, size_t touch_bytes = 0, int x_alias = -1, int keep_partials = 0);
 
 int vkn_launch_gather_ex(const float* x, const float* masks, float thr, float* xraw, float* cnt, float* part, float* cntp,
                          int B, int N, int C, int P, int mask_rows, hipStream_t stream, int xdt, int* status, const void* touch,
-                         size_t touch_bytes) {
-    return gather_launch(x, masks, thr, xraw, cnt, part, cntp, B, N, C, P, mask_rows, 0, stream, xdt, status, touch, touch_bytes);
+                         size_t touch_bytes, int keep_partials) {
+    return gather_launch(x, masks, thr, xraw, cnt, part, cntp, B, N, C, P, mask_rows, 0, stream, xdt, status, touch, touch_bytes, -1,
+                         keep_partials);
 }
 
 int vkn_launch_gather_real(const float* x, const float* a, float* xraw, float* cnt, float* part, float* cntp, int B, int N, int C,
@@ -557,16 +554,19 @@
 }
 
 int vkn_launch_gather_bits(const float* x, const unsigned* bits, float* xraw, float* cnt, float* part, float* cntp, int B, int N,
-                           int C, int P, hipStream_t stream, int xdt, int* status, const void* touch, size_t touch_bytes) {
+                           int C, int P, hipStream_t stream, int xdt, int* status, const void* touch, size_t touch_bytes,
+                           int keep_partials) {
     if ((P % 64) != 0) return VKN_E_SHAPE;
     return gather_launch(x, reinterpret_cast<const float*>(bits), 0.f, xraw, cnt, part, cntp, B, N, C, P, N, 1, stream, xdt, status, touch,
-                         touch_bytes);
+                         touch_bytes, -1, keep_partials);
 }
 
 static int gather_launch(const float* x, const float* masks, float thr, float* xraw, float* cnt, float* part, float* cntp, int B,
                          int N, int C, int P, int mask_rows, int bits, hipStream_t stream, int xdt, int* status, const void* touch,
-                         size_t touch_bytes, int x_alias) {
+                         size_t touch_bytes, int x_alias, int keep_partials) {
     if (x_alias >= 0 && bits != 2) return VKN_E_ARG;
+    if (touch_bytes >= (1ull << 31)) touch = nullptr;
+    const char* const touch_c = static_cast<const char*>(touch);
     if (B <= 0 || N <= 0 || P <= 0 || mask_rows < N) return VKN_E_ARG;
     if (xdt < 0 || xdt > 2) return VKN_E_ARG;
     if (xdt && (bits >= 2 || (P % 64) != 0)) return VKN_E_SHAPE;
@@ -609,7 +609,8 @@
     do {                                                                                                         \
         VKN_ALLOW_FULL_LDS((k_gather_mfma<NBV, BV, XHV>));                                                       \
         hipLaunchKernelGGL((k_gather_mfma<NBV, BV, XHV>), grid, block, lds, stream, x, masks, thr, part, cntp, N, NPT, n0, C, P, \
-                           px_per_wg, mask_fs, ileave, x_alias);                                                 \
+                           px_per_wg, mask_fs, ileave, x_alias, (keep_partials && n0 + 128 >= NPT) ? touch_c : nullptr,             \
+                           (unsigned)touch_bytes);                                                               \
     } while (0)
 #define GA_CASE(NBV)                                 \
     case NBV:                                        \
@@ -634,8 +635,9 @@
 #undef GA_LAUNCH
         VKN_CHECK_LAUNCH();
     }
-    hipLaunchKernelGGL(k_gather_reduce, dim3(B * N), dim3(256), 0, stream, part, cntp, xraw, cnt, N, NPT, C, G, status,
-                       static_cast<const char*>(touch), (unsigned)(touch_bytes < (1ull << 31) ? touch_bytes : 0));
+    if (keep_partials) return VKN_OK;
+    hipLaunchKernelGGL(k_gather_reduce, dim3(B * N), dim3(256), 0, stream, part, cntp, xraw, cnt, N, NPT, C, G, status, touch_c,
+                       (unsigned)touch_bytes);
     VKN_CHECK_LAUNCH();
     return VKN_OK;
 }
diff --git a/video-k-net_amd/csrc/vkn_launch.h b/video-k-net_amd/csrc/vkn_launch.h
--- a/video-k-net_amd/csrc/vkn_launch.h
+++ b/video-k-net_amd/csrc/vkn_launch.h
@@ -39,7 +39,7 @@
 int vkn_gather_groups(int B, int P);
 int vkn_launch_gather_ex(const float* x, const float* masks, float thr, float* xraw, float* cnt, float* part, float* cntp,
                          int B, int N, int C, int P, int mask_rows, hipStream_t stream, int xdt = 0, int* status = nullptr,
-                         const void* touch = nullptr, size_t touch_bytes = 0);
+                         const void* touch = nullptr, size_t touch_bytes = 0, int keep_partials = 0);
 int vkn_launch_gather_ref_ex(const float* x, const float* masks, float thr, float* xraw, float* cnt, int B, int N, int C,
                              int P, int mask_rows, hipStream_t stream);
 int vkn_launch_gather_real(const float* x, const float* a, float* xraw, float* cnt, float* part, float* cntp, int B, int N, int C,
@@ -48,17 +48,17 @@
                            int N, int C, int P, int mask_rows, hipStream_t stream);
 int vkn_launch_gather_bits(const float* x, const unsigned* bits, float* xraw, float* cnt, float* part, float* cntp, int B, int N,
                            int C, int P, hipStream_t stream, int xdt = 0, int* status = nullptr, const void* touch = nullptr,
-                           size_t touch_bytes = 0);
+                           size_t touch_bytes = 0, int keep_partials = 0);
 int vkn_launch_gather_reduce(const float* part, const float* cntp, float* xraw, float* cnt, int B, int N, int C, int G,
                              hipStream_t stream, int* status = nullptr, const void* touch = nullptr, size_t touch_bytes = 0);
 int vkn_fused_supported(int C, int P);
 int vkn_launch_fused_decode_gather(const float* x, const _Float16* kfh, const _Float16* kfl, const float* kb, float thr,
                                    float* xraw, float* cnt, float* part, float* cntp, int B, int N, int C, int P,
                                    hipStream_t stream, int xdt = 0, int* status = nullptr, const void* touch = nullptr,
-                                   size_t touch_bytes = 0);
+                                   size_t touch_bytes = 0, int keep_partials = 0);
 int vkn_launch_gather(const float* x, const float* masks, float thr, float* xraw, float* cnt, float* part, float* cntp,
                       int B, int N, int C, int P, hipStream_t stream, int xdt = 0, int* status = nullptr, const void* touch = nullptr,
-                      size_t touch_bytes = 0);
+                      size_t touch_bytes = 0, int keep_partials = 0);
 int vkn_launch_gather_ref(const float* x, const float* masks, float thr, float* xraw, float* cnt, int B, int N, int C,
                           int P, hipStream_t stream);
 struct VknDecodeStrides {
@@ -142,6 +142,9 @@
     float* obj1;
     float* qkv;
     int* status;
+    const float* part;
+    const float* cntp;
+    int G, N, NPT;
 };
 struct VknChainC {
     const float* ao;
diff --git a/video-k-net_amd/ops.py b/video-k-net_amd/ops.py
--- a/video-k-net_amd/ops.py
+++ b/video-k-net_amd/ops.py
@@ -20,6 +20,8 @@
 FLAG_INIT_SEPARATE = _H['VKN_FLAG_INIT_SEPARATE']
 FLAG_CHAIN_KSPLIT = _H['VKN_FLAG_CHAIN_KSPLIT']
 FLAG_SERIAL_LINK = _H['VKN_FLAG_SERIAL_LINK']
+FLAG_REDUCE_SEPARATE = _H['VKN_FLAG_REDUCE_SEPARATE']
+FLAG_CLS_ALL_STAGES = _H['VKN_FLAG_CLS_ALL_STAGES']
 
 _tls = threading.local()
 
```
